# Sukikui/PTI-LDM-VAE

Measured on AMD Instinct MI355X. Metric: vae_train_images_per_sec_256x256, higher is better.
Workload: dtype fp16 forward operands + activations / bf16 backward operands + gradients, fp32 accumulate; 1 GPU; config/vae_dente_no_adv.json 256x256x1 batch 32/GPU: fwd + L1 + 1e-3*KL + bwd + all-reduce + Adam (perceptual term omitted: --perceptual times it; adversarial branch inactive before epoch 6, --adv times it); global_batch=32, parallelism=dp1

## Files before the change

### include/pti_vae.h

```cpp
#ifndef PTI_VAE_H
#define PTI_VAE_H

#include <stdint.h>

#ifdef __cplusplus
extern "C" {
#endif

typedef void* pti_stream_t;

#define PTI_ABI_VERSION 5

#define PTI_OK 0
#define PTI_EINVAL (-1)
#define PTI_EUNSUPPORTED (-2)
#define PTI_ELAUNCH (-3)

#define PTI_CONV_S1 0
#define PTI_CONV_S2PAD 1
#define PTI_CONV_UP2 2
#define PTI_CONV_ZINS 3

#define PTI_PRO_NONE 0
#define PTI_PRO_GN 1
#define PTI_PRO_GN_SILU 2

typedef struct pti_conv_desc {
  int32_t n, h, w, cin;
  int32_t ho, wo, cout;
  int32_t ksize;
  int32_t mode;
  int32_t prologue;
  int32_t groups;
  int32_t add_residual;
  int32_t accum_stats;
  int32_t out_groups;
  float eps;
  int32_t in_f32;
  int32_t out_f32;
  int64_t in_stride[4];
  int64_t out_stride[4];
  int32_t in_f16, res_f16, out_f16;
  int32_t pool2x2_out;
  int32_t w_f16;
  int32_t relu_out;
} pti_conv_desc;

int pti_abi_version(void);
const char* pti_last_error_string(void);
const char* pti_last_kernel_name(void);

int64_t pti_conv_packed_bytes(int cout, int cin, int ksize, int mode);
int pti_conv_pack_weights(const float* const* w_oihw, int nsrc, void* packed, int cout, int cin,
                          int ksize, int mode, int transpose_flip, int w_f16, pti_stream_t s);

int pti_conv_pack_entry_bytes(void);
int pti_conv_pack_table_fill(void* host_entry, const float* w_oihw_dev, void* packed_dev, int cout,
                             int cin, int ksize, int mode, int transpose_flip, int w_f16, int64_t* nblocks);
int pti_conv_pack_weights_batched(const void* table_dev, const int* blk_first_dev, int n,
                                  int total_blocks, pti_stream_t s);

int pti_gn_stats(const void* x_nhwc_16bit, int64_t* stats, int n, int hw, int c, int groups,
                 int x_f16, pti_stream_t s);

int pti_conv2d_mfma(const void* x, const void* w_packed, const float* bias, const int64_t* in_stats,
                    const float* gamma, const float* beta, const void* residual, void* y,
                    int64_t* out_stats, const pti_conv_desc* d, pti_stream_t s);

int pti_conv2d_mfma_saveact(const void* x, const void* w_packed, const float* bias, const int64_t* in_stats,
                            const float* gamma, const float* beta, const void* residual, void* y,
                            int64_t* out_stats, void* act_out, const pti_conv_desc* d, pti_stream_t s);

int pti_conv2d_direct(const void* x, const float* w_tck, const float* bias, const int64_t* in_stats,
                      const float* gamma, const float* beta, void* y, const pti_conv_desc* d,
                      pti_stream_t s);

#define PTI_DIRECT_REPACK_MAX 8
typedef struct {
  const float* w; const float* b;
  float* w_tck; float* w_tck_t; float* wpad; float* bpad;
  int cout, cin, pad_cin, reserved;
} pti_direct_repack_entry;
typedef struct {
  pti_direct_repack_entry e[PTI_DIRECT_REPACK_MAX];
  int n;
} pti_direct_repack_table;
int pti_direct_repack(const pti_direct_repack_table* t, pti_stream_t s);

int pti_wgrad_direct(const void* wide, const void* narrow, float* dw, float* dbias_wide,
                     float* dbias_narrow, const int64_t* in_stats, const float* gamma,
                     const float* beta, int n, int h, int w, int cw, int cn, int ksize, int sgn,
                     int prologue, int groups, float eps, int narrow_f32, int wide_f16,
                     const int64_t* narrow_stride, int64_t dw_stride_tap, int64_t dw_stride_cw,
                     int64_t dw_stride_k, void* workspace, int64_t workspace_bytes, pti_stream_t s);

int64_t pti_conv_wgrad_workspace_bytes(int cout, int cin, int ksize, int splits);
int pti_conv_wgrad_mfma(const void* x, const void* dy, const int64_t* in_stats, const float* gamma,
                        const float* beta, float* dw, float* dbias, void* workspace,
                        int64_t workspace_bytes, int accumulate, const pti_conv_desc* d,
                        pti_stream_t s);
int pti_conv_wgrad_mfma_partials(const void* x, const void* dy, const int64_t* in_stats,
                                 const float* gamma, const float* beta, void* workspace,
                                 int64_t workspace_bytes, const pti_conv_desc* d, int* splits_out,
                                 pti_stream_t s);
int pti_conv_wgrad_reduce(const void* workspace, int splits, float* dw, float* dbias,
                          int accumulate, const pti_conv_desc* d, pti_stream_t s);

#define PTI_WGRAD_BATCH_MAX 16
typedef struct pti_wgrad_job {
  const void* x;
  const void* dy;
  float* dw;
  float* dbias;
  int32_t n, h, w, cin, cout;
  int32_t accumulate;
} pti_wgrad_job;
int pti_conv_wgrad_mfma_batched(const pti_wgrad_job* jobs, int njobs, void* workspace, int64_t workspace_bytes,
                                pti_stream_t s);
int pti_conv_wgrad_batched_mode(int n, int h, int w, int cin, int cout);

int pti_gn_bwd_blocks(int n, int hw, int c);
int pti_gn_bwd(const void* x, const void* da, const void* dres, void* dx, const int64_t* stats,
               const float* gamma, const float* beta, float* sums, float* partials, float* dgamma,
               float* dbeta, int n, int hw, int c, int groups, float eps, int silu, int x_f16,
               pti_stream_t s);
int pti_conv_gnbwd_tiles(const pti_conv_desc* d);
int pti_conv_gnbwd_chain_supported(int cin, int cout, int ksize);
int pti_conv2d_mfma_gnbwd_chain(const void* g_in, const void* x_in, int x_in_f16, const int64_t* in_stats,
                                const float* in_gamma, const float* in_sums, void* dx_in_out, const void* w_packed,
                                const void* gx, const int64_t* gstats, const float* ggamma, const float* gbeta,
                                void* dy_out, float* gsums, const pti_conv_desc* d, int silu, pti_stream_t s);
int pti_gn_affine_grads(const float* sums, float* dgamma, float* dbeta, int n, int c, pti_stream_t s);
int pti_gn_sums_finalize_affine(const float* partials, float* sums, int n, int tiles, int row_len, const float* affine_sums,
                                float* dgamma, float* dbeta, int affine_c, pti_stream_t s);
int pti_conv2d_mfma_gnbwd(const void* dy_in, const void* w_packed, const void* gx, const int64_t* gstats,
                          const float* ggamma, const float* gbeta, void* dy_out, float* gpartials,
                          const pti_conv_desc* d, int silu, pti_stream_t s);
int pti_gn_sums_finalize(const float* partials, float* sums, int n, int tiles, int row_len,
                         pti_stream_t s);
int pti_gn_bwd_apply(const void* x, const void* dy, const void* dres, void* dx, const int64_t* stats,
                     const float* gamma, const float* beta, const float* sums, float* dgamma,
                     float* dbeta, int n, int hw, int c, int groups, float eps, int x_f16,
                     pti_stream_t s);
int pti_pool2x2_sum(const void* x, void* y, int n, int h, int w, int c, pti_stream_t s);

int pti_attention_fwd(const void* qkv, void* o, float* lse2, int b, int l, int c, pti_stream_t s);
int pti_attention_bwd(const void* qkv, const void* o, const void* dout, const float* lse2,
                      float* delta, void* dqkv, int b, int l, int c, pti_stream_t s);

int pti_latent_head_fwd(const float* h, const float* eps, const float* wm, const float* bm,
                        const float* wl, const float* bl, const float* wp, const float* bp,
                        float* mu, float* sigma, float* logvar, float* zq, int b, int hw, int l,
                        pti_stream_t s);
int pti_post_quant(const float* z_nchw, const float* wp, const float* bp, float* zq_nhwc, int b,
                   int hw, int l, pti_stream_t s);
#define PTI_POST_QUANT_BWD_MAX_BLOCKS 256
#define PTI_POST_QUANT_BWD_WS_FLOATS(l) (PTI_POST_QUANT_BWD_MAX_BLOCKS * ((l) * (l) + (l)))
int pti_post_quant_bwd(const float* dzq_nhwc, const float* z_nchw, const float* wp, float* dz_nchw,
                       float* gwp, float* gbp, float* workspace, int b, int hw, int l,
                       pti_stream_t s);
#define PTI_LATENT_BWD_MAX_BLOCKS 512
#define PTI_LATENT_BWD_WS_FLOATS(l) (PTI_LATENT_BWD_MAX_BLOCKS * 3 * ((l) * (l) + (l)))
int pti_latent_head_bwd(const float* h, const float* eps, const float* wm, const float* bm,
                        const float* wl, const float* bl, const float* wp, const float* bp,
                        const float* dzq, const float* dmu, const float* dsigma, float* dh,
                        float* gwm, float* gbm, float* gwl, float* gbl, float* gwp, float* gbp,
                        float* workspace, int b, int hw, int l, pti_stream_t s);

#define PTI_VAE_LOSS_MAX_BLOCKS 1024
#define PTI_VAE_LOSS_WS_FLOATS (2 * PTI_VAE_LOSS_MAX_BLOCKS)
int pti_vae_loss(const float* recon, const float* images, int64_t npix, const float* mu,
                 const float* third, int64_t nlat, int batch, float* out2, float* d_recon,
                 float* d_mu, float* d_third, float* workspace, int l2, int third_mode,
                 float kl_weight, pti_stream_t s);

int pti_ar_vae_loss(const float* mu_nchw, int b, int l, int hw, const float* attrs, const int32_t* channels,
                    const float* deltas, int na, const uint8_t* pair_mask, float gamma, float* per_attr,
                    int32_t* counts, float* d_mu, pti_stream_t s);

int pti_adam_step(float* p, const float* g, float* m, float* v, int64_t n, float lr, float beta1,
                  float beta2, float eps, int step, float grad_scale, pti_stream_t s);

int pti_cast_nchw_f32_to_nhwc_bf16(const float* x, void* y, int n, int c, int hw, pti_stream_t s);
int pti_cast_nhwc_bf16_to_nchw_f32(const void* x, float* y, int n, int c, int hw, pti_stream_t s);

int pti_preprocess_batch(const float* src, const int64_t* offsets, const int32_t* hw, int b, int hp, int wp,
                         float* out, double* stats, pti_stream_t s);

int pti_pd_im2col_image(const float* img, void* patches, int n, int h, int w, pti_stream_t s);
int pti_pd_im2col(const void* src, const float* norm, void* patches, int n, int h, int w, int c, int stride,
                  int act, float slope, pti_stream_t s);
int pti_pd_in_stats(const void* y, float* table, int n, int hw, int c, float eps, pti_stream_t s);
int pti_pd_col2im_blocks(int n, int hw, int c);
int pti_pd_col2im(const void* d_patches, const void* y_prev, const float* norm, void* g, float* partials, int n,
                  int h, int w, int c, int stride, float slope, pti_stream_t s);
int pti_pd_col2im_image(const void* d_patches, float* d_img, int n, int h, int w, float scale, int accumulate,
                        pti_stream_t s);
int pti_pd_in_bwd_apply(const void* g, const void* y, const float* norm, const float* sums, void* dy, int n, int hw,
                        int c, pti_stream_t s);
int pti_pd_lsgan_blocks(int count);
int pti_pd_lsgan(const void* logits, int logits_f16, int stride, int count, float target, float slope,
                 float grad_scale, float* loss_out, void* d_logits, pti_stream_t s);

int pti_pd_final_fwd(const void* y_prev, const float* norm, const float* w, const float* bias, float* logits, int n,
                     int h, int w_, int c, float slope, pti_stream_t s);
int pti_pd_final_dgrad(const float* d_logits, const void* y_prev, const float* norm, const float* w, void* g,
                       float* partials, int n, int h, int w_, int c, float slope, pti_stream_t s);
int pti_pd_final_wgrad_blocks(int n, int h, int w_);
int pti_pd_final_wgrad(const float* d_logits, const void* y_prev, const float* norm, float* partials, int n, int h,
                       int w_, int c, float slope, pti_stream_t s);

int pti_lpips_tap_blocks(int c, int hw);
int pti_lpips_tap_fwd(const float* a, const float* b, const float* w, float* saved, float* partials, int n, int c, int hw,
                      pti_stream_t s);
int pti_lpips_tap_bwd(const float* a, const float* b, const float* w, const float* saved, const float* gout, float* ga,
                      int n, int c, int hw, pti_stream_t s);

int pti_relu_f16(void* x, int64_t count, pti_stream_t s);
int pti_relu_bwd(void* g, const void* y, int64_t count, pti_stream_t s);
int pti_relu_bwd_add(void* g, const void* g2, const void* y, int64_t count, pti_stream_t s);
int pti_maxpool3s2_out(int h);
int pti_maxpool3s2_fwd(const void* x, void* y, int n, int h, int w, int c, pti_stream_t s);
int pti_maxpool3s2_bwd(const void* gy, const void* x, const void* y, void* gx, int n, int h, int w, int c, int accumulate,
                       pti_stream_t s);
int pti_squeeze_conv1_fwd(const float* x, const float* w10, void* y, int n, int h, int w, pti_stream_t s);
int pti_squeeze_conv1_bwd(const void* g, const void* t0, const float* w10, float* dx, int n, int h, int w, pti_stream_t s);
int pti_nchw_f32_to_nhwc_f16(const float* x, void* y, int n, int c, int hw, pti_stream_t s);
int pti_nhwc_bf16_add_to_nchw_f32(const void* g, float* y, int n, int c, int hw, pti_stream_t s);
int pti_pad_nchw_to_nhwc32(const float* x, void* ya, void* yb, int n, int c, int hw, int a_f16, int b_f16, pti_stream_t s);
int pti_slice_nhwc32_to_nchw(const void* x, float* y, int n, int c, int hw, int x_f16, pti_stream_t s);
int pti_lpips_tap_nhwc_blocks(int c, int hw);
int pti_lpips_tap_nhwc_fwd(const void* a, const void* b, const float* w, float* saved, float* partials, int n, int c,
                           int hw, pti_stream_t s);
int pti_lpips_tap_nhwc_bwd(const void* a, const void* b, const float* w, const float* saved, const float* gout, void* ga,
                           int n, int c, int hw, pti_stream_t s);


int64_t pti_image_metrics_ws_floats(int n, int c, int h, int w);
int pti_image_metrics(const float* pred, const float* target, int n, int c, int h, int w, int clamp, float lo, float hi,
                      float data_range, float k1, float k2, const float* taps11, float* out_n4, float* workspace,
                      pti_stream_t s);

int64_t pti_latent_pairwise_ws_floats(int n1, int n2, int d);
int pti_latent_pairwise(const float* a, int64_t lda, int n1, const float* b, int64_t ldb, int n2, int d, const float* center,
                        int mode, float* out, int64_t ldo, float* workspace, pti_stream_t s);
int64_t pti_latent_group_stats_ws_floats(int n1, int n2, int patients, int d);
int pti_latent_group_stats(const float* a, int64_t lda, int n1, const int32_t* seg_a, const float* b, int64_t ldb, int n2,
                           const int32_t* seg_b, int patients, int d, float* out_e4, float* workspace, pti_stream_t s);

int pti_mask_geometry(const void* src, const int64_t* offsets, const int32_t* hw, int b, int elem, int max_h,
                      const int32_t* sample_rows, int samples, const int32_t* bottom_offsets, int n_bottom,
                      int32_t* bbox_b4, int32_t* bbox_widths, int32_t* bottom_widths, pti_stream_t s);

#define PTI_MLP_MAX_LAYERS 8
#define PTI_MLP_MAX_WIDTH 1024
#define PTI_MLP_MAX_OUT 64
int64_t pti_mlp_head_ws_floats(int n, int d, const int32_t* dims, int n_layers);
int pti_mlp_head_fwd(const float* x, int64_t ldx, int n, int d, const float* params, const int32_t* dims, int n_layers,
                     int act, const float* mean, const float* std, const float* targets, int loss_kind, float* pred,
                     float* rowloss, float* workspace, pti_stream_t s);
int pti_regression_metrics(const float* pred, const float* targets, const float* rowloss, int n, int t, int batch,
                           double* out, pti_stream_t s);

#define PTI_ELASTIC_MAX_RADIUS 30
int pti_elastic_field(const uint64_t* keys, const float* alpha, float sigma, int b, int h, int w, float* field,
                      pti_stream_t s);
int pti_augment_warp(const float* src, const float* mat, const float* field, int b, int c, int h, int w, float* out,
                     pti_stream_t s);

int64_t pti_tsne_affinities_ws_floats(int n);
int pti_tsne_affinities(const float* d2, int64_t ldd, int n, float perplexity, float* p, int64_t ldp, double* plogp2,
                        float* workspace, pti_stream_t s);
int64_t pti_tsne_step_ws_floats(int n, int n_components);
int pti_tsne_step(const float* p, int64_t ldp, int n, int n_components, const float* y_in, float* y_out, float* update,
                  float* gains, const double* plogp2, float exaggeration, float momentum, float lr, double* record,
                  int with_record, float* workspace, pti_stream_t s);

int pti_umap_knn(const float* dist, int64_t ldd, int n, int k, int* knn_idx, float* knn_dist, pti_stream_t s);
int64_t pti_umap_graph_capacity(int n, int k);
int64_t pti_umap_graph_ws_floats(int n, int k);
int pti_umap_graph(const int* knn_idx, const float* knn_dist, int n, int k, int n_epochs, int* indptr, int* indices,
                   float* weights, int* rate, int64_t capacity, float* rho, float* sigma, float* workspace, pti_stream_t s);
int pti_umap_epoch(const int* indptr, const int* indices, const int* rate, int64_t capacity, int n, int n_components,
                   const float* y_in, float* y_out, double a, double b, double alpha, int epoch, uint32_t seed,
                   int negative_sample_rate, pti_stream_t s);

int pti_umap_knn_cross(const float* dist, int64_t ldd, int m, int n, int k, int* knn_idx, float* knn_dist, pti_stream_t s);
int64_t pti_umap_transform_graph_ws_floats(int m, int n, int k);
int pti_umap_transform_graph(const int* knn_idx, const float* knn_dist, int m, int k, const float* y_train, int n, int n_epochs,
                             float* sigma, float* weights, int* rate, float* y0, float* workspace, pti_stream_t s);
int pti_umap_transform_layout(const int* knn_idx, const int* rate, int m, int k, const float* y_train, int n, const float* y_in,
                              float* y_out, double a, double b, double initial_alpha, int n_epochs, int epoch_begin,
                              int epoch_end, uint32_t seed, int negative_sample_rate, pti_stream_t s);

int pti_display_planes(const float* a, const float* b, int n, int h, int w, int nsrc, double low, double high, int rot_k,
                       float* out_f32, uint8_t* out_u8, double* stats, pti_stream_t s);

int64_t pti_rank_agreement_ws_bytes(int n, int l, int na);
int pti_rank_agreement(const float* zt, int64_t ldz, const float* attrs, int64_t lda, int n, int l, int na,
                       const int32_t* channels, const float* deltas, int64_t* counts, double* loss_sum, void* workspace,
                       int64_t ws_bytes, pti_stream_t s);

int pti_tied_ranks(const float* cols, int64_t ld, int n, int m, int32_t* rank2, pti_stream_t s);
int pti_rank_moments(const int32_t* rank2, int n, int m, int64_t* sums, int64_t* gram, pti_stream_t s);

int64_t pti_joint_histogram_ws_bytes(int n, int l, int na, int bins);
int pti_joint_histogram(const float* zt, int64_t ldz, const float* attrs, int64_t lda, int n, int l, int na, int bins,
                        const double* edges_z, const double* edges_a, uint8_t* bins_z, uint8_t* bins_a, int32_t* counts,
                        void* workspace, int64_t ws_bytes, pti_stream_t s);

int pti_ksg_counts(const float* zt, int64_t ldz, const float* attrs, int64_t lda, int n, int l, int na, int k, float* eps,
                   int32_t* nx, int32_t* ny, pti_stream_t s);

#define PTI_MASK_COMPARE_MAX_EDGE 1024
#define PTI_MASK_COMPARE_COLUMNS 24
int64_t pti_mask_compare_ws_bytes(int n, int h, int w);
int pti_mask_compare(const float* gt, const float* pred, int n, int h, int w, float threshold, int32_t* counts, double* sums,
                     void* workspace, int64_t ws_bytes, pti_stream_t s);

int pti_neighbor_ranks(const float* dist, int64_t ldd, int n, const int32_t* nbr_idx, int m, int32_t* out, pti_stream_t s);
int pti_segment_row_sums(const float* dist, int64_t ldd, int n, const int32_t* seg, int groups, double* out, pti_stream_t s);
int pti_projection_distances(const float* y, int64_t ldy, int n, int d, float* out, int64_t ldo, pti_stream_t s);

int pti_full_ranks(const float* dist, int64_t ldd, int m, int n, int row0, int16_t* out, int64_t ldo, pti_stream_t s);
int pti_coranking_fold(const int16_t* rank_high, int64_t ldh, const int16_t* rank_low, int64_t ldl, int m, int n, uint32_t* hist,
                       int64_t* sqdiff, pti_stream_t s);
int pti_shepard_fold(const float* dist_high, int64_t ldh, const float* dist_low, int64_t ldl, int n, const float* scale, int bins,
                     double* sums, uint32_t* hist, pti_stream_t s);

#define PTI_MASK_MOMENTS_COLUMNS 10
#define PTI_ALIGN_BOTTOM_COLUMNS 6
int64_t pti_mask_moments_ws_bytes(int n, int h, int w);
int pti_mask_moments(const float* gt, const float* pred, int n, int h, int w, float threshold, float* cleaned, int64_t* moments,
                     double* coeffs, void* workspace, int64_t ws_bytes, pti_stream_t s);
int pti_warp_cubic(const float* gt, const float* pred, const double* coeffs, int n, int h, int w, float* out_gt, float* out_pred,
                   pti_stream_t s);
int pti_align_bottom(const float* rot_gt, const float* rot_pred, int n, int h, int w, float* aligned, int32_t* info,
                     pti_stream_t s);

int64_t pti_ssim_uniform_ws_bytes(int n, int h, int w);
int pti_ssim_uniform(const float* x, const float* y, int n, int h, int w, double data_range, double* out, void* workspace,
                     int64_t ws_bytes, pti_stream_t s);
int pti_mask_compare_cleaned(const float* gt, const float* pred, int n, int h, int w, float threshold, int32_t* counts,
                             double* sums, float* cleaned, void* workspace, int64_t ws_bytes, pti_stream_t s);

#ifdef __cplusplus
}
#endif
#endif
```

### pti_ldm_vae_amd/_lib.py

```python
from __future__ import annotations

import ctypes as C
import os

_HERE = os.path.dirname(os.path.abspath(__file__))
LIB_PATH = os.environ.get("PTI_VAE_LIB") or os.path.join(_HERE, "libpti_vae_hip.so")

def env_overrides() -> dict:
    return {k: v for k, v in sorted(os.environ.items()) if k.startswith("PTI_")}


def refuse_wrong_result_env(who: str) -> None:
    bad = [k for k in os.environ if k.startswith("PTI_") and ("DIAG" in k or k == "PTI_ALLOW_WRONG_RESULTS")]
    if bad:
        raise SystemExit(f"{who}: refusing to run with wrong-result diagnostic variable(s) set: {sorted(bad)} "
                         "(timing diagnostics live in tools/diag_skip.py)")


ABI_VERSION = 5
PTI_CONV_S1, PTI_CONV_S2PAD, PTI_CONV_UP2, PTI_CONV_ZINS = 0, 1, 2, 3
PTI_PRO_NONE, PTI_PRO_GN, PTI_PRO_GN_SILU = 0, 1, 2


class ConvDesc(C.Structure):

    _fields_ = [
        ("n", C.c_int32), ("h", C.c_int32), ("w", C.c_int32), ("cin", C.c_int32),
        ("ho", C.c_int32), ("wo", C.c_int32), ("cout", C.c_int32),
        ("ksize", C.c_int32), ("mode", C.c_int32), ("prologue", C.c_int32), ("groups", C.c_int32),
        ("add_residual", C.c_int32), ("accum_stats", C.c_int32), ("out_groups", C.c_int32),
        ("eps", C.c_float), ("in_f32", C.c_int32), ("out_f32", C.c_int32),
        ("in_stride", C.c_int64 * 4), ("out_stride", C.c_int64 * 4),
        ("in_f16", C.c_int32), ("res_f16", C.c_int32), ("out_f16", C.c_int32), ("pool2x2_out", C.c_int32),
        ("w_f16", C.c_int32), ("relu_out", C.c_int32),
    ]


class WgradJob(C.Structure):

    _fields_ = [("x", C.c_void_p), ("dy", C.c_void_p), ("dw", C.c_void_p), ("dbias", C.c_void_p),
                ("n", C.c_int32), ("h", C.c_int32), ("w", C.c_int32), ("cin", C.c_int32), ("cout", C.c_int32),
                ("accumulate", C.c_int32)]


WGRAD_BATCH_MAX = 16
DIRECT_REPACK_MAX = 8
MASK_COMPARE_COLUMNS = ("n_gt", "n_pred", "components_gt", "components_pred", "kept_gt", "kept_pred", "filled_pred",
                        "intersection", "union", "gt_x", "gt_y", "gt_w", "gt_h", "pred_x", "pred_y", "pred_w", "pred_h",
                        "gt_width_upper", "gt_width_middle", "gt_width_lower",
                        "pred_width_upper", "pred_width_middle", "pred_width_lower", "status")
MASK_MOMENTS_COLUMNS = ("m00", "m10", "m01", "m20", "m11", "m02", "A", "B", "C", "status")
ALIGN_BOTTOM_COLUMNS = ("centre_gt", "centre_pred", "count_gt", "count_pred", "shift", "status")


class DirectRepackEntry(C.Structure):

    _fields_ = [("w", C.c_void_p), ("b", C.c_void_p), ("w_tck", C.c_void_p), ("w_tck_t", C.c_void_p), ("wpad", C.c_void_p),
                ("bpad", C.c_void_p), ("cout", C.c_int32), ("cin", C.c_int32), ("pad_cin", C.c_int32), ("reserved", C.c_int32)]


class DirectRepackTable(C.Structure):

    _fields_ = [("e", DirectRepackEntry * DIRECT_REPACK_MAX), ("n", C.c_int32)]


_P = C.c_void_p
_I = C.c_int
_I64 = C.c_int64
_F = C.c_float
_D = C.c_double
_U32 = C.c_uint32

SIGNATURES = {
    "pti_abi_version": (_I, []),
    "pti_last_error_string": (C.c_char_p, []),
    "pti_last_kernel_name": (C.c_char_p, []),
    "pti_conv_packed_bytes": (_I64, [_I, _I, _I, _I]),
    "pti_conv_pack_weights": (_I, [C.POINTER(_P), _I, _P, _I, _I, _I, _I, _I, _I, _P]),
    "pti_conv_pack_entry_bytes": (_I, []),
    "pti_conv_pack_table_fill": (_I, [_P, _P, _P, _I, _I, _I, _I, _I, _I, C.POINTER(_I64)]),
    "pti_conv_pack_weights_batched": (_I, [_P, _P, _I, _I, _P]),
    "pti_gn_stats": (_I, [_P, _P, _I, _I, _I, _I, _I, _P]),
    "pti_conv2d_mfma": (_I, [_P, _P, _P, _P, _P, _P, _P, _P, _P, C.POINTER(ConvDesc), _P]),
    "pti_conv2d_mfma_saveact": (_I, [_P, _P, _P, _P, _P, _P, _P, _P, _P, _P, C.POINTER(ConvDesc), _P]),
    "pti_conv2d_direct": (_I, [_P, _P, _P, _P, _P, _P, _P, C.POINTER(ConvDesc), _P]),
    "pti_wgrad_direct": (_I, [_P, _P, _P, _P, _P, _P, _P, _P, _I, _I, _I, _I, _I, _I, _I, _I, _I, _F, _I, _I,
                              C.POINTER(_I64), _I64, _I64, _I64, _P, _I64, _P]),
    "pti_conv_wgrad_workspace_bytes": (_I64, [_I, _I, _I, _I]),
    "pti_conv_wgrad_mfma": (_I, [_P, _P, _P, _P, _P, _P, _P, _P, _I64, _I, C.POINTER(ConvDesc), _P]),
    "pti_conv_wgrad_mfma_partials": (_I, [_P, _P, _P, _P, _P, _P, _I64, C.POINTER(ConvDesc), C.POINTER(_I), _P]),
    "pti_conv_wgrad_mfma_batched": (_I, [C.POINTER(WgradJob), _I, _P, _I64, _P]),
    "pti_conv_wgrad_batched_mode": (_I, [_I, _I, _I, _I, _I]),
    "pti_direct_repack": (_I, [C.POINTER(DirectRepackTable), _P]),
    "pti_conv_wgrad_reduce": (_I, [_P, _I, _P, _P, _I, C.POINTER(ConvDesc), _P]),
    "pti_gn_bwd_blocks": (_I, [_I, _I, _I]),
    "pti_gn_bwd": (_I, [_P, _P, _P, _P, _P, _P, _P, _P, _P, _P, _P, _I, _I, _I, _I, _F, _I, _I, _P]),
    "pti_conv_gnbwd_tiles": (_I, [C.POINTER(ConvDesc)]),
    "pti_gn_sums_finalize": (_I, [_P, _P, _I, _I, _I, _P]),
    "pti_conv2d_mfma_gnbwd": (_I, [_P, _P, _P, _P, _P, _P, _P, _P, C.POINTER(ConvDesc), _I, _P]),
    "pti_conv_gnbwd_chain_supported": (_I, [_I, _I, _I]),
    "pti_conv2d_mfma_gnbwd_chain": (_I, [_P, _P, _I, _P, _P, _P, _P, _P, _P, _P, _P, _P, _P, _P, C.POINTER(ConvDesc), _I, _P]),
    "pti_gn_affine_grads": (_I, [_P, _P, _P, _I, _I, _P]),
    "pti_gn_sums_finalize_affine": (_I, [_P, _P, _I, _I, _I, _P, _P, _P, _I, _P]),
    "pti_gn_bwd_apply": (_I, [_P, _P, _P, _P, _P, _P, _P, _P, _P, _P, _I, _I, _I, _I, _F, _I, _P]),
    "pti_pool2x2_sum": (_I, [_P, _P, _I, _I, _I, _I, _P]),
    "pti_attention_fwd": (_I, [_P, _P, _P, _I, _I, _I, _P]),
    "pti_attention_bwd": (_I, [_P, _P, _P, _P, _P, _P, _I, _I, _I, _P]),
    "pti_latent_head_fwd": (_I, [_P] * 12 + [_I, _I, _I, _P]),
    "pti_post_quant": (_I, [_P, _P, _P, _P, _I, _I, _I, _P]),
    "pti_post_quant_bwd": (_I, [_P, _P, _P, _P, _P, _P, _P, _I, _I, _I, _P]),
    "pti_latent_head_bwd": (_I, [_P] * 19 + [_I, _I, _I, _P]),
    "pti_vae_loss": (_I, [_P, _P, _I64, _P, _P, _I64, _I, _P, _P, _P, _P, _P, _I, _I, _F, _P]),
    "pti_ar_vae_loss": (_I, [_P, _I, _I, _I, _P, _P, _P, _I, _P, _F, _P, _P, _P, _P]),
    "pti_pd_im2col_image": (_I, [_P, _P, _I, _I, _I, _P]),
    "pti_pd_im2col": (_I, [_P, _P, _P, _I, _I, _I, _I, _I, _I, _F, _P]),
    "pti_pd_in_stats": (_I, [_P, _P, _I, _I, _I, _F, _P]),
    "pti_pd_col2im_blocks": (_I, [_I, _I, _I]),
    "pti_pd_col2im": (_I, [_P, _P, _P, _P, _P, _I, _I, _I, _I, _I, _F, _P]),
    "pti_pd_col2im_image": (_I, [_P, _P, _I, _I, _I, _F, _I, _P]),
    "pti_pd_in_bwd_apply": (_I, [_P, _P, _P, _P, _P, _I, _I, _I, _P]),
    "pti_pd_lsgan_blocks": (_I, [_I]),
    "pti_pd_lsgan": (_I, [_P, _I, _I, _I, _F, _F, _F, _P, _P, _P]),
    "pti_pd_final_fwd": (_I, [_P, _P, _P, _P, _P, _I, _I, _I, _I, _F, _P]),
    "pti_pd_final_dgrad": (_I, [_P, _P, _P, _P, _P, _P, _I, _I, _I, _I, _F, _P]),
    "pti_pd_final_wgrad_blocks": (_I, [_I, _I, _I]),
    "pti_pd_final_wgrad": (_I, [_P, _P, _P, _P, _I, _I, _I, _I, _F, _P]),
    "pti_lpips_tap_blocks": (_I, [_I, _I]),
    "pti_lpips_tap_fwd": (_I, [_P, _P, _P, _P, _P, _I, _I, _I, _P]),
    "pti_lpips_tap_bwd": (_I, [_P, _P, _P, _P, _P, _P, _I, _I, _I, _P]),
    "pti_relu_f16": (_I, [_P, _I64, _P]),
    "pti_relu_bwd": (_I, [_P, _P, _I64, _P]),
    "pti_relu_bwd_add": (_I, [_P, _P, _P, _I64, _P]),
    "pti_maxpool3s2_out": (_I, [_I]),
    "pti_maxpool3s2_fwd": (_I, [_P, _P, _I, _I, _I, _I, _P]),
    "pti_maxpool3s2_bwd": (_I, [_P, _P, _P, _P, _I, _I, _I, _I, _I, _P]),
    "pti_squeeze_conv1_fwd": (_I, [_P, _P, _P, _I, _I, _I, _P]),
    "pti_squeeze_conv1_bwd": (_I, [_P, _P, _P, _P, _I, _I, _I, _P]),
    "pti_nchw_f32_to_nhwc_f16": (_I, [_P, _P, _I, _I, _I, _P]),
    "pti_pad_nchw_to_nhwc32": (_I, [_P, _P, _P, _I, _I, _I, _I, _I, _P]),
    "pti_slice_nhwc32_to_nchw": (_I, [_P, _P, _I, _I, _I, _I, _P]),
    "pti_nhwc_bf16_add_to_nchw_f32": (_I, [_P, _P, _I, _I, _I, _P]),
    "pti_lpips_tap_nhwc_blocks": (_I, [_I, _I]),
    "pti_lpips_tap_nhwc_fwd": (_I, [_P, _P, _P, _P, _P, _I, _I, _I, _P]),
    "pti_lpips_tap_nhwc_bwd": (_I, [_P, _P, _P, _P, _P, _P, _I, _I, _I, _P]),
    "pti_adam_step": (_I, [_P, _P, _P, _P, _I64, _F, _F, _F, _F, _I, _F, _P]),
    "pti_preprocess_batch": (_I, [_P, _P, _P, _I, _I, _I, _P, _P, _P]),
    "pti_cast_nchw_f32_to_nhwc_bf16": (_I, [_P, _P, _I, _I, _I, _P]),
    "pti_cast_nhwc_bf16_to_nchw_f32": (_I, [_P, _P, _I, _I, _I, _P]),
    "pti_image_metrics_ws_floats": (_I64, [_I, _I, _I, _I]),
    "pti_image_metrics": (_I, [_P, _P, _I, _I, _I, _I, _I, _F, _F, _F, _F, _F, _P, _P, _P, _P]),
    "pti_latent_pairwise_ws_floats": (_I64, [_I, _I, _I]),
    "pti_latent_pairwise": (_I, [_P, _I64, _I, _P, _I64, _I, _I, _P, _I, _P, _I64, _P, _P]),
    "pti_latent_group_stats_ws_floats": (_I64, [_I, _I, _I, _I]),
    "pti_latent_group_stats": (_I, [_P, _I64, _I, _P, _P, _I64, _I, _P, _I, _I, _P, _P, _P]),
    "pti_mask_geometry": (_I, [_P, _P, _P, _I, _I, _I, _P, _I, _P, _I, _P, _P, _P, _P]),
    "pti_mlp_head_ws_floats": (_I64, [_I, _I, C.POINTER(C.c_int32), _I]),
    "pti_mlp_head_fwd": (_I, [_P, _I64, _I, _I, _P, C.POINTER(C.c_int32), _I, _I, _P, _P, _P, _I, _P, _P, _P, _P]),
    "pti_regression_metrics": (_I, [_P, _P, _P, _I, _I, _I, _P, _P]),
    "pti_elastic_field": (_I, [_P, _P, _F, _I, _I, _I, _P, _P]),
    "pti_augment_warp": (_I, [_P, _P, _P, _I, _I, _I, _I, _P, _P]),
    "pti_tsne_affinities_ws_floats": (_I64, [_I]),
    "pti_tsne_affinities": (_I, [_P, _I64, _I, _F, _P, _I64, _P, _P, _P]),
    "pti_tsne_step_ws_floats": (_I64, [_I, _I]),
    "pti_tsne_step": (_I, [_P, _I64, _I, _I, _P, _P, _P, _P, _P, _F, _F, _F, _P, _I, _P, _P]),
    "pti_umap_knn": (_I, [_P, _I64, _I, _I, _P, _P, _P]),
    "pti_umap_graph_capacity": (_I64, [_I, _I]),
    "pti_umap_graph_ws_floats": (_I64, [_I, _I]),
    "pti_umap_graph": (_I, [_P, _P, _I, _I, _I, _P, _P, _P, _P, _I64, _P, _P, _P, _P]),
    "pti_umap_epoch": (_I, [_P, _P, _P, _I64, _I, _I, _P, _P, _D, _D, _D, _I, _U32, _I, _P]),
    "pti_umap_knn_cross": (_I, [_P, _I64, _I, _I, _I, _P, _P, _P]),
    "pti_umap_transform_graph_ws_floats": (_I64, [_I, _I, _I]),
    "pti_umap_transform_graph": (_I, [_P, _P, _I, _I, _P, _I, _I, _P, _P, _P, _P, _P, _P]),
    "pti_umap_transform_layout": (_I, [_P, _P, _I, _I, _P, _I, _P, _P, _D, _D, _D, _I, _I, _I, _U32, _I, _P]),
    "pti_display_planes": (_I, [_P, _P, _I, _I, _I, _I, _D, _D, _I, _P, _P, _P, _P]),
    "pti_rank_agreement_ws_bytes": (_I64, [_I, _I, _I]),
    "pti_rank_agreement": (_I, [_P, _I64, _P, _I64, _I, _I, _I, C.POINTER(C.c_int32), C.POINTER(_F), _P, _P, _P, _I64, _P]),
    "pti_tied_ranks": (_I, [_P, _I64, _I, _I, _P, _P]),
    "pti_rank_moments": (_I, [_P, _I, _I, _P, _P, _P]),
    "pti_joint_histogram_ws_bytes": (_I64, [_I, _I, _I, _I]),
    "pti_joint_histogram": (_I, [_P, _I64, _P, _I64, _I, _I, _I, _I, _P, _P, _P, _P, _P, _P, _I64, _P]),
    "pti_ksg_counts": (_I, [_P, _I64, _P, _I64, _I, _I, _I, _I, _P, _P, _P, _P]),
    "pti_mask_compare_ws_bytes": (_I64, [_I, _I, _I]),
    "pti_mask_compare": (_I, [_P, _P, _I, _I, _I, _F, _P, _P, _P, _I64, _P]),
    "pti_neighbor_ranks": (_I, [_P, _I64, _I, _P, _I, _P, _P]),
    "pti_segment_row_sums": (_I, [_P, _I64, _I, _P, _I, _P, _P]),
    "pti_projection_distances": (_I, [_P, _I64, _I, _I, _P, _I64, _P]),
    "pti_full_ranks": (_I, [_P, _I64, _I, _I, _I, _P, _I64, _P]),
    "pti_coranking_fold": (_I, [_P, _I64, _P, _I64, _I, _I, _P, _P, _P]),
    "pti_shepard_fold": (_I, [_P, _I64, _P, _I64, _I, _P, _I, _P, _P, _P]),
    "pti_mask_moments_ws_bytes": (_I64, [_I, _I, _I]),
    "pti_mask_moments": (_I, [_P, _P, _I, _I, _I, _F, _P, _P, _P, _P, _I64, _P]),
    "pti_warp_cubic": (_I, [_P, _P, _P, _I, _I, _I, _P, _P, _P]),
    "pti_align_bottom": (_I, [_P, _P, _I, _I, _I, _P, _P, _P]),
    "pti_ssim_uniform_ws_bytes": (_I64, [_I, _I, _I]),
    "pti_ssim_uniform": (_I, [_P, _P, _I, _I, _I, _D, _P, _P, _I64, _P]),
    "pti_mask_compare_cleaned": (_I, [_P, _P, _I, _I, _I, _F, _P, _P, _P, _P, _I64, _P]),
}

_lib = None


class PtiError(RuntimeError):
    pass


def lib() -> C.CDLL:
    global _lib
    if _lib is None:
        if not os.path.exists(LIB_PATH):
            raise PtiError(
                f"{LIB_PATH} is missing: the HIP extension was not built. Run "
                "`python -c 'import __graft_entry__ as g; g.build()'` (or pti_ldm_vae_amd/csrc/build.sh). "
                "There is no CPU/PyTorch fallback for the VAE hot path.")
        import torch
        handle = C.CDLL(LIB_PATH)
        for name, (res, args) in SIGNATURES.items():
            fn = getattr(handle, name)
            fn.restype = res
            fn.argtypes = args
        ver = handle.pti_abi_version()
        if ver != ABI_VERSION:
            raise PtiError(f"libpti_vae_hip.so ABI version {ver}, expected {ABI_VERSION}")
        _lib = handle
    return _lib


def check(rc: int, what: str = "") -> None:
    if rc != 0:
        msg = lib().pti_last_error_string()
        raise PtiError(f"{what or 'pti call'} failed (code {rc}): {msg.decode() if msg else ''}")
```

### pti_ldm_vae_amd/csrc/conv_mfma.hip

```cpp
#include "conv_common.h"

namespace {
using namespace pti_conv;

constexpr int TH = 8, TW = 16;

__host__ __device__ constexpr int pick_cout_tile(int cout) { return cout % 128 == 0 ? 128 : (cout % 64 == 0 ? 64 : 32); }
__host__ __device__ constexpr int pick_ck(int cin, int stride2) {
  int ck = cin % 128 == 0 ? 128 : (cin % 64 == 0 ? 64 : 32);
  return (stride2 && ck > 64) ? 64 : ck;
}
__host__ __device__ constexpr int pick_wblk(int kbc, int nt) {
  int best = 1;
  for (int w = 1; w <= kbc; ++w)
    if (kbc % w == 0 && w * nt <= 16) best = w;
  return best;
}

template <int KS, int S, int CK, int COUT_TILE>
struct Cfg {
  static constexpr int HH = (TH - 1) * S + KS, HW = (TW - 1) * S + KS;
  static constexpr int NP = HH * HW;
  static constexpr int NC = CK / 8;
  static constexpr int PIXB = CK * 2;
// ... 474 lines not shown
            if constexpr (OPH) {
              float f[8];
              unpack8f(piece, f, true);
              piece = pack8(f);
            }
            __builtin_amdgcn_raw_buffer_store_b128(__builtin_bit_cast(bu32x4, piece), srs,
                                                   ((unsigned)((n * a.H + vy) * a.W + vx) * a.Cin + chunk * CK + c8 * 8) * 2u, 0, 2 );
          }
        }
      }
    }

    if constexpr (WLATE) wload(wa, 0);
    const int txl = lane & 15;
    auto baddr = [&](int kb) -> const unsigned char* {
      kb = kb < C::KBC ? kb : C::KBC - 1;
      const int tap = kb / C::KPC, kc = kb - tap * C::KPC;
      const int kh = (KS == 3) ? tap / 3 : 0, kw = tap - kh * KS;
      const int hx = txl + kw;
      const int tk = (hsel ^ ((hx >> C::KEY_SHIFT) & (C::NC - 1))) << 4;
      return halo + pbase[0] + (kh * C::HW + kw) * C::PIXB + ((kc * 32) ^ tk);
    };
    bf16x8 b0[PXF], b1[PXF];
    auto bread = [&](bf16x8 (&dst)[PXF], int kb) {
      const unsigned char* bp = baddr(kb);
#pragma unroll
      for (int i = 0; i < PXF; ++i) dst[i] = *(const bf16x8*)(bp + 2 * i * C::HW * C::PIXB);
    };
    auto group = [&](const bf16x8 (&w)[C::R], int g) {
      const int kb0 = g * C::R;
#pragma unroll
      for (int u = 0; u < C::R; ++u) {
        if ((u & 1) == 0) {
          bread(b1, kb0 + u + 1);
#pragma unroll
          for (int i = 0; i < PXF; ++i) acc[i] = mfma32<OPH>(w[u], b0[i], acc[i]);
        } else {
          bread(b0, kb0 + u + 1);
#pragma unroll
          for (int i = 0; i < PXF; ++i) acc[i] = mfma32<OPH>(w[u], b1[i], acc[i]);
        }
      }
      if (C::R & 1) {
#pragma unroll
        for (int i = 0; i < PXF; ++i) b0[i] = b1[i];
      }
    };
    constexpr int NG = C::KBC / C::R;
    bread(b0, 0);
    if constexpr (NG == 1) {
      group(wa, 0);
    } else {
#pragma clang loop unroll(disable)
      for (int g = 0; g < NG; g += 2) {
        wload(wb, g + 1);
        group(wa, g);
        wload(wa, g + 2);
        group(wb, g + 1);
      }
    }
  }

  const int j = lane & 31;
  unsigned char* etile = smem;
  const bool do_stats = (FM == 2 || FM == 3) ? false : a.out_stats != nullptr;
  const int ocpg = do_stats ? a.Cout / a.out_groups : 1;
  __syncthreads();
  float* gtab = reinterpret_cast<float*>(smem + C::GT_OFF);
  if (gn_on) {
    if (tid < CT) {
      gtab[tid] = gq;
      gtab[CT + tid] = bq;
    }
    __syncthreads();
  }
  const unsigned char* rtile = smem + C::RT_OFF;
  const int col0 = wn * 32 + 4 * hsel;
  float st1[4] = {0.f, 0.f, 0.f, 0.f}, st2[4] = {0.f, 0.f, 0.f, 0.f};
  float su1[4] = {0.f, 0.f, 0.f, 0.f}, su2[4] = {0.f, 0.f, 0.f, 0.f};
  if (gn_on) {
    const int gcpg = a.Cout / a.g_groups;
    float* gsm = reinterpret_cast<float*>(smem + C::STAT_OFF);
    float L[32];
#pragma unroll
    for (int q = 0; q < 4; ++q) {
      const int col = col0 + 8 * q, ch0 = ct * CT + col;
      float scv[4], shv[4], muv[4], rsv[4], l1[4] = {0.f, 0.f, 0.f, 0.f}, l2[4] = {0.f, 0.f, 0.f, 0.f};
      gn_params<4>(sfl, gtab - ct * CT, gtab + CT - ct * CT, ch0, gcpg, a.g_inv_cnt, a.g_eps, scv, shv, muv, rsv);
      float nmr[4];
#pragma unroll
      for (int r = 0; r < 4; ++r) nmr[r] = -muv[r] * rsv[r];
#pragma unroll
      for (int i = 0; i < PXF; ++i) {
        const int p = (2 * PXF * wm + 2 * i + (j >> 4)) * 16 + (j & 15);
        const bool inb = (oy0 + (p >> 4) < a.Ho) && (ox0 + (p & 15) < a.Wo);
        unsigned char* ep = etile + p * C::EPITCH + col * 2;
        const u32x2 rr = *(const u32x2*)(rtile + p * (CT * 2) + ((((col >> 3) ^ (p >> 2)) & (C::ENC - 1)) << 4) + (col & 7) * 2);
        float xv[4];
        unpack2f(rr[0], res_f16, xv[0], xv[1]);
        unpack2f(rr[1], res_f16, xv[2], xv[3]);
        float dv[4];
#pragma unroll
        for (int r = 0; r < 4; ++r) {
          float v = acc[i][4 * q + r];
          if (a.gn_mode == 2) v *= dsilu_f(xv[r] * scv[r] + shv[r]);
          dv[r] = v;
        }
        const u32x2 packed = pack4(dv[0], dv[1], dv[2], dv[3]);
        *(u32x2*)ep = packed;
        if (inb) {
#pragma unroll
          for (int r = 0; r < 4; ++r) {
            l1[r] += dv[r];
            l2[r] = fmaf(dv[r], fmaf(xv[r], rsv[r], nmr[r]), l2[r]);
          }
        }
      }
#pragma unroll
      for (int r = 0; r < 4; ++r) {
        L[8 * q + 2 * r] = l1[r];
        L[8 * q + 2 * r + 1] = l2[r];
      }
    }
    fold32<32>(L, j);
    gsm[wm * 2 * CT + col0 * 2 + 16 * (j >> 3) + (j & 7)] = L[0];
  } else {
#pragma unroll
  for (int i = 0; i < PXF; ++i) {
    const int p = (2 * PXF * wm + 2 * i + (j >> 4)) * 16 + (j & 15);
    const bool inb = (oy0 + (p >> 4) < a.Ho) && (ox0 + (p & 15) < a.Wo);
#pragma unroll
    for (int q = 0; q < 4; ++q) {
      const int col = col0 + 8 * q;
      float v0 = acc[i][4 * q + 0], v1 = acc[i][4 * q + 1], v2 = acc[i][4 * q + 2], v3 = acc[i][4 * q + 3];
      if (a.bias) {
        const f32x4 b = *(const f32x4*)(smem + C::BIAS_OFF + col * 4);
        v0 += b[0]; v1 += b[1]; v2 += b[2]; v3 += b[3];
      }
      unsigned char* ep = etile + p * C::EPITCH + col * 2;
      if (a.res) {
        const u32x2 rr = *(const u32x2*)(rtile + p * (CT * 2) + ((((col >> 3) ^ (p >> 2)) & (C::ENC - 1)) << 4) + (col & 7) * 2);
        float e0, e1, e2, e3;
        unpack2f(rr[0], res_f16, e0, e1);
        unpack2f(rr[1], res_f16, e2, e3);
        v0 += e0; v1 += e1; v2 += e2; v3 += e3;
      }
      if constexpr (FM == 1 && PRO == PTI_PRO_NONE) {
        if (a.relu_out) { v0 = fmaxf(v0, 0.f); v1 = fmaxf(v1, 0.f); v2 = fmaxf(v2, 0.f); v3 = fmaxf(v3, 0.f); }
      }
      const u32x2 packed = pack4f(v0, v1, v2, v3, out_f16);
      *(u32x2*)ep = packed;
      if (do_stats && inb) {
        float r0, r1, r2, r3;
        unpack2f(packed[0], out_f16, r0, r1);
        unpack2f(packed[1], out_f16, r2, r3);
        if (ocpg >= 4) {
          st1[q] += (r0 + r1) + (r2 + r3);
          st2[q] += (r0 * r0 + r1 * r1) + (r2 * r2 + r3 * r3);
        } else {
          st1[q] += r0 + r1; st2[q] += r0 * r0 + r1 * r1;
          su1[q] += r2 + r3; su2[q] += r2 * r2 + r3 * r3;
        }
      }
    }
  }
  }
  if (do_stats) {
    stat_t* sstat = reinterpret_cast<stat_t*>(smem + C::STAT_OFF);
    if (ocpg >= 4) {
      float v[8];
#pragma unroll
      for (int q = 0; q < 4; ++q) { v[2 * q] = st1[q]; v[2 * q + 1] = st2[q]; }
      fold32<8>(v, j);
      if ((j & 3) == 0) {
        const int idx = j >> 2, q = idx >> 1;
        const int g = (ct * CT + col0 + 8 * q) / ocpg;
        stat_add(&sstat[2 * g + (idx & 1)], v[0]);
      }
    } else {
      float v[16];
#pragma unroll
      for (int q = 0; q < 4; ++q) { v[4 * q] = st1[q]; v[4 * q + 1] = st2[q]; v[4 * q + 2] = su1[q]; v[4 * q + 3] = su2[q]; }
      fold32<16>(v, j);
      if ((j & 1) == 0) {
        const int idx = j >> 1, q = idx >> 2;
        const int g = (ct * CT + col0 + 8 * q) / 2;
        stat_add(&sstat[2 * g + (idx & 3)], v[0]);
      }
    }
  }
  __syncthreads();
  const __amdgpu_buffer_rsrc_t yrs = __builtin_amdgcn_make_buffer_rsrc(
      a.y, 0, ((unsigned)a.N * (unsigned)a.Ho * (unsigned)a.Wo * (unsigned)a.Cout * 2u) >> (a.pool2 ? 2 : 0), 0x00020000);
  if ((FM == 0 || FM == 2) && a.pool2) {
    constexpr int PITERS = (C::EITERS + 3) / 4;
#pragma unroll
    for (int it = 0; it < PITERS; ++it) {
      const int idx = tid + it * 256;
      const int c8 = idx % C::ENC, pp = idx / C::ENC;
      const int py = pp / 8, px = pp % 8;
      const int oy = (oy0 >> 1) + py, ox = (ox0 >> 1) + px;
      if (pp < C::MPX / 4 && oy < (a.Ho >> 1) && ox < (a.Wo >> 1)) {
        const unsigned char* src = etile + ((2 * py) * 16 + 2 * px) * C::EPITCH + c8 * 16;
        float s_[8], f_[8];
        unpack8f(*(const u32x4*)src, s_, out_f16);
        unpack8f(*(const u32x4*)(src + C::EPITCH), f_, out_f16);
#pragma unroll
        for (int q = 0; q < 8; ++q) s_[q] += f_[q];
        unpack8f(*(const u32x4*)(src + 16 * C::EPITCH), f_, out_f16);
#pragma unroll
        for (int q = 0; q < 8; ++q) s_[q] += f_[q];
        unpack8f(*(const u32x4*)(src + 17 * C::EPITCH), f_, out_f16);
#pragma unroll
        for (int q = 0; q < 8; ++q) s_[q] += f_[q];
        __builtin_amdgcn_raw_buffer_store_b128(__builtin_bit_cast(bu32x4, pack8f(s_, out_f16)), yrs,
                                               ((unsigned)((n * (a.Ho >> 1) + oy) * (a.Wo >> 1) + ox) * a.Cout + ct * CT + c8 * 8) * 2u, 0, 2);
      }
    }
  } else
#pragma unroll
  for (int it = 0; it < C::EITERS; ++it) {
    const int p = epp0 + it * EPSTEP;
    const int oy = oy0 + (p >> 4), ox = ox0 + (p & 15);
    if (oy < a.Ho && ox < a.Wo)
      __builtin_amdgcn_raw_buffer_store_b128(__builtin_bit_cast(bu32x4, *(const u32x4*)(etile + p * C::EPITCH + epc * 16)), yrs,
                                             ((unsigned)((n * a.Ho + oy) * a.Wo + ox) * a.Cout + ct * CT + epc * 8) * 2u, 0, 2);
  }
  if (gn_on) {
    if (tid < 2 * CT) {
      const float* gsm = reinterpret_cast<const float*>(smem + C::STAT_OFF);
      float v = gsm[tid];
#pragma unroll
      for (int m = 1; m < C::WM; ++m) v += gsm[m * 2 * CT + tid];
      a.g_sums[(((size_t)n * a.g_T + tile_y * a.tiles_x + tile_x) * a.Cout + ct * CT) * 2 + tid] = v;
    }
  } else if (do_stats) {
    const stat_t* sstat = reinterpret_cast<const stat_t*>(smem + C::STAT_OFF);
    const int g0 = (ct * CT) / ocpg, ng = CT / ocpg;
    if (tid < 2 * ng)
      atomicAdd((unsigned long long*)&a.out_stats[(n * a.out_groups + g0) * 2 + tid], (unsigned long long)sstat[2 * g0 + tid]);
  }
}

template <int KS, int CK, int CT, int PXF>
int launch2_cfg(ConvArgs a, hipStream_t st) {
  using C = Cfg2<KS, CK, CT, PXF>;
  a.tiles_x = cdiv(a.Wo, C::TW2);
  a.tiles_y = cdiv(a.Ho, C::TH2);
  a.g_T = a.tiles_x * a.tiles_y;
  dim3 grid(a.N * a.tiles_x * a.tiles_y, a.Cout / CT);
  const bool res = a.res != nullptr;
  const int fm = (a.w_f16 && a.in_f16 && a.out_f16 && (a.res_f16 || !res)) ? 1
               : (!a.in_f16 && !a.out_f16 && (!a.res_f16 || !res)) ? 2
               : (!a.in_f16 && !a.out_f16 && a.res_f16) ? 3 : 0;
  const bool fwd_silu = fm == 1 && a.prologue == PTI_PRO_GN_SILU && !a.gn_mode && !a.pool2;
  const bool fwd_plain = fm == 1 && a.prologue == PTI_PRO_NONE && !a.gn_mode && !a.pool2;
  const bool dgrad = fm == 2 && a.prologue == PTI_PRO_NONE && !a.gn_mode && !a.out_stats;
  const bool dgrad_gn = fm == 3 && a.prologue == PTI_PRO_NONE && a.gn_mode && !a.out_stats && !a.pool2;
  if (a.x2) {
    if constexpr (KS == 3 && PXF == 4 && CT == 128) {
      if (!(fm == 3 && a.gn_mode && a.act_out && !a.out_stats && !a.pool2 && a.mode == PTI_CONV_S1 && !a.relu_out)) return 4;
      PTI_LAUNCH((conv_mfma2_kernel<KS, CK, CT, PXF, true, 3, PRO_GNB>), grid, dim3(256), 0, st, a);
      return 0;
    } else {
      return 4;
    }
  }
  if (a.relu_out && !(fwd_plain && !a.act_out)) return 3;
  constexpr int FPRO = PXF == 4 ? PTI_PRO_GN_SILU : -1;
  const bool fwd_gn_rt = fm == 1 && a.prologue == PTI_PRO_GN && !a.gn_mode && !a.pool2 && FPRO < 0;
  if constexpr (KS == 3) {
    if (a.act_out) {
      if (fwd_silu || fwd_gn_rt) PTI_LAUNCH((conv_mfma2_kernel<KS, CK, CT, PXF, true, 1, FPRO>), grid, dim3(256), 0, st, a);
      else if (a.w_f16) return 2;
      else PTI_LAUNCH((conv_mfma2_kernel<KS, CK, CT, PXF, true, 0, -1>), grid, dim3(256), 0, st, a);
      return 0;
    }
  } else if (a.act_out) {
    return 1;
  }
  if (fwd_silu) PTI_LAUNCH((conv_mfma2_kernel<KS, CK, CT, PXF, false, 1, FPRO>), grid, dim3(256), 0, st, a);
  else if (fwd_plain) PTI_LAUNCH((conv_mfma2_kernel<KS, CK, CT, PXF, false, 1, PTI_PRO_NONE>), grid, dim3(256), 0, st, a);
  else if (fm == 1 && !a.gn_mode && !a.pool2) PTI_LAUNCH((conv_mfma2_kernel<KS, CK, CT, PXF, false, 1, -1>), grid, dim3(256), 0, st, a);
  else if (a.w_f16) return 2;
  else if (dgrad) PTI_LAUNCH((conv_mfma2_kernel<KS, CK, CT, PXF, false, 2, PTI_PRO_NONE>), grid, dim3(256), 0, st, a);
  else if (dgrad_gn) PTI_LAUNCH((conv_mfma2_kernel<KS, CK, CT, PXF, false, 3, PTI_PRO_NONE>), grid, dim3(256), 0, st, a);
  else PTI_LAUNCH((conv_mfma2_kernel<KS, CK, CT, PXF, false, 0, -1>), grid, dim3(256), 0, st, a);
  return 0;
}
template <int KS>
int launch2(const ConvArgs& a, int ck, int ct, hipStream_t st) {
  if (ct == 128) {
    if (ck == 128) return launch2_cfg<KS, 128, 128, 4>(a, st);
    if (ck == 64) return launch2_cfg<KS, 64, 128, 4>(a, st);
    return launch2_cfg<KS, 32, 128, 4>(a, st);
  }
  if (ct == 64) {
    if (ck == 64) return launch2_cfg<KS, 64, 64, 2>(a, st);
    return launch2_cfg<KS, 32, 64, 2>(a, st);
  }
  return launch2_cfg<KS, 32, 32, 2>(a, st);
}

struct PackArgs {
  const float* src[4];
  int nsrc;
  bf16* dst;
  int cout_l, cin_l;
  int cout_o, cin_o;
  int ks, ck, cout_tile, flip;
  int f16;
  long long total;
};

__device__ __forceinline__ void pack_eight(const PackArgs& p, int e8) {
  const int NT = p.cout_tile / 32, KPC = p.ck / 16, KBC = p.ks * p.ks * KPC, nch = p.cin_l / p.ck;
  int r = e8;
  const int lane = r % 64; r /= 64;
  const int nt = r % NT; r /= NT;
  const int kb = r % KBC; r /= KBC;
  const int chunk = r % nch;
  const int ct = r / nch;
  const int co = ct * p.cout_tile + nt * 32 + (lane & 31);
  const int tap = kb / KPC, kc = kb % KPC;
  const int ci0 = chunk * p.ck + kc * 16 + 8 * (lane >> 5);
  const int kk = p.ks * p.ks;
  const float* src;
  size_t stride;
  if (!p.flip) {
    const int s_ = co / p.cout_o, cs = co % p.cout_o;
    src = p.src[s_] + ((size_t)cs * p.cin_o + ci0) * kk + tap;
    stride = kk;
  } else {
    src = p.src[0] + ((size_t)ci0 * p.cin_o + co) * kk + (kk - 1 - tap);
    stride = (size_t)p.cin_o * kk;
  }
  float f[8];
#pragma unroll
  for (int j = 0; j < 8; ++j) f[j] = src[j * stride];
  *(u32x4*)(p.dst + (size_t)e8 * 8) = p.f16 ? pack8f(f, true) : pack8(f);
}

__global__ void pack_weights_kernel(PackArgs p) {
  if (p.f16) fp16_saturate_on();
  const long long e8 = (long long)blockIdx.x * blockDim.x + threadIdx.x;
  if (e8 * 8 < p.total) pack_eight(p, (int)e8);
}

__global__ void pack_weights_batched_kernel(const PackArgs* __restrict__ table, const int* __restrict__ blk_first, int n) {
  int lo = 0, hi = n - 1;
  const int b = blockIdx.x;
  while (lo < hi) {
    const int mid = (lo + hi + 1) >> 1;
    if (blk_first[mid] <= b) lo = mid; else hi = mid - 1;
  }
  const PackArgs p = table[lo];
  if (p.f16) fp16_saturate_on();
  const int e8 = (b - blk_first[lo]) * 256 + threadIdx.x;
  if ((long long)e8 * 8 < p.total) pack_eight(p, e8);
}

template <int KS, int S, int CK, int COUT_TILE>
int launch_cfg(const ConvArgs& a, hipStream_t st) {
  dim3 grid(a.N * a.tiles_x * a.tiles_y, a.Cout / COUT_TILE);
  if (a.w_f16) PTI_LAUNCH((conv_mfma_kernel<KS, S, CK, COUT_TILE, true>), grid, dim3(256), 0, st, a);
  else PTI_LAUNCH((conv_mfma_kernel<KS, S, CK, COUT_TILE, false>), grid, dim3(256), 0, st, a);
  return 0;
}

template <int KS, int S, int CK>
int launch_ct(const ConvArgs& a, int cout_tile, hipStream_t st) {
  switch (cout_tile) {
    case 128: return launch_cfg<KS, S, CK, 128>(a, st);
    case 64: return launch_cfg<KS, S, CK, 64>(a, st);
    default: return launch_cfg<KS, S, CK, 32>(a, st);
  }
}

template <int KS, int S>
int launch_ck(const ConvArgs& a, int ck, int cout_tile, hipStream_t st) {
  static_assert(S == 2, "the v1 kernel is kept for the stride-2 gather only");
  switch (ck) {
    case 64: return launch_ct<KS, S, 64>(a, cout_tile, st);
    default: return launch_ct<KS, S, 32>(a, cout_tile, st);
  }
}

}

extern "C" int64_t pti_conv_packed_bytes(int cout, int cin, int ksize, int mode) {
  (void)mode;
  if (cout <= 0 || cin <= 0 || cout % 32 || cin % 32 || (ksize != 1 && ksize != 3)) return 0;
  return (int64_t)2 * cout * cin * ksize * ksize;
}

extern "C" int pti_conv_pack_weights(const float* const* w, int nsrc, void* packed, int cout, int cin,
                                     int ksize, int mode, int transpose_flip, int w_f16, pti_stream_t s) {
  if (!w || !packed || nsrc < 1 || nsrc > 4) PTI_FAIL(PTI_EINVAL, "pack_weights: bad pointer/nsrc");
  if (cout % 32 || cin % 32 || (ksize != 1 && ksize != 3))
    PTI_FAIL(PTI_EUNSUPPORTED, "pack_weights: cout=%d cin=%d k=%d need multiples of 32, k in {1,3}", cout, cin, ksize);
  if (transpose_flip && nsrc != 1) PTI_FAIL(PTI_EINVAL, "pack_weights: transpose_flip needs nsrc=1");
  PackArgs p;
  for (int i = 0; i < 4; ++i) p.src[i] = i < nsrc ? w[i] : nullptr;
  p.nsrc = nsrc;
  p.dst = (bf16*)packed;
  p.cout_o = cout;
  p.cin_o = cin;
  p.cout_l = transpose_flip ? cin : cout * nsrc;
  p.cin_l = transpose_flip ? cout : cin;
  p.ks = ksize;
  p.flip = transpose_flip;
  p.f16 = w_f16 ? 1 : 0;
  p.cout_tile = pick_cout_tile(p.cout_l);
  p.ck = (mode == PTI_CONV_S2PAD) ? pick_ck(p.cin_l, true) : pick_ck2(p.cin_l, p.cout_tile);
  p.total = (long long)p.cout_l * p.cin_l * ksize * ksize;
  const int blocks = (int)((p.total + 2047) / 2048);
  PTI_LAUNCH(pack_weights_kernel, dim3(blocks), dim3(256), 0, (hipStream_t)s, p);
  PTI_CHECK_LAUNCH("pack_weights");
  return PTI_OK;
}

static int fill_pack(PackArgs& p, const float* w, void* packed, int cout, int cin, int ksize, int mode, int flip, int f16) {
  if (cout % 32 || cin % 32 || (ksize != 1 && ksize != 3)) return -1;
  for (int i = 0; i < 4; ++i) p.src[i] = nullptr;
  p.src[0] = w;
  p.nsrc = 1;
  p.dst = (bf16*)packed;
  p.cout_o = cout; p.cin_o = cin;
  p.cout_l = flip ? cin : cout;
  p.cin_l = flip ? cout : cin;
  p.ks = ksize; p.flip = flip; p.f16 = f16 ? 1 : 0;
  p.cout_tile = pick_cout_tile(p.cout_l);
  p.ck = (mode == PTI_CONV_S2PAD) ? pick_ck(p.cin_l, true) : pick_ck2(p.cin_l, p.cout_tile);
  p.total = (long long)p.cout_l * p.cin_l * ksize * ksize;
  return 0;
}

extern "C" int pti_conv_pack_entry_bytes(void) { return (int)sizeof(PackArgs); }
extern "C" int pti_conv_pack_table_fill(void* host_entry, const float* w, void* packed, int cout, int cin, int ksize,
                                        int mode, int transpose_flip, int w_f16, int64_t* nblocks) {
  if (!host_entry || !w || !packed || !nblocks) PTI_FAIL(PTI_EINVAL, "pack_table_fill: null pointer");
  PackArgs p;
  if (fill_pack(p, w, packed, cout, cin, ksize, mode, transpose_flip, w_f16))
    PTI_FAIL(PTI_EUNSUPPORTED, "pack_table_fill: cout=%d cin=%d k=%d", cout, cin, ksize);
  *(PackArgs*)host_entry = p;
  *nblocks = (p.total + 2047) / 2048;
  return PTI_OK;
}
extern "C" int pti_conv_pack_weights_batched(const void* table_dev, const int* blk_first_dev, int n, int total_blocks,
                                             pti_stream_t s) {
  if (!table_dev || !blk_first_dev || n <= 0 || total_blocks <= 0) PTI_FAIL(PTI_EINVAL, "pack_weights_batched: bad args");
  PTI_LAUNCH(pack_weights_batched_kernel, dim3(total_blocks), dim3(256), 0, (hipStream_t)s,
                     (const PackArgs*)table_dev, blk_first_dev, n);
  PTI_CHECK_LAUNCH("pack_weights_batched");
  return PTI_OK;
}

struct GnBwdFuse {
  int mode; const int64_t* stats; const float* gamma; const float* beta; float* sums;
  const void* x2 = nullptr; int x2_f16 = 0; const int64_t* p_stats = nullptr; const float* p_gamma = nullptr; const float* p_sums = nullptr;
};

static int conv2d_mfma_impl(const void* x, const void* w_packed, const float* bias, const int64_t* in_stats,
                            const float* gamma, const float* beta, const void* residual, void* y,
                            int64_t* out_stats, const pti_conv_desc* d, const GnBwdFuse* gf, void* act_out,
                            pti_stream_t s) {
  if (!x || !w_packed || !y || !d) PTI_FAIL(PTI_EINVAL, "conv2d_mfma: null pointer");
  const bool chain = gf && gf->x2;
  if (act_out && !chain && (d->mode != PTI_CONV_S1 || d->prologue == PTI_PRO_NONE || d->ksize != 3))
    PTI_FAIL(PTI_EUNSUPPORTED, "conv2d_mfma: the activated-input side output needs a 3x3 PTI_CONV_S1 launch with a GroupNorm prologue");
  if (d->cin % 32 || d->cout % 32 || d->cin <= 0 || d->cout <= 0)
    PTI_FAIL(PTI_EUNSUPPORTED, "conv2d_mfma: cin=%d cout=%d must be positive multiples of 32", d->cin, d->cout);
  if (d->ksize != 1 && d->ksize != 3) PTI_FAIL(PTI_EUNSUPPORTED, "conv2d_mfma: ksize %d", d->ksize);
  if (d->ksize == 1 && d->mode != PTI_CONV_S1) PTI_FAIL(PTI_EUNSUPPORTED, "conv2d_mfma: 1x1 supports PTI_CONV_S1 only");
  if (d->n <= 0 || d->h <= 0 || d->w <= 0) PTI_FAIL(PTI_EINVAL, "conv2d_mfma: bad dims");
  int eho, ewo;
  switch (d->mode) {
    case PTI_CONV_S1: eho = d->h; ewo = d->w; break;
    case PTI_CONV_S2PAD: eho = (d->h + 1 - 3) / 2 + 1; ewo = (d->w + 1 - 3) / 2 + 1; break;
    case PTI_CONV_UP2: case PTI_CONV_ZINS: eho = 2 * d->h; ewo = 2 * d->w; break;
    default: PTI_FAIL(PTI_EUNSUPPORTED, "conv2d_mfma: mode %d", d->mode);
  }
  if (d->ho != eho || d->wo != ewo)
    PTI_FAIL(PTI_EINVAL, "conv2d_mfma: output %dx%d does not match mode %d on %dx%d (want %dx%d)", d->ho, d->wo,
             d->mode, d->h, d->w, eho, ewo);
  if (d->prologue != PTI_PRO_NONE) {
    if (!in_stats || !gamma || !beta || d->groups <= 0 || d->cin % d->groups)
      PTI_FAIL(PTI_EINVAL, "conv2d_mfma: prologue needs stats/gamma/beta and groups | cin");
    if (d->groups > 32) PTI_FAIL(PTI_EUNSUPPORTED, "conv2d_mfma: prologue supports at most 32 groups");
  }
  if (d->add_residual && !residual) PTI_FAIL(PTI_EINVAL, "conv2d_mfma: add_residual without residual");
  if (d->accum_stats) {
    if (!out_stats || d->out_groups <= 0 || d->cout % d->out_groups) PTI_FAIL(PTI_EINVAL, "conv2d_mfma: bad out stats");
    const int ocpg = d->cout / d->out_groups;
    if (ocpg != 2 && (ocpg % 4 != 0 || ocpg > 32)) PTI_FAIL(PTI_EUNSUPPORTED, "conv2d_mfma: channels/group %d for fused stats", ocpg);
    if (d->out_groups > 64) PTI_FAIL(PTI_EUNSUPPORTED, "conv2d_mfma: fused statistics support at most 64 groups");
  }
  ConvArgs a;
  a.x = (const bf16*)x; a.w = (const unsigned char*)w_packed; a.bias = bias; a.in_stats = (const stat_t*)in_stats;
  a.gamma = gamma; a.beta = beta; a.res = d->add_residual ? (const bf16*)residual : nullptr; a.y = (bf16*)y;
  a.out_stats = d->accum_stats ? (stat_t*)out_stats : nullptr;
  a.N = d->n; a.H = d->h; a.W = d->w; a.Cin = d->cin; a.Ho = d->ho; a.Wo = d->wo; a.Cout = d->cout;
  a.mode = d->mode; a.prologue = d->prologue; a.groups = d->groups; a.out_groups = d->out_groups;
  a.gn_mode = 0; a.g_groups = 0; a.g_inv_cnt = 0.f; a.g_eps = 0.f;
  a.g_stats = nullptr; a.g_gamma = a.g_beta = nullptr; a.g_sums = nullptr; a.g_T = 0;
  a.act_out = (bf16*)act_out;
  a.in_f16 = d->in_f16; a.res_f16 = d->res_f16; a.out_f16 = d->out_f16;
  a.pool2 = d->pool2x2_out;
  a.w_f16 = d->w_f16;
  a.relu_out = d->relu_out;
  if (a.relu_out && (gf || d->mode == PTI_CONV_S2PAD))
    PTI_FAIL(PTI_EUNSUPPORTED, "conv2d_mfma: relu_out is for plain fp16 forward launches (stride-1 gather, no prologue)");
  if (a.w_f16 && !(d->in_f16 && d->out_f16 && (d->res_f16 || !d->add_residual)) )
    PTI_FAIL(PTI_EUNSUPPORTED, "conv2d_mfma: fp16-packed weights need fp16 input, output and residual (the forward convs)");
  if (a.w_f16 && (gf || d->pool2x2_out))
    PTI_FAIL(PTI_EUNSUPPORTED, "conv2d_mfma: fp16-packed weights are for forward launches only");
  if (a.pool2 && (d->mode == PTI_CONV_S2PAD || d->accum_stats || gf || (d->ho & 1) || (d->wo & 1)))
    PTI_FAIL(PTI_EUNSUPPORTED, "conv2d_mfma: pool2x2_out needs a stride-1 gather, even output size, no fused statistics");
  a.eps = d->eps;
  a.inv_cnt = d->prologue != PTI_PRO_NONE ? 1.0f / ((float)(d->cin / d->groups) * (float)d->h * (float)d->w) : 0.f;
  if (gf) {
    if (d->groups > 32) PTI_FAIL(PTI_EUNSUPPORTED, "conv2d_mfma_gnbwd: at most 32 groups");
    a.gn_mode = gf->mode; a.g_groups = d->groups; a.g_eps = d->eps;
    a.g_inv_cnt = 1.0f / ((float)(d->cout / d->groups) * (float)d->ho * (float)d->wo);
    a.g_stats = (const stat_t*)gf->stats; a.g_gamma = gf->gamma; a.g_beta = gf->beta; a.g_sums = gf->sums;
  }
  a.x2 = nullptr; a.p_sums = nullptr; a.x2_f16 = 0;
  if (chain) {
    if (!gf->p_stats || !gf->p_gamma || !gf->p_sums || !act_out || d->mode != PTI_CONV_S1 || d->ksize != 3 ||
        d->cin % d->groups || d->cin / d->groups < 8)
      PTI_FAIL(PTI_EINVAL, "conv2d_mfma_gnbwd_chain: bad arguments (3x3 stride-1, >= 8 channels per group)");
    a.x2 = (const bf16*)gf->x2; a.x2_f16 = gf->x2_f16; a.p_sums = gf->p_sums;
    a.in_stats = (const stat_t*)gf->p_stats; a.gamma = gf->p_gamma; a.groups = d->groups;
    a.inv_cnt = 1.0f / ((float)(d->cin / d->groups) * (float)d->h * (float)d->w);
  }
  if ((long long)d->n * d->ho * d->wo * d->cout * 2 >= (1ll << 31))
    PTI_FAIL(PTI_EUNSUPPORTED, "conv2d_mfma: output tensor of %lld bytes (the stores use 32-bit offsets: < 2 GiB)",
             (long long)d->n * d->ho * d->wo * d->cout * 2);
  if (d->mode != PTI_CONV_S2PAD && (long long)d->n * d->h * d->w * d->cin * 2 >= (1ll << 31))
    PTI_FAIL(PTI_EUNSUPPORTED, "conv2d_mfma: input tensor of %lld bytes (the halo loads use 32-bit offsets: < 2 GiB)",
             (long long)d->n * d->h * d->w * d->cin * 2);
  a.tiles_x = cdiv(d->wo, TW); a.tiles_y = cdiv(d->ho, TH);
  const int cout_tile = pick_cout_tile(d->cout);
  int rc, ck;
  if (d->mode == PTI_CONV_S2PAD) {
    ck = pick_ck(d->cin, true);
    rc = launch_ck<3, 2>(a, ck, cout_tile, (hipStream_t)s);
  } else {
    ck = pick_ck2(d->cin, cout_tile);
    rc = (d->ksize == 3 && d->cin == 128 && d->cout == 128 && !a.x2) ? launch_conv_ws128(a, (hipStream_t)s) : 1;
    if (rc == 1)
      rc = d->ksize == 1 ? launch2<1>(a, ck, cout_tile, (hipStream_t)s) : launch2<3>(a, ck, cout_tile, (hipStream_t)s);
  }
  if (rc == 3) PTI_FAIL(PTI_EUNSUPPORTED, "conv2d_mfma: relu_out needs a plain fp16 forward launch (w_f16, fp16 in/out, no prologue, no side output)");
  if (rc == 2) PTI_FAIL(PTI_EUNSUPPORTED, "conv2d_mfma: no fp16-operand kernel for this launch (w_f16 with this prologue / epilogue)");
  if (rc == 4) PTI_FAIL(PTI_EUNSUPPORTED, "conv2d_mfma_gnbwd_chain: only 3x3 launches on 128-wide input and output tiles with an fp16 GroupNorm input");
  if (rc != 0) PTI_FAIL(PTI_EUNSUPPORTED, "conv2d_mfma: no kernel for ck=%d cout_tile=%d", ck, cout_tile);
  PTI_CHECK_LAUNCH("conv2d_mfma");
  return PTI_OK;
}

extern "C" int pti_conv2d_mfma(const void* x, const void* w_packed, const float* bias, const int64_t* in_stats,
                               const float* gamma, const float* beta, const void* residual, void* y,
                               int64_t* out_stats, const pti_conv_desc* d, pti_stream_t s) {
  return conv2d_mfma_impl(x, w_packed, bias, in_stats, gamma, beta, residual, y, out_stats, d, nullptr, nullptr, s);
}

extern "C" int pti_conv2d_mfma_saveact(const void* x, const void* w_packed, const float* bias, const int64_t* in_stats,
                                       const float* gamma, const float* beta, const void* residual, void* y,
                                       int64_t* out_stats, void* act_out, const pti_conv_desc* d, pti_stream_t s) {
  if (!act_out) PTI_FAIL(PTI_EINVAL, "conv2d_mfma_saveact: null act_out");
  return conv2d_mfma_impl(x, w_packed, bias, in_stats, gamma, beta, residual, y, out_stats, d, nullptr, act_out, s);
}

extern "C" int pti_conv_gnbwd_tiles(const pti_conv_desc* d) {
  if (!d || d->cout % 32 || d->ho <= 0 || d->wo <= 0) return 0;
  const int ct = pick_cout_tile(d->cout);
  const int th = ct == 128 ? 8 : (ct == 64 ? 8 : 16);
  return cdiv(d->ho, th) * cdiv(d->wo, 16);
}

extern "C" int pti_conv_gnbwd_chain_supported(int cin, int cout, int ksize) {
  return ksize == 3 && cin % 128 == 0 && cout % 128 == 0;
}

extern "C" int pti_conv2d_mfma_gnbwd_chain(const void* g_in, const void* x_in, int x_in_f16, const int64_t* in_stats,
                                           const float* in_gamma, const float* in_sums, void* dx_in_out, const void* w_packed,
                                           const void* gx, const int64_t* gstats, const float* ggamma, const float* gbeta,
                                           void* dy_out, float* gsums, const pti_conv_desc* d, int silu, pti_stream_t s) {
  if (!g_in || !x_in || !in_stats || !in_gamma || !in_sums || !dx_in_out || !gx || !gstats || !ggamma || !gbeta || !gsums || !d)
    PTI_FAIL(PTI_EINVAL, "conv2d_mfma_gnbwd_chain: null pointer");
  if (d->mode != PTI_CONV_S1 || d->prologue != PTI_PRO_NONE || d->add_residual || d->accum_stats)
    PTI_FAIL(PTI_EUNSUPPORTED, "conv2d_mfma_gnbwd_chain: plain stride-1 data-gradient launches only");
  if (d->groups <= 0 || d->cout % d->groups || d->cin % d->groups) PTI_FAIL(PTI_EINVAL, "conv2d_mfma_gnbwd_chain: groups must divide cin and cout");
  GnBwdFuse gf{silu ? 2 : 1, gstats, ggamma, gbeta, gsums};
  gf.x2 = x_in; gf.x2_f16 = x_in_f16; gf.p_stats = in_stats; gf.p_gamma = in_gamma; gf.p_sums = in_sums;
  pti_conv_desc dd = *d;
  dd.add_residual = 1;
  return conv2d_mfma_impl(g_in, w_packed, nullptr, nullptr, nullptr, nullptr, gx, dy_out, nullptr, &dd, &gf, dx_in_out, s);
}

extern "C" int pti_conv2d_mfma_gnbwd(const void* dy_in, const void* w_packed, const void* gx, const int64_t* gstats,
                                     const float* ggamma, const float* gbeta, void* dy_out, float* gsums,
                                     const pti_conv_desc* d, int silu, pti_stream_t s) {
  if (!gx || !gstats || !ggamma || !gbeta || !gsums || !d) PTI_FAIL(PTI_EINVAL, "conv2d_mfma_gnbwd: null pointer");
  if (d->mode == PTI_CONV_S2PAD || d->prologue != PTI_PRO_NONE || d->add_residual || d->accum_stats)
    PTI_FAIL(PTI_EUNSUPPORTED, "conv2d_mfma_gnbwd: plain stride-1 / zero-insert data-gradient launches only");
  if (d->groups <= 0 || d->cout % d->groups) PTI_FAIL(PTI_EINVAL, "conv2d_mfma_gnbwd: groups must divide cout");
  GnBwdFuse gf{silu ? 2 : 1, gstats, ggamma, gbeta, gsums};
  pti_conv_desc dd = *d;
  dd.add_residual = 1;
  return conv2d_mfma_impl(dy_in, w_packed, nullptr, nullptr, nullptr, nullptr, gx, dy_out, nullptr, &dd, &gf, nullptr, s);
}
```

### pti_ldm_vae_amd/engine.py

```python
from __future__ import annotations

import contextlib
import gc
import os
import warnings

import torch

from . import ops
from .models import autoencoderkl as M
from .ops import (BF16, F32, PTI_CONV_S1, PTI_CONV_S2PAD, PTI_CONV_UP2, PTI_CONV_ZINS, PTI_PRO_GN, PTI_PRO_GN_SILU,
                  PTI_PRO_NONE)


class _Act:

    __slots__ = ("t", "stats")

    def __init__(self, t, stats=None):
        self.t, self.stats = t, stats


def _empty(shape, like, dtype=BF16):
    return torch.empty(shape, dtype=dtype, device=like.device)


@contextlib.contextmanager
def gc_off_for_capture():
    gc.collect()
    enabled = gc.isenabled()
    gc.disable()
    try:
        yield
    finally:
        if enabled:
            gc.enable()


def capture_or_eager(what, *bodies):
    graphs, results = [], []
    try:
        with gc_off_for_capture():
            for body in bodies:
                g = torch.cuda.CUDAGraph()
                with torch.cuda.graph(g, pool=graphs[0].pool() if graphs else None, capture_error_mode="thread_local"):
                    results.append(body(*results))
                graphs.append(g)
    except Exception as ex:
        warnings.warn(f"HIP-graph capture of {what} failed ({ex!r}); continuing with eager launches")
        torch.cuda.synchronize()
        return None
    return graphs, results


class _MfmaConv:

    def __init__(self, net, wname, bname, ksize, mode, fused_names=None, fwd_f16=True):
        self.net, self.ksize, self.mode = net, ksize, mode
        self.fwd_f16, self.f16 = fwd_f16, False
        self.wname, self.bname, self.fused = wname, bname, fused_names
        if fused_names:
            w0 = net._param_by_name[fused_names[0][0]]
            self.cout, self.cin = 3 * w0.shape[0], w0.shape[1]
        else:
            w = net._param_by_name[wname]
            self.cout, self.cin = w.shape[0], w.shape[1]
        self.wp = self.wpt = None

    def _w(self):
        if self.fused:
            o, n, _ = self.net._slots[self.fused[0][0]]
            return self.net._arena[o:o + 3 * n].view(self.cout, self.cin, 1, 1)
        return self.net._param_by_name[self.wname].data.view(self.cout, self.cin, self.ksize, self.ksize)

    def bias(self):
        if self.fused:
            o, n, _ = self.net._slots[self.fused[0][1]]
            return self.net._arena[o:o + 3 * n]
        return self.net._param_by_name[self.bname].data

    def grads(self):
        if self.fused:
            o, n, _ = self.net._slots[self.fused[0][0]]
            ob, nb, _ = self.net._slots[self.fused[0][1]]
            g = self.net.grad_arena
            return g[o:o + 3 * n], g[ob:ob + 3 * nb]
        return self.net.grad_view(self.wname).view(-1), self.net.grad_view(self.bname)

    def fwd(self, x, *, pro=PTI_PRO_NONE, norm=None, residual=None, want_stats=False, eng=None, act_out=None,
            out_dtype=None):
        n, h, w, _ = x.t.shape
        ho, wo = ops.conv_out_hw(h, w, self.mode)
        y = _empty((n, ho, wo, self.cout), x.t, out_dtype or eng.act_dtype)
        st = eng.new_stats(n) if want_stats else None
        g, b = (norm.weight.data, norm.bias.data) if norm is not None else (None, None)
        ops.conv_mfma(x.t, self.wp, self.bias(), y, cout=self.cout, ksize=self.ksize, mode=self.mode, prologue=pro,
                      in_stats=x.stats if pro else None, gamma=g, beta=b, groups=eng.G, eps=eng.eps,
                      residual=residual, out_stats=st, out_groups=eng.G, act_out=act_out)
        return _Act(y, st)

    def dgrad(self, dy, *, residual=None):
        n, ho, wo, _ = dy.shape
        if self.mode == PTI_CONV_S2PAD:
            out = _empty((n, 2 * ho, 2 * wo, self.cin), dy)
            ops.conv_mfma(dy, self.wpt, None, out, cout=self.cin, ksize=3, mode=PTI_CONV_ZINS, residual=residual)
            return out
        if self.mode == PTI_CONV_UP2:
            pooled = _empty((n, ho // 2, wo // 2, self.cin), dy)
            ops.conv_mfma(dy, self.wpt, None, pooled, cout=self.cin, ksize=self.ksize, mode=PTI_CONV_S1, pool2=True)
            return pooled
        out = _empty((n, ho, wo, self.cin), dy)
        ops.conv_mfma(dy, self.wpt, None, out, cout=self.cin, ksize=self.ksize, mode=PTI_CONV_S1, residual=residual)
        return out

    def dgrad_gn(self, dy, x, norm, *, silu, dres, eng):
        g, sums = self.dgrad_gn_raw(dy, x, norm, silu=silu, eng=eng)
        return self._gn_apply(g, sums, x, norm, dres, eng)

    def _gn_apply(self, g, sums, x, norm, dres, eng):
        dx = _empty(x.t.shape, x.t)
        ops.gn_bwd_apply(x.t, g, dx, x.stats, norm.weight.data, norm.bias.data, sums,
                         norm.net.grad_view(norm.prefix + ".weight"), norm.net.grad_view(norm.prefix + ".bias"),
                         groups=eng.G, eps=eng.eps, dres=dres)
        return dx

    def dgrad_gn_raw(self, dy, x, norm, *, silu, eng):
        n, ho, wo, _ = dy.shape
        g = _empty((n, ho, wo, self.cin), dy)
        sums = eng.zeros(n * self.cin * 2)
        ops.conv_mfma_gnbwd(dy, self.wpt, x.t, x.stats, norm.weight.data, norm.bias.data, g, sums, cout=self.cin,
                            ksize=self.ksize, mode=PTI_CONV_S1, groups=eng.G, eps=eng.eps, silu=silu)
        return g, sums

    def dgrad_gn_chain(self, g_in, x_in, norm_in, sums_in, x, norm, *, silu, dres, eng):
        n, ho, wo, _ = g_in.shape
        dxin = _empty(g_in.shape, g_in)
        dyt = _empty((n, ho, wo, self.cin), g_in)
        sums = eng.zeros(n * self.cin * 2)
        ops.conv_mfma_gnbwd_chain(g_in, x_in.t, x_in.stats, norm_in.weight.data, sums_in, dxin, self.wpt, x.t, x.stats,
                                  norm.weight.data, norm.bias.data, dyt, sums, cout=self.cin, groups=eng.G, eps=eng.eps,
                                  silu=silu, in_dgamma=norm_in.net.grad_view(norm_in.prefix + ".weight"),
                                  in_dbeta=norm_in.net.grad_view(norm_in.prefix + ".bias"))
        return self._gn_apply(dyt, sums, x, norm, dres, eng), dxin

    def wgrad(self, x, dy, *, pro=PTI_PRO_NONE, norm=None, eng=None):
        dw, db = self.grads()
        if eng.batch_wgrad and ops.wgrad_batch_eligible(x.t, dy, self.ksize, self.mode, pro):
            eng.defer_wgrad(x.t, dy, dw, db)
            return
        g, b = (norm.weight.data, norm.bias.data) if norm is not None else (None, None)
        kw = dict(ksize=self.ksize, mode=self.mode, prologue=pro, in_stats=x.stats if pro else None, gamma=g, beta=b,
                  groups=eng.G, eps=eng.eps, accumulate=True)
        with eng.side_stream(x.t, dy, dw, db, *kw.values()) as workspace:
            ops.conv_wgrad_mfma(x.t, dy, dw, db, workspace=workspace, **kw)


class _Norm:
    def __init__(self, net, prefix):
        self.net, self.prefix = net, prefix
        self.weight = net._param_by_name[prefix + ".weight"]
        self.bias = net._param_by_name[prefix + ".bias"]

    def bwd(self, x, da, *, silu, dres, eng):
        n, h, w, c = x.t.shape
        dx = _empty(x.t.shape, x.t)
        sums = eng.zeros(n * c * 2)
        ops.gn_bwd(x.t, da, dx, x.stats, self.weight.data, self.bias.data, sums,
                   self.net.grad_view(self.prefix + ".weight"), self.net.grad_view(self.prefix + ".bias"),
                   groups=eng.G, eps=eng.eps, silu=silu, dres=dres)
        return dx


class _ResBlock:
    def __init__(self, net, p, blk):
        self.norm1, self.norm2 = _Norm(net, p + ".norm1"), _Norm(net, p + ".norm2")
        self.conv1 = _MfmaConv(net, p + ".conv1.conv.weight", p + ".conv1.conv.bias", 3, PTI_CONV_S1)
        self.conv2 = _MfmaConv(net, p + ".conv2.conv.weight", p + ".conv2.conv.bias", 3, PTI_CONV_S1)
        self.nin = None
        if blk.in_channels != blk.out_channels:
            self.nin = _MfmaConv(net, p + ".nin_shortcut.conv.weight", p + ".nin_shortcut.conv.bias", 1, PTI_CONV_S1)
        self.convs = [c for c in (self.conv1, self.conv2, self.nin) if c is not None]
        self.needs_in_stats = True
        self.prefix = p + "."

    def fwd(self, x, eng, want_stats, save):
        a1 = a2 = None
        if save is not None and eng.saves_activated_input(x.t):
            a1 = _empty(x.t.shape, x.t)
        h1 = self.conv1.fwd(x, pro=PTI_PRO_GN_SILU, norm=self.norm1, want_stats=True, eng=eng, act_out=a1)
        sc = x.t if self.nin is None else self.nin.fwd(x, eng=eng).t
        if save is not None and eng.saves_activated_input(h1.t):
            a2 = _empty(h1.t.shape, h1.t)
        out = self.conv2.fwd(h1, pro=PTI_PRO_GN_SILU, norm=self.norm2, residual=sc, want_stats=want_stats, eng=eng,
                             act_out=a2)
        if save is not None:
            save.append((x, h1, a1, a2))
        return out

    @staticmethod
    def _wgrad(conv, x, norm, a, dy, eng):
        if a is not None:
            conv.wgrad(_Act(a), dy, eng=eng)
        else:
            conv.wgrad(x, dy, pro=PTI_PRO_GN_SILU, norm=norm, eng=eng)

    def _shortcut_bwd(self, x, dout, eng):
        if self.nin is None:
            return dout
        dres = self.nin.dgrad(dout)
        self.nin.wgrad(x, dout, eng=eng)
        return dres

    def bwd(self, dout, saved, eng):
        x, h1, a1, a2 = saved
        self._wgrad(self.conv2, h1, self.norm2, a2, dout, eng)
        if eng.gnbwd_chain and ops.gnbwd_chain_supported(self.conv1.cout, self.conv1.cin, 3, x.t.dtype, eng.G):
            g2, sums2 = self.conv2.dgrad_gn_raw(dout, h1, self.norm2, silu=True, eng=eng)
            dres = self._shortcut_bwd(x, dout, eng)
            dx, dh1 = self.conv1.dgrad_gn_chain(g2, h1, self.norm2, sums2, x, self.norm1, silu=True, dres=dres, eng=eng)
            self._wgrad(self.conv1, x, self.norm1, a1, dh1, eng)
            return dx
        dh1 = self.conv2.dgrad_gn(dout, h1, self.norm2, silu=True, dres=None, eng=eng)
        self._wgrad(self.conv1, x, self.norm1, a1, dh1, eng)
        dres = self._shortcut_bwd(x, dout, eng)
        return self.conv1.dgrad_gn(dh1, x, self.norm1, silu=True, dres=dres, eng=eng)


class _Resample:

    def __init__(self, net, wprefix, mode, prefix):
        self.conv = _MfmaConv(net, wprefix + ".weight", wprefix + ".bias", 3, mode)
        self.convs = [self.conv]
        self.needs_in_stats = False
        self.prefix = prefix

    def fwd(self, x, eng, want_stats, save):
        out = self.conv.fwd(x, want_stats=want_stats, eng=eng)
        if save is not None:
            save.append(x)
        return out

    def bwd(self, dout, saved, eng):
        x = saved
        self.conv.wgrad(x, dout, eng=eng)
        return self.conv.dgrad(dout)


class _Attention:
    def __init__(self, net, p):
        self.norm = _Norm(net, p + ".norm")
        a = p + ".attn."
        self.qkv = _MfmaConv(net, None, None, 1, PTI_CONV_S1,
                             fused_names=[(a + "to_q.weight", a + "to_q.bias")], fwd_f16=False)
        self.proj = _MfmaConv(net, a + "out_proj.weight", a + "out_proj.bias", 1, PTI_CONV_S1, fwd_f16=False)
        self.convs = [self.qkv, self.proj]
        self.needs_in_stats = True
        self.prefix = p + "."

    def fwd(self, x, eng, want_stats, save):
        n, h, w, c = x.t.shape
        qkv = self.qkv.fwd(x, pro=PTI_PRO_GN, norm=self.norm, eng=eng, out_dtype=BF16).t
        o = _empty((n, h * w, c), x.t)
        lse = _empty((n, h * w), x.t, F32)
        ops.attention_fwd(qkv.view(n, h * w, 3 * c), o, lse)
        out = self.proj.fwd(_Act(o.view(n, h, w, c)), residual=x.t, want_stats=want_stats, eng=eng)
        if save is not None:
            save.append((x, qkv, o, lse))
        return out

    def bwd(self, dout, saved, eng):
        x, qkv, o, lse = saved
        n, h, w, c = x.t.shape
        do = self.proj.dgrad(dout)
        self.proj.wgrad(_Act(o.view(n, h, w, c)), dout, eng=eng)
        dqkv = _empty(qkv.shape, qkv)
        delta = _empty((n, h * w), qkv, F32)
        ops.attention_bwd(qkv.view(n, h * w, 3 * c), o, do.view(n, h * w, c), lse, delta, dqkv.view(n, h * w, 3 * c))
        self.qkv.wgrad(x, dqkv, pro=PTI_PRO_GN, norm=self.norm, eng=eng)
        return self.qkv.dgrad_gn(dqkv, x, self.norm, silu=False, dres=dout, eng=eng)


class _DirectConv:

    def __init__(self, net, prefix, norm_prefix=None):
        self.net, self.prefix = net, prefix
        self.w = net._param_by_name[prefix + ".weight"]
        self.b = net._param_by_name[prefix + ".bias"]
        self.cout, self.cin = self.w.shape[0], self.w.shape[1]
        self.norm = _Norm(net, norm_prefix) if norm_prefix else None
        self.few_cin = self.cin <= 16
        self.w_tck = self.w_tck_t = None
        self.convs = []
        self.needs_in_stats = self.norm is not None
        narrow, wide = min(self.cin, self.cout), max(self.cin, self.cout)
        self.mfma_narrow = 4 <= narrow <= 32 and wide % 32 == 0
        self.wpad = self.wp_mfma = None
        self.pack_f16 = False
        self.img_mfma = False
        self.wp_img = self.wpt_img = self.wpad_img = self.bpad_img = None
        self.dw_img = self.db_img = None

    def alloc(self):
        w = self.w.data
        if self.w_tck is not None:
            return
        self.w_tck = torch.empty(9, self.cin, self.cout, dtype=F32, device=w.device)
        self.w_tck_t = torch.empty(9, self.cout, self.cin, dtype=F32, device=w.device)
        if self.mfma_narrow:
            shape = (32, self.cin, 3, 3) if self.cout < self.cin else (self.cout, 32, 3, 3)
            self.wpad = torch.zeros(shape, dtype=F32, device=w.device)
            self.bpad = torch.zeros(32, dtype=F32, device=w.device)
        if self.img_mfma:
            shape = (self.cout, 32, 3, 3) if self.cin < self.cout else (32, self.cin, 3, 3)
            self.wpad_img = torch.zeros(shape, dtype=F32, device=w.device)
            self.bpad_img = torch.zeros(32, dtype=F32, device=w.device)
            self.dw_img = torch.zeros(shape, dtype=F32, device=w.device)
            self.db_img = torch.zeros(32, dtype=F32, device=w.device) if self.cout < self.cin else None

    def repack_entries(self):
        w, b = self.w.data, self.b.data
        out = [dict(w=w, b=b, w_tck=self.w_tck, w_tck_t=self.w_tck_t,
                    wpad=self.wpad, bpad=self.bpad if (self.mfma_narrow and self.cout < self.cin) else None)]
        if self.img_mfma:
            out.append(dict(w=w, b=b, wpad=self.wpad_img, bpad=self.bpad_img if self.cout < self.cin else None))
        return out

    def pack_entries(self):
        out = []
        if self.mfma_narrow:
            if self.cout < self.cin:
                out.append(("wp_mfma", (self.wpad, 3, PTI_CONV_S1, False, self.pack_f16)))
            else:
                out.append(("wp_mfma", (self.wpad, 3, PTI_CONV_S1, True, False)))
        if self.img_mfma:
            out.append(("wp_img", (self.wpad_img, 3, PTI_CONV_S1, False, self.pack_f16)))
            if self.cout < self.cin:
                out.append(("wpt_img", (self.wpad_img, 3, PTI_CONV_S1, True, False)))
        return out


class Engine:
    def __init__(self, net: "M.AutoencoderKL"):
        self.net = net
        self.G, self.eps = net.norm_num_groups, float(net.norm_eps)
        self.dev = net.param_arena.device
        self.workspace = ops.wgrad_workspace(self.dev)
        self.packed_version = -1
        self.pack_gen = 0
        self.grad_ready_cb = None
        self._range_cache = {}
        self._zpool, self._zoff, self._zpool_size = None, 0, 1 << 16
        self._packer = None
        self.save_act_min_hw = int(os.environ.get("PTI_SAVE_ACT_MIN_HW", "0"))
        self.act_dtype = {"fp16": torch.float16, "bf16": BF16}[os.environ.get("PTI_FWD_ACT_DTYPE", "fp16")]
        self.wgrad_stream = torch.cuda.Stream(device=self.dev) if os.environ.get("PTI_WGRAD_STREAM", "1") == "1" else None
        self.workspace_side = torch.empty_like(self.workspace) if self.wgrad_stream is not None else None
        self._wgrad_pending = False
        self._side_owned = set()
        self.wgrad_batch_max = max(1, min(ops.L.WGRAD_BATCH_MAX, int(os.environ.get("PTI_WGRAD_BATCH", "16"))))
        self.batch_wgrad = self.wgrad_batch_max > 1
        self._wgrad_jobs, self._ready_queue = [], []
        self.encode_graphs = os.environ.get("PTI_ENCODE_GRAPH", "1") == "1"
        self._enc_graphs, self._dec_graphs, self._enc_graph_version = {}, {}, None
        ops.L.lib()
        for c in net.channels:
            if c % 32:
                raise ValueError(f"HIP path needs channel counts that are multiples of 32, got {net.channels}")
            cpg = c // self.G
            if cpg not in (2, 4, 8, 16, 32) or (c & (c - 1)):
                raise ValueError(f"HIP GroupNorm path supports power-of-two channels with 2..32 channels per group; "
                                 f"got channels={c}, groups={self.G}")
        eb = net.encoder.blocks
        self.enc_in = _DirectConv(net, "encoder.blocks.0.conv")
        self.enc_layers = []
        last = len(eb) - 1
        for i in range(1, last - 1):
            self.enc_layers.append(self._make_layer(eb[i], f"encoder.blocks.{i}"))
        self.enc_out = _DirectConv(net, f"encoder.blocks.{last}.conv", norm_prefix=f"encoder.blocks.{last - 1}")
        db = net.decoder.blocks
        self.dec_in = _DirectConv(net, "decoder.blocks.0.conv")
        self.dec_layers = []
        last = len(db) - 1
        for i in range(1, last - 1):
            self.dec_layers.append(self._make_layer(db[i], f"decoder.blocks.{i}"))
        self.dec_out = _DirectConv(net, f"decoder.blocks.{last}.conv", norm_prefix=f"decoder.blocks.{last - 1}")
        self.mfma_convs = [c for l in self.enc_layers + self.dec_layers for c in l.convs]
        for c in self.mfma_convs:
            c.f16 = c.fwd_f16 and self.act_dtype == torch.float16
        self.direct_convs = [self.enc_in, self.enc_out, self.dec_in, self.dec_out]
        self.enc_out.pack_f16 = self.act_dtype == torch.float16
        img = os.environ.get("PTI_IMG_MFMA", "1") == "1"
        self.enc_in.img_mfma = img and 2 <= net.in_channels <= 8 and net.channels[0] % 32 == 0
        self.dec_out.img_mfma = img and 2 <= net.out_channels <= 8 and net.channels[0] % 32 == 0
        self.enc_in.pack_f16 = self.dec_out.pack_f16 = self.act_dtype == torch.float16
        self._wgrad_posts, self._wgrad_zero = [], ()
        self._flush_up = int(os.environ.get("PTI_WGRAD_FLUSH_UP", "1"))
        self.gnbwd_chain = os.environ.get("PTI_GNBWD_CHAIN", "0") == "1"
        self.Lc = net.latent_channels
        self._plist = list(net._param_by_name.values())

    def saves_activated_input(self, t) -> bool:
        return t.shape[1] * t.shape[2] >= self.save_act_min_hw

    def _make_layer(self, blk, prefix):
        if isinstance(blk, M.AEKLResBlock):
            return _ResBlock(self.net, prefix, blk)
        if isinstance(blk, M.AEKLDownsample):
            return _Resample(self.net, prefix + ".conv.conv", PTI_CONV_S2PAD, prefix + ".")
        if isinstance(blk, M.Upsample):
            return _Resample(self.net, prefix + ".postconv.conv", PTI_CONV_UP2, prefix + ".")
        if isinstance(blk, M.SpatialAttentionBlock):
            return _Attention(self.net, prefix)
        raise TypeError(f"unsupported block {type(blk)} at {prefix}")

    def new_stats(self, n):
        return self.zeros(n * self.G * 4).view(torch.int64).view(n, self.G, 2)

    def zeros(self, count):
        count = (count + 3) // 4 * 4
        pool = self._zpool
        if pool is None or self._zoff + count > pool.numel():
            pool = self._zpool = torch.zeros(max(count, self._zpool_size), dtype=F32, device=self.dev)
            self._zoff = 0
        out = pool[self._zoff:self._zoff + count]
        self._zoff += count
        return out

    def begin_pass(self, batch, backward=False):
        cmax = max(self.net.channels)
        self._zpool_size = (64 * batch * cmax * 2) if backward else (96 * batch * self.G * 2)
        self._zpool = None
        if backward and self.wgrad_stream is not None:
            self._side_owned = {t.untyped_storage().data_ptr()
                                for t in (self.net.param_arena, self.net.grad_arena, self.workspace_side)}

    def _pack_buffer_ids(self):
        ids = [t.data_ptr() for c in self.mfma_convs for t in (c.wp, c.wpt) if t is not None]
        for c in self.direct_convs:
            ids += [t.data_ptr() for t in (c.w_tck, c.w_tck_t, c.wp_mfma, c.wpad, c.wp_img, c.wpt_img, c.wpad_img) if t is not None]
        return tuple(ids)

    def _drop_stale_graphs(self):
        ids = self._pack_buffer_ids()
        if ids != self._enc_graph_version:
            self._enc_graphs.clear()
            self._dec_graphs.clear()
            self._enc_graph_version = ids

    def refresh_weights(self):
        v = sum(p._version for p in self._plist)
        if v == self.packed_version:
            return
        if self._packer is None:
            entries = []
            for c in self.mfma_convs:
                dmode = PTI_CONV_ZINS if c.mode == PTI_CONV_S2PAD else PTI_CONV_S1
                entries += [(c._w(), c.ksize, c.mode, False, c.f16), (c._w(), c.ksize, dmode, True, False)]
            rep, targets = [], []
            for c in self.direct_convs:
                c.alloc()
                rep += c.repack_entries()
                for attr, e in c.pack_entries():
                    targets.append((c, attr, len(entries)))
                    entries.append(e)
            self._direct_repack = ops.DirectRepack(rep)
            self._packer = ops.BatchedPacker(entries, self.dev)
            for i, c in enumerate(self.mfma_convs):
                c.wp, c.wpt = self._packer.outputs[2 * i], self._packer.outputs[2 * i + 1]
            for c, attr, i in targets:
                setattr(c, attr, self._packer.outputs[i])
        self._direct_repack.run()
        self._packer.run()
        self.packed_version = v
        self.pack_gen += 1

    def _qp(self, name):
        L = self.Lc
        w = self.net._param_by_name[name + ".conv.weight"].data.view(L, L)
        b = self.net._param_by_name[name + ".conv.bias"].data
        return w, b

    def _check_input(self, x, channels, what):
        if not x.is_cuda:
            raise RuntimeError(f"{what}: expected a cuda (HIP) tensor; the VAE hot path has no CPU fallback")
        if x.dim() != 4 or x.shape[1] != channels:
            raise ValueError(f"{what}: expected [B,{channels},H,W], got {tuple(x.shape)}")
        if x.dtype != F32:
            x = x.float()
        return x.contiguous()

    def _walk_fwd(self, layers, act, tail_needs_stats, save):
        for i, l in enumerate(layers):
            nxt_needs = layers[i + 1].needs_in_stats if i + 1 < len(layers) else tail_needs_stats
            act = l.fwd(act, self, nxt_needs, save)
        return act

    def _walk_bwd(self, layers, dout, saved):
        for l, s in zip(reversed(layers), reversed(saved)):
            dout = l.bwd(dout, s, self)
            self._ready(l.prefix)
        return dout

    @contextlib.contextmanager
    def side_stream(self, *operands):
        ws = self.wgrad_stream
        if ws is None:
            yield self.workspace
            return
        ev = torch.cuda.Event()
        ev.record(torch.cuda.current_stream())
        ws.wait_event(ev)
        self.record_side(*operands)
        with torch.cuda.stream(ws):
            yield self.workspace_side
        self._wgrad_pending = True

    def _wgrad_direct(self, wide, narrow, *args, **kw):
        with self.side_stream(wide, narrow, *args, *kw.values()) as workspace:
            ops.wgrad_direct(wide, narrow, *args, workspace=workspace, **kw)

    def record_side(self, *operands):
        ws = self.wgrad_stream
        owned = self._side_owned
        for t in operands:
            if isinstance(t, torch.Tensor) and t.untyped_storage().data_ptr() not in owned:
                t.record_stream(ws)

    def defer_wgrad(self, x, dy, dw, db, post=None, zero=()):
        if self._flush_up and self._wgrad_jobs:
            new, old = x.shape[1] * x.shape[2], self._wgrad_jobs[-1][0].shape[1] * self._wgrad_jobs[-1][0].shape[2]
            if new > old or (self._flush_up == 2 and new != old):
                self.flush_wgrad()
        self._wgrad_jobs.append((x, dy, dw, db))
        if post is not None:
            self._wgrad_posts.append(post)
        self._wgrad_zero += zero
        if len(self._wgrad_jobs) >= self.wgrad_batch_max:
            self.flush_wgrad()

    def wgrad_padded(self, x, dy, dw, db, post, zero):
        if self.batch_wgrad and ops.wgrad_batch_eligible(x, dy, 3, PTI_CONV_S1, PTI_PRO_NONE):
            self.defer_wgrad(x, dy, dw, db, post, zero)
            return
        with self.side_stream(x, dy, dw, db) as workspace:
            for t in zero:
                t.zero_()
            ops.conv_wgrad_mfma(x, dy, dw, db, accumulate=True, workspace=workspace)
            post()

    def flush_wgrad(self):
        jobs, self._wgrad_jobs = self._wgrad_jobs, []
        posts, self._wgrad_posts = self._wgrad_posts, []
        zero, self._wgrad_zero = self._wgrad_zero, ()
        if jobs:
            with self.side_stream(*(t for job in jobs for t in job)) as workspace:
                for t in zero:
                    t.zero_()
                ops.conv_wgrad_mfma_batched(jobs, workspace=workspace)
                for p in posts:
                    p()
        queue, self._ready_queue = self._ready_queue, []
        for rng in queue:
            self._emit_ready(rng)

    def join_wgrad(self):
        self.flush_wgrad()
        if self.wgrad_stream is not None and self._wgrad_pending:
            ev = torch.cuda.Event()
            ev.record(self.wgrad_stream)
            torch.cuda.current_stream().wait_event(ev)
            self._wgrad_pending = False

    def _ready(self, *prefixes):
        cb = self.grad_ready_cb
        if cb is None:
            return
        rng = self._range_cache.get(prefixes)
        if rng is None:
            lo, hi = None, None
            for name, (o, n, _) in self.net._slots.items():
                if name.startswith(prefixes):
                    lo = o if lo is None else min(lo, o)
                    hi = o + (n + 3) // 4 * 4 if hi is None else max(hi, o + (n + 3) // 4 * 4)
            rng = self._range_cache[prefixes] = (lo, hi)
        if rng[0] is None:
            return
        if self._wgrad_jobs or self._ready_queue:
            self._ready_queue.append(rng)
            if len(self._ready_queue) >= 6:
                self.flush_wgrad()
            return
        self._emit_ready(rng)

    def _emit_ready(self, rng):
        cb = self.grad_ready_cb
        if cb is None:
            return
        with self.side_stream():
            cb(*rng)

    def encode_forward(self, x, save):
        self.refresh_weights()
        x = self._check_input(x, self.net.in_channels, "encode")
        n, cin, h, w = x.shape
        down = 2 ** (len(self.net.channels) - 1)
        if h % down or w % down:
            raise ValueError(f"encode: H,W must be multiples of {down}, got {h}x{w}")
        self.begin_pass(n)
        c0 = self.net.channels[0]
        t0 = _empty((n, h, w, c0), x, self.act_dtype)
        xpad_b = None
        if self.enc_in.img_mfma:
            xpad, xpad_b = ops.pad_nchw_to_nhwc32(x, self.act_dtype, BF16 if (save and self.act_dtype != BF16) else None)
            if save and xpad_b is None:
                xpad_b = xpad
            st0 = self.new_stats(n)
            ops.conv_mfma(xpad, self.enc_in.wp_img, self.enc_in.b.data, t0, cout=c0, ksize=3, out_stats=st0, out_groups=self.G)
            a0 = _Act(t0, st0)
        else:
            ops.conv_direct(x, self.enc_in.w_tck, self.enc_in.b.data, t0, n=n, h=h, w=w, cin=cin, cout=c0, x_layout="nchw")
            a0 = _Act(t0, ops.gn_stats(t0, self.G, self.new_stats(n)))
        saved = [] if save else None
        act = self._walk_fwd(self.enc_layers, a0, True, saved)
        hl, wl, L = act.t.shape[1], act.t.shape[2], self.Lc
        nm = self.enc_out.norm
        if self.enc_out.mfma_narrow:
            ypad = _empty((n, hl, wl, 32), x, self.act_dtype)
            ops.conv_mfma(act.t, self.enc_out.wp_mfma, self.enc_out.bpad, ypad, cout=32, ksize=3, prologue=PTI_PRO_GN,
                          in_stats=act.stats, gamma=nm.weight.data, beta=nm.bias.data, groups=self.G, eps=self.eps)
            hlat = ypad.view(n, hl * wl, 32)[..., :L].float()
        else:
            hlat = _empty((n, hl * wl, L), x, F32)
            ops.conv_direct(act.t, self.enc_out.w_tck, self.enc_out.b.data, hlat.view(n, hl, wl, L), n=n, h=hl, w=wl,
                            cin=act.t.shape[3], cout=L, prologue=PTI_PRO_GN, in_stats=act.stats, gamma=nm.weight.data,
                            beta=nm.bias.data, groups=self.G, eps=self.eps)
        mu = _empty((n, L, hl, wl), x, F32)
        sigma = _empty((n, L, hl, wl), x, F32)
        zq_unused = _empty((n, hl * wl, L), x, F32)
        wm, bm = self._qp("quant_conv_mu")
        wl_, bl = self._qp("quant_conv_log_sigma")
        wp, bp = self._qp("post_quant_conv")
        ops.latent_head_fwd(hlat, None, wm, bm, wl_, bl, wp, bp, mu, sigma, None, zq_unused)
        ctx = (x, a0, saved, act, hlat, xpad_b) if save else None
        return mu, sigma, ctx

    def encode_backward(self, ctx, dmu, dsigma, want_dx=False):
        x, a0, saved, act, hlat, xpad_b = ctx
        net = self.net
        n, L = hlat.shape[0], self.Lc
        hl, wl = act.t.shape[1], act.t.shape[2]
        wm, bm = self._qp("quant_conv_mu")
        wl_, bl = self._qp("quant_conv_log_sigma")
        wp, bp = self._qp("post_quant_conv")
        self.begin_pass(n, backward=True)
        dh = torch.empty_like(hlat)
        gv = net.grad_view
        scratch = self.zeros(L * L + L)
        ops.latent_head_bwd(hlat, None, wm, bm, wl_, bl, wp, bp, None,
                            None if dmu is None else dmu.contiguous().float(),
                            None if dsigma is None else dsigma.contiguous().float(), dh,
                            gv("quant_conv_mu.conv.weight"), gv("quant_conv_mu.conv.bias"),
                            gv("quant_conv_log_sigma.conv.weight"), gv("quant_conv_log_sigma.conv.bias"),
                            scratch[:L * L], scratch[L * L:])
        self._ready("quant_conv_mu.", "quant_conv_log_sigma.")
        eo, nm = self.enc_out, self.enc_out.norm
        C = act.t.shape[3]
        self._wgrad_direct(act.t, dh.view(n, hl, wl, L), gv(eo.prefix + ".weight"), n=n, h=hl, w=wl, cw=C, cn=L, ksize=3,
                         sgn=1, narrow_layout="nhwc", dw_strides=(1, 9, C * 9), dbias_narrow=gv(eo.prefix + ".bias"),
                         prologue=PTI_PRO_GN, in_stats=act.stats, gamma=nm.weight.data, beta=nm.bias.data, groups=self.G,
                         eps=self.eps)
        da = _empty(act.t.shape, x)
        ops.conv_direct(dh.view(n, hl, wl, L), eo.w_tck_t, None, da, n=n, h=hl, w=wl, cin=L, cout=C)
        dout = nm.bwd(act, da, silu=False, dres=None, eng=self)
        self._ready(eo.prefix[:-4], nm.prefix + ".")
        dout = self._walk_bwd(self.enc_layers, dout, saved)
        ei = self.enc_in
        _, cin, h, w = x.shape
        c0 = dout.shape[3]
        if ei.img_mfma:
            dwp = ei.dw_img
            gw = gv(ei.prefix + ".weight")
            self.wgrad_padded(xpad_b, dout, dwp, gv(ei.prefix + ".bias"),
                              lambda: gw.view(c0, cin, 3, 3).add_(dwp[:, :cin]), (dwp,))
        else:
            self._wgrad_direct(dout, x, gv(ei.prefix + ".weight"), n=n, h=h, w=w, cw=c0, cn=cin, ksize=3, sgn=-1,
                               narrow_layout="nchw", dw_strides=(1, cin * 9, 9), dbias_wide=gv(ei.prefix + ".bias"))
        self._ready("encoder.blocks.0.")
        self.join_wgrad()
        if not want_dx:
            return None
        dx = torch.empty_like(x)
        ops.conv_direct(dout, ei.w_tck_t, None, dx, n=n, h=h, w=w, cin=c0, cout=cin, y_layout="nchw")
        return dx

    def decode_forward(self, z, save):
        self.refresh_weights()
        z = self._check_input(z, self.Lc, "decode")
        n, L, hl, wl = z.shape
        self.begin_pass(n)
        wp, bp = self._qp("post_quant_conv")
        zq = _empty((n, hl * wl, L), z, F32)
        ops.post_quant(z, wp, bp, zq)
        di = self.dec_in
        t0 = _empty((n, hl, wl, di.cout), z, self.act_dtype)
        ops.conv_direct(zq.view(n, hl, wl, L), di.w_tck, di.b.data, t0, n=n, h=hl, w=wl, cin=L, cout=di.cout)
        a0 = _Act(t0, ops.gn_stats(t0, self.G, self.new_stats(n)))
        saved = [] if save else None
        act = self._walk_fwd(self.dec_layers, a0, True, saved)
        h, w, C = act.t.shape[1], act.t.shape[2], act.t.shape[3]
        do, nm = self.dec_out, self.dec_out.norm
        recon = _empty((n, do.cout, h, w), z, F32)
        gact = None
        if do.img_mfma:
            ypad = _empty((n, h, w, 32), z, self.act_dtype)
            gact = _empty(act.t.shape, z) if save else None
            ops.conv_mfma(act.t, do.wp_img, do.bpad_img, ypad, cout=32, ksize=3, prologue=PTI_PRO_GN, in_stats=act.stats,
                          gamma=nm.weight.data, beta=nm.bias.data, groups=self.G, eps=self.eps, act_out=gact)
            ops.slice_nhwc32_to_nchw(ypad, do.cout, out=recon)
        else:
            ops.conv_direct(act.t, do.w_tck, do.b.data, recon, n=n, h=h, w=w, cin=C, cout=do.cout, y_layout="nchw",
                            prologue=PTI_PRO_GN, in_stats=act.stats, gamma=nm.weight.data, beta=nm.bias.data, groups=self.G,
                            eps=self.eps)
        ctx = (z, zq, a0, saved, act, gact) if save else None
        return recon, ctx

    def decode_backward(self, ctx, drecon, want_dz=True, join=True):
        z, zq, a0, saved, act, gact = ctx
        net, gv = self.net, self.net.grad_view
        n, L, hl, wl = z.shape
        self.begin_pass(n, backward=True)
        drecon = drecon.contiguous().float()
        do, nm = self.dec_out, self.dec_out.norm
        h, w, C = act.t.shape[1], act.t.shape[2], act.t.shape[3]
        co = do.cout
        da = _empty(act.t.shape, z)
        if do.img_mfma:
            dpad, _ = ops.pad_nchw_to_nhwc32(drecon, BF16)
            dwp, dbp = do.dw_img, do.db_img
            gw, gb = gv(do.prefix + ".weight"), gv(do.prefix + ".bias")

            def post():
                gw.view(co, C, 3, 3).add_(dwp[:co])
                gb.add_(dbp[:co])
            self.wgrad_padded(gact, dpad, dwp, dbp, post, (dwp, dbp))
            ops.conv_mfma(dpad, do.wpt_img, None, da, cout=C, ksize=3)
        else:
            self._wgrad_direct(act.t, drecon, gv(do.prefix + ".weight"), n=n, h=h, w=w, cw=C, cn=co, ksize=3, sgn=1,
                               narrow_layout="nchw", dw_strides=(1, 9, C * 9), dbias_narrow=gv(do.prefix + ".bias"),
                               prologue=PTI_PRO_GN, in_stats=act.stats, gamma=nm.weight.data, beta=nm.bias.data,
                               groups=self.G, eps=self.eps)
            ops.conv_direct(drecon, do.w_tck_t, None, da, n=n, h=h, w=w, cin=co, cout=C, x_layout="nchw")
        dout = nm.bwd(act, da, silu=False, dres=None, eng=self)
        self._ready(do.prefix[:-4], nm.prefix + ".")
        dout = self._walk_bwd(self.dec_layers, dout, saved)
        di = self.dec_in
        self._wgrad_direct(dout, zq.view(n, hl, wl, L), gv(di.prefix + ".weight"), n=n, h=hl, w=wl, cw=di.cout, cn=L,
                         ksize=3, sgn=-1, narrow_layout="nhwc", dw_strides=(1, L * 9, 9),
                         dbias_wide=gv(di.prefix + ".bias"))
        self._ready("decoder.blocks.0.")
        if di.mfma_narrow:
            dpad = _empty((n, hl, wl, 32), z)
            ops.conv_mfma(dout, di.wp_mfma, None, dpad, cout=32, ksize=3)
            dzq = dpad.view(n, hl * wl, 32)[..., :L].float()
        else:
            dzq = _empty((n, hl * wl, L), z, F32)
            ops.conv_direct(dout, di.w_tck_t, None, dzq.view(n, hl, wl, L), n=n, h=hl, w=wl, cin=di.cout, cout=L)
        wp, _ = self._qp("post_quant_conv")
        dz = torch.empty_like(z) if want_dz else None
        ops.post_quant_bwd(dzq, z, wp, dz, gv("post_quant_conv.conv.weight"), gv("post_quant_conv.conv.bias"))
        self._ready("post_quant_conv.")
        if join:
# ... 108 lines not shown
```

### pti_ldm_vae_amd/ops.py

```python
from __future__ import annotations

import ctypes as C
import os
from collections import namedtuple

import torch

from . import _lib as L
from ._lib import (PTI_CONV_S1, PTI_CONV_S2PAD, PTI_CONV_UP2, PTI_CONV_ZINS, PTI_PRO_GN, PTI_PRO_GN_SILU,
                   PTI_PRO_NONE, ConvDesc)

BF16 = torch.bfloat16
F16 = torch.float16
F32 = torch.float32
I64 = torch.int64
I32 = torch.int32
I16 = torch.int16
STAT_SCALE = 65536.0
ACT16 = (BF16, F16)
LATENT_BWD_MAX_BLOCKS = 512
VAE_LOSS_MAX_BLOCKS = 1024
POST_QUANT_BWD_MAX_BLOCKS = 256


_raw_stream = getattr(torch._C, "_cuda_getCurrentRawStream", None)
_cur_device = getattr(torch._C, "_cuda_getDevice", None)


def _stream() -> int:
    if _raw_stream is not None and _cur_device is not None:
        return _raw_stream(_cur_device())
    return torch.cuda.current_stream().cuda_stream


def _ptr(t):
    return None if t is None else C.c_void_p(t.data_ptr())


def _chk(t, dtype, name, dims=None):
    if not t.is_cuda:
        raise ValueError(f"{name}: expected a CUDA(HIP) tensor")
    if (t.dtype not in dtype) if isinstance(dtype, tuple) else (t.dtype != dtype):
        raise TypeError(f"{name}: expected {dtype}, got {t.dtype}")
    if not t.is_contiguous():
        raise ValueError(f"{name}: must be contiguous")
    if dims is not None and t.dim() != dims:
        raise ValueError(f"{name}: expected {dims} dims, got {tuple(t.shape)}")


def _out(out, shape, dtype, device, name, chk_name=None, rank=True, msg=None):
    if out is None:
        return torch.empty(shape, dtype=dtype, device=device)
    _chk(out, dtype, chk_name or name, len(shape) if rank else None)
    if tuple(out.shape) != tuple(shape) or out.device != device:
        raise ValueError(msg or f"{name} must be {list(shape)} on {device}")
    return out


_SCRATCH = {}


def _scratch(kind, shape, floats, device, stream):
    key = (kind, device.index, stream) + tuple(shape)
    ws = _SCRATCH.get(key)
    if ws is None:
        ws = _SCRATCH[key] = torch.empty(floats, dtype=F32, device=device)
    return ws


def conv_out_hw(h, w, mode):
    if mode == PTI_CONV_S1:
        return h, w
    if mode == PTI_CONV_S2PAD:
        return (h + 1 - 3) // 2 + 1, (w + 1 - 3) // 2 + 1
    return 2 * h, 2 * w


def pack_conv_weight(ws, ksize, mode=PTI_CONV_S1, flip=False, out=None, f16=False):
    ws = list(ws) if isinstance(ws, (list, tuple)) else [ws]
    w0 = ws[0]
    cout, cin = w0.shape[0], w0.shape[1]
    for w in ws:
        _chk(w, F32, "weight")
        if w.shape[0] != cout or w.shape[1] != cin or w.numel() != cout * cin * ksize * ksize:
            raise ValueError("pack_conv_weight: inconsistent weight shapes")
    nbytes = L.lib().pti_conv_packed_bytes(cout * len(ws), cin, ksize, mode)
    if nbytes == 0:
        raise ValueError(f"pack_conv_weight: unsupported cout={cout} cin={cin} k={ksize}")
    if out is None:
        out = torch.empty(nbytes // 2, dtype=F16 if f16 else BF16, device=w0.device)
    elif out.numel() * 2 != nbytes or out.dtype != (F16 if f16 else BF16):
        raise ValueError("pack_conv_weight: bad out size")
    arr = (C.c_void_p * len(ws))(*[w.data_ptr() for w in ws])
    L.check(L.lib().pti_conv_pack_weights(arr, len(ws), _ptr(out), cout, cin, ksize, mode, int(flip), int(f16), _stream()),
            "pti_conv_pack_weights")
    return out


class DirectRepack:

    def __init__(self, entries):
        if not 1 <= len(entries) <= L.DIRECT_REPACK_MAX:
            raise ValueError(f"DirectRepack: 1..{L.DIRECT_REPACK_MAX} entries")
        self.table = L.DirectRepackTable()
        self.table.n = len(entries)
        self._keep = entries
        for i, e in enumerate(entries):
            w = e["w"]
            _chk(w, F32, "w", 4)
            cout, cin = w.shape[0], w.shape[1]
            if w.shape[2] != 3 or w.shape[3] != 3:
                raise ValueError("DirectRepack: 3x3 weights")
            for k in ("b", "w_tck", "w_tck_t", "wpad", "bpad"):
                if e.get(k) is not None:
                    _chk(e[k], F32, k)
            wpad = e.get("wpad")
            pad_cin = 0
            if wpad is not None:
                pad_cin = wpad.shape[1]
                if wpad.dim() != 4 or wpad.shape[0] < cout or pad_cin < cin or wpad.shape[2:] != w.shape[2:]:
                    raise ValueError("DirectRepack: wpad shape")
            for k, size in (("w_tck", cout * cin * 9), ("w_tck_t", cout * cin * 9), ("bpad", cout)):
                if e.get(k) is not None and e[k].numel() < size:
                    raise ValueError(f"DirectRepack: {k} too small")
            if e.get("bpad") is not None and (e.get("b") is None or e["b"].numel() != cout):
                raise ValueError("DirectRepack: bpad needs b")
            self.table.e[i] = L.DirectRepackEntry(_ptr(w), _ptr(e.get("b")), _ptr(e.get("w_tck")), _ptr(e.get("w_tck_t")),
                                                  _ptr(wpad), _ptr(e.get("bpad")), cout, cin, pad_cin, 0)

    def run(self):
        L.check(L.lib().pti_direct_repack(C.byref(self.table), _stream()), "pti_direct_repack")


def _chk_stats(t, count, name):
    _chk(t, I64, name)
    if t.numel() != count:
        raise ValueError(f"{name}: expected {count} fixed-point sums, got {t.numel()}")


def _chk_prologue(who, in_stats, gamma, beta, n, groups, cin):
    _chk_stats(in_stats, n * groups * 2, "in_stats")
    for t, nm in ((gamma, "gamma"), (beta, "beta")):
        _chk(t, F32, nm)
        if t.numel() != cin:
            raise ValueError(f"{who}: {nm} size")


KERNEL_PROFILE = None
_MODE_NAME = {PTI_CONV_S1: "s1", PTI_CONV_S2PAD: "s2", PTI_CONV_UP2: "up2", PTI_CONV_ZINS: "zins"}


def last_kernel_name() -> str:
    name = (L.lib().pti_last_kernel_name() or b"").decode()
    name = name.replace("(anonymous namespace)::", "")
    if name.startswith("void "):
        name = name[5:]
    depth = 0
    for i, ch in enumerate(name):
        if ch == "<":
            depth += 1
        elif ch == ">":
            depth -= 1
        elif ch == "(" and depth == 0:
            return name[:i].strip()
    return name.strip()


def _prof_begin(prof):
    e0, e1 = (torch.cuda.Event(enable_timing=True) for _ in range(2))
    e0.record()
    return prof, e0, e1


def _prof_end(rec, flops, nbytes, shape):
    prof, e0, e1 = rec
    e1.record()
    prof.append((last_kernel_name(), flops, nbytes, e0, e1, shape))


def stats_to_float(stats):
    return stats.double() / STAT_SCALE


def gn_stats(x, groups, stats=None):
    _chk(x, ACT16, "x", 4)
    n, h, w, c = x.shape
    if stats is None:
        stats = torch.zeros(n, groups, 2, dtype=I64, device=x.device)
    else:
        _chk_stats(stats, n * groups * 2, "stats")
    L.check(L.lib().pti_gn_stats(_ptr(x), _ptr(stats), n, h * w, c, groups, int(x.dtype == F16), _stream()),
            "pti_gn_stats")
    return stats


def conv_mfma(x, w_packed, bias, y, *, cout, ksize=3, mode=PTI_CONV_S1, prologue=PTI_PRO_NONE, in_stats=None,
              gamma=None, beta=None, groups=0, eps=1e-6, residual=None, out_stats=None, out_groups=0, act_out=None,
              pool2=False, relu=False):
    _chk(x, ACT16, "x", 4)
    _chk(y, ACT16, "y", 4)
    n, h, w, cin = x.shape
    if act_out is not None:
        _chk(act_out, BF16, "act_out", 4)
        if act_out.shape != x.shape:
            raise ValueError("conv_mfma: act_out shape")
    ho, wo = conv_out_hw(h, w, mode)
    yshape = (n, ho // 2, wo // 2, cout) if pool2 else (n, ho, wo, cout)
    if tuple(y.shape) != yshape:
        raise ValueError(f"conv_mfma: y shape {tuple(y.shape)} != {yshape}")
    if w_packed.numel() != cout * cin * ksize * ksize or w_packed.dtype not in (BF16, F16):
        raise ValueError("conv_mfma: packed weight size/dtype mismatch")
    w_f16 = w_packed.dtype == F16
    if bias is not None:
        _chk(bias, F32, "bias")
        if bias.numel() != cout:
            raise ValueError("conv_mfma: bias size")
    if prologue != PTI_PRO_NONE:
        _chk_prologue("conv_mfma", in_stats, gamma, beta, n, groups, cin)
    if residual is not None:
        _chk(residual, ACT16, "residual", 4)
        if residual.shape != y.shape or pool2:
            raise ValueError("conv_mfma: residual shape")
    if out_stats is not None:
        _chk_stats(out_stats, n * out_groups * 2, "out_stats")
    d = ConvDesc(n=n, h=h, w=w, cin=cin, ho=ho, wo=wo, cout=cout, ksize=ksize, mode=mode, prologue=prologue,
                 groups=groups, add_residual=int(residual is not None), accum_stats=int(out_stats is not None),
                 out_groups=out_groups, eps=eps, in_f16=int(x.dtype == F16),
                 res_f16=int(residual is not None and residual.dtype == F16), out_f16=int(y.dtype == F16),
                 pool2x2_out=int(pool2), w_f16=int(w_f16), relu_out=int(relu))
    prof = KERNEL_PROFILE
    rec = None if prof is None else _prof_begin(prof)
    if act_out is not None:
        L.check(L.lib().pti_conv2d_mfma_saveact(_ptr(x), _ptr(w_packed), _ptr(bias), _ptr(in_stats), _ptr(gamma),
                                                _ptr(beta), _ptr(residual), _ptr(y), _ptr(out_stats), _ptr(act_out),
                                                C.byref(d), _stream()), "pti_conv2d_mfma_saveact")
    else:
        L.check(L.lib().pti_conv2d_mfma(_ptr(x), _ptr(w_packed), _ptr(bias), _ptr(in_stats), _ptr(gamma), _ptr(beta),
                                        _ptr(residual), _ptr(y), _ptr(out_stats), C.byref(d), _stream()),
                "pti_conv2d_mfma")
    if rec is not None:
        flops = 2.0 * n * ho * wo * cout * cin * ksize * ksize * (0.25 if mode == PTI_CONV_ZINS else 1.0)
        nbytes = 2.0 * (x.numel() * (2 if act_out is not None else 1) + y.numel() * (2 if residual is not None else 1))
        kind = "conv fwd" if x.dtype == F16 or prologue != PTI_PRO_NONE else "conv dgrad"
        _prof_end(rec, flops, nbytes, (kind, cin, cout, ho, wo, ksize, _MODE_NAME[mode], n))
    return y


def _strides4(t, layout):
    s = t.stride()
    return (s[0], s[2], s[3], s[1]) if layout == "nchw" else (s[0], s[1], s[2], s[3])


def conv_direct(x, w_tck, bias, y, *, n, h, w, cin, cout, ksize=3, x_layout="nhwc", y_layout="nhwc",
                prologue=PTI_PRO_NONE, in_stats=None, gamma=None, beta=None, groups=0, eps=1e-6):
    _chk(w_tck, F32, "w_tck")
    if w_tck.numel() != ksize * ksize * cin * cout:
        raise ValueError("conv_direct: weight size")
    if x.numel() != n * h * w * cin or y.numel() != n * h * w * cout:
        raise ValueError("conv_direct: tensor sizes do not match n,h,w,cin,cout")
    if prologue != PTI_PRO_NONE:
        _chk_stats(in_stats, n * groups * 2, "in_stats")
    d = ConvDesc(n=n, h=h, w=w, cin=cin, ho=h, wo=w, cout=cout, ksize=ksize, mode=PTI_CONV_S1, prologue=prologue,
                 groups=groups, eps=eps, in_f32=int(x.dtype == F32), out_f32=int(y.dtype == F32),
                 in_f16=int(x.dtype == F16), out_f16=int(y.dtype == F16))
    d.in_stride = (C.c_int64 * 4)(*_strides4(x, x_layout))
    d.out_stride = (C.c_int64 * 4)(*_strides4(y, y_layout))
    if cout % 32 == 0 and cin <= 16:
        if y.dtype not in ACT16 or not y.is_contiguous() or y_layout != "nhwc":
            raise ValueError("conv_direct: wide output must be dense NHWC bf16/fp16")
    else:
        if x.dtype not in ACT16 or not x.is_contiguous() or x_layout != "nhwc":
            raise ValueError("conv_direct: wide input must be dense NHWC bf16/fp16")
    L.check(L.lib().pti_conv2d_direct(_ptr(x), _ptr(w_tck), _ptr(bias), _ptr(in_stats), _ptr(gamma), _ptr(beta),
                                      _ptr(y), C.byref(d), _stream()), "pti_conv2d_direct")
    return y


def wgrad_direct(wide, narrow, dw, *, n, h, w, cw, cn, ksize, sgn, narrow_layout, dw_strides, dbias_wide=None,
                 dbias_narrow=None, prologue=PTI_PRO_NONE, in_stats=None, gamma=None, beta=None, groups=0, eps=1e-6,
                 workspace=None):
    _chk(wide, ACT16, "wide", 4)
    _chk(dw, F32, "dw")
    if prologue != PTI_PRO_NONE:
        _chk_stats(in_stats, n * groups * 2, "in_stats")
    ns = (C.c_int64 * 4)(*_strides4(narrow, narrow_layout))
    ws = workspace if workspace is not None else wgrad_workspace(wide.device)
    L.check(L.lib().pti_wgrad_direct(_ptr(wide), _ptr(narrow), _ptr(dw), _ptr(dbias_wide), _ptr(dbias_narrow),
                                     _ptr(in_stats), _ptr(gamma), _ptr(beta), n, h, w, cw, cn, ksize, sgn, prologue,
                                     groups, eps, int(narrow.dtype == F32), int(wide.dtype == F16), ns, dw_strides[0],
                                     dw_strides[1],
                                     dw_strides[2], _ptr(ws), ws.numel() * 4, _stream()), "pti_wgrad_direct")
    return dw


_WS = {}


def wgrad_workspace(device, nbytes=int(os.environ.get("PTI_WGRAD_WORKSPACE_MB", "256")) << 20):
    key = (device.index if device.index is not None else torch.cuda.current_device())
    ws = _WS.get(key)
    if ws is None or ws.numel() * 4 < nbytes:
        ws = torch.empty(nbytes // 4, dtype=F32, device=device)
        _WS[key] = ws
    return ws


def conv_wgrad_mfma(x, dy, dw, dbias, *, ksize=3, mode=PTI_CONV_S1, prologue=PTI_PRO_NONE, in_stats=None, gamma=None,
                    beta=None, groups=0, eps=1e-6, accumulate=False, workspace=None):
    _chk(x, ACT16, "x", 4)
    _chk(dy, BF16, "dy", 4)
    _chk(dw, F32, "dw")
    n, h, w, cin = x.shape
    ho, wo = conv_out_hw(h, w, mode)
    cout = dy.shape[3]
    if tuple(dy.shape) != (n, ho, wo, cout):
        raise ValueError(f"conv_wgrad_mfma: dy shape {tuple(dy.shape)} != {(n, ho, wo, cout)}")
    if dw.numel() != cout * cin * ksize * ksize:
        raise ValueError("conv_wgrad_mfma: dw size")
    if dbias is not None:
        _chk(dbias, F32, "dbias")
        if dbias.numel() != cout:
            raise ValueError("conv_wgrad_mfma: dbias size")
    if prologue != PTI_PRO_NONE:
        _chk_prologue("conv_wgrad_mfma", in_stats, gamma, beta, n, groups, cin)
    ws = workspace if workspace is not None else wgrad_workspace(x.device)
    d = ConvDesc(n=n, h=h, w=w, cin=cin, ho=ho, wo=wo, cout=cout, ksize=ksize, mode=mode, prologue=prologue,
                 groups=groups, eps=eps, in_f16=int(x.dtype == F16))
    prof = KERNEL_PROFILE
    if prof is None:
        L.check(L.lib().pti_conv_wgrad_mfma(_ptr(x), _ptr(dy), _ptr(in_stats), _ptr(gamma), _ptr(beta), _ptr(dw),
                                            _ptr(dbias), _ptr(ws), ws.numel() * 4, int(accumulate), C.byref(d),
                                            _stream()), "pti_conv_wgrad_mfma")
        return dw
    splits = C.c_int(0)
    rec = _prof_begin(prof)
    L.check(L.lib().pti_conv_wgrad_mfma_partials(_ptr(x), _ptr(dy), _ptr(in_stats), _ptr(gamma), _ptr(beta), _ptr(ws),
                                                 ws.numel() * 4, C.byref(d), C.byref(splits), _stream()),
            "pti_conv_wgrad_mfma_partials")
    _prof_end(rec, 2.0 * n * ho * wo * cout * cin * ksize * ksize, 2.0 * (x.numel() + dy.numel()),
              ("conv wgrad", cin, cout, ho, wo, ksize, _MODE_NAME[mode], n))
    L.check(L.lib().pti_conv_wgrad_reduce(_ptr(ws), splits.value, _ptr(dw), _ptr(dbias), int(accumulate), C.byref(d),
                                          _stream()), "pti_conv_wgrad_reduce")
    return dw


def wgrad_batch_eligible(x, dy, ksize, mode, prologue):
    return (ksize == 3 and mode == PTI_CONV_S1 and prologue == PTI_PRO_NONE and x.dtype == BF16 and dy.dtype == BF16
            and x.shape[3] % 32 == 0 and dy.shape[3] % 32 == 0 and x.numel() * 2 < (1 << 31) and dy.numel() * 2 < (1 << 31))


def conv_wgrad_mfma_batched(jobs, workspace=None, accumulate=True):
    if not 1 <= len(jobs) <= L.WGRAD_BATCH_MAX:
        raise ValueError(f"conv_wgrad_mfma_batched: 1..{L.WGRAD_BATCH_MAX} jobs, got {len(jobs)}")
    arr = (L.WgradJob * len(jobs))()
    for i, (x, dy, dw, db) in enumerate(jobs):
        _chk(x, BF16, "x", 4)
        _chk(dy, BF16, "dy", 4)
        _chk(dw, F32, "dw")
        n, h, w, cin = x.shape
        cout = dy.shape[3]
        if tuple(dy.shape) != (n, h, w, cout) or dw.numel() != cout * cin * 9 or (db is not None and db.numel() != cout):
            raise ValueError(f"conv_wgrad_mfma_batched: job {i}: shapes")
        if db is not None:
            _chk(db, F32, "dbias")
        arr[i] = L.WgradJob(x.data_ptr(), dy.data_ptr(), dw.data_ptr(), None if db is None else db.data_ptr(), n, h, w, cin,
                            cout, int(accumulate))
    ws = workspace if workspace is not None else wgrad_workspace(jobs[0][0].device)
    prof = KERNEL_PROFILE
    if prof is None:
        L.check(L.lib().pti_conv_wgrad_mfma_batched(arr, len(jobs), _ptr(ws), ws.numel() * 4, _stream()),
                "pti_conv_wgrad_mfma_batched")
        return
    groups = {}
    for i, j in enumerate(arr):
        groups.setdefault(L.lib().pti_conv_wgrad_batched_mode(j.n, j.h, j.w, j.cin, j.cout), []).append(i)
    for mode in sorted(groups, reverse=True):
        idx = groups[mode]
        sub = (L.WgradJob * len(idx))(*[arr[i] for i in idx])
        rec = _prof_begin(prof)
        L.check(L.lib().pti_conv_wgrad_mfma_batched(sub, len(idx), _ptr(ws), ws.numel() * 4, _stream()),
                "pti_conv_wgrad_mfma_batched")
        _prof_end(rec, sum(2.0 * arr[i].n * arr[i].h * arr[i].w * arr[i].cout * arr[i].cin * 9 for i in idx),
                  sum(2.0 * (jobs[i][0].numel() + jobs[i][1].numel()) for i in idx),
                  ("conv wgrad (batched)", 0, 0, 0, 0, 3, "s1", len(idx)))


def gn_bwd(x, da, dx, stats, gamma, beta, sums, dgamma, dbeta, *, groups, eps=1e-6, silu=True, dres=None):
    _chk(x, ACT16, "x", 4)
    _chk(da, BF16, "da", 4)
    _chk(dx, BF16, "dx", 4)
    n, h, w, c = x.shape
    if da.shape != x.shape or dx.shape != x.shape or (dres is not None and dres.shape != x.shape):
        raise ValueError("gn_bwd: shape mismatch")
    _chk_stats(stats, n * groups * 2, "stats")
    if sums.numel() != n * c * 2:
        raise ValueError("gn_bwd: scratch sizes")
    blocks = L.lib().pti_gn_bwd_blocks(n, h * w, c)
    if blocks <= 0:
        raise ValueError(f"gn_bwd: unsupported channel count {c}")
    part = torch.empty(n * blocks * c * 2, dtype=torch.float32, device=x.device)
    L.check(L.lib().pti_gn_bwd(_ptr(x), _ptr(da), _ptr(dres), _ptr(dx), _ptr(stats), _ptr(gamma), _ptr(beta),
                               _ptr(sums), _ptr(part), _ptr(dgamma), _ptr(dbeta), n, h * w, c, groups, eps, int(silu),
                               int(x.dtype == F16), _stream()), "pti_gn_bwd")
    return dx


def conv_mfma_gnbwd(dy_in, w_packed_t, gx, gstats, ggamma, gbeta, dy_out, gsums, *, cout, ksize=3, mode=PTI_CONV_S1,
                    groups=0, eps=1e-6, silu=True):
    _chk(dy_in, BF16, "dy_in", 4)
    _chk(gx, ACT16, "gx", 4)
    _chk(dy_out, BF16, "dy_out", 4)
    n, h, w, cin = dy_in.shape
    ho, wo = conv_out_hw(h, w, mode)
    if tuple(dy_out.shape) != (n, ho, wo, cout) or gx.shape != dy_out.shape:
        raise ValueError("conv_mfma_gnbwd: shapes")
    _chk_stats(gstats, n * groups * 2, "gstats")
    if gsums.numel() != n * cout * 2 or ggamma.numel() != cout:
        raise ValueError("conv_mfma_gnbwd: GroupNorm buffers")
    d = ConvDesc(n=n, h=h, w=w, cin=cin, ho=ho, wo=wo, cout=cout, ksize=ksize, mode=mode, groups=groups, eps=eps,
                 res_f16=int(gx.dtype == F16))
    tiles = L.lib().pti_conv_gnbwd_tiles(C.byref(d))
    if tiles <= 0:
        raise ValueError("conv_mfma_gnbwd: unsupported shape")
    part = torch.empty(n * tiles * cout * 2, dtype=torch.float32, device=dy_in.device)
    prof = KERNEL_PROFILE
    rec = None if prof is None else _prof_begin(prof)
    L.check(L.lib().pti_conv2d_mfma_gnbwd(_ptr(dy_in), _ptr(w_packed_t), _ptr(gx), _ptr(gstats), _ptr(ggamma),
                                          _ptr(gbeta), _ptr(dy_out), _ptr(part), C.byref(d), int(silu), _stream()),
            "pti_conv2d_mfma_gnbwd")
    if rec is not None:
        _prof_end(rec, 2.0 * n * ho * wo * cout * cin * ksize * ksize * (0.25 if mode == PTI_CONV_ZINS else 1.0),
                  2.0 * (dy_in.numel() + 2 * dy_out.numel()),
                  ("conv dgrad+GN bwd", cin, cout, ho, wo, ksize, "zins" if mode == PTI_CONV_ZINS else "s1", n))
    L.check(L.lib().pti_gn_sums_finalize(_ptr(part), _ptr(gsums), n, tiles, 2 * cout, _stream()), "pti_gn_sums_finalize")
    return dy_out


def gnbwd_chain_supported(cin, cout, ksize, x_dtype, groups=16):
    return (x_dtype == F16 and groups > 0 and cin % groups == 0 and cin // groups >= 8
            and bool(L.lib().pti_conv_gnbwd_chain_supported(int(cin), int(cout), int(ksize))))


def conv_mfma_gnbwd_chain(g_in, x_in, in_stats, in_gamma, in_sums, dx_in, w_packed_t, gx, gstats, ggamma, gbeta, dy_out, gsums,
                          *, cout, groups, eps=1e-6, silu=True, in_dgamma=None, in_dbeta=None):
    _chk(g_in, BF16, "g_in", 4)
    _chk(x_in, ACT16, "x_in", 4)
    _chk(dx_in, BF16, "dx_in", 4)
    _chk(gx, ACT16, "gx", 4)
    _chk(dy_out, BF16, "dy_out", 4)
    n, h, w, cin = g_in.shape
    if x_in.shape != g_in.shape or dx_in.shape != g_in.shape or tuple(dy_out.shape) != (n, h, w, cout) or gx.shape != dy_out.shape:
        raise ValueError("conv_mfma_gnbwd_chain: shapes")
    _chk_stats(in_stats, n * groups * 2, "in_stats")
    _chk_stats(gstats, n * groups * 2, "gstats")
    if in_sums.numel() != n * cin * 2 or gsums.numel() != n * cout * 2 or in_gamma.numel() != cin or ggamma.numel() != cout:
        raise ValueError("conv_mfma_gnbwd_chain: GroupNorm buffers")
    d = ConvDesc(n=n, h=h, w=w, cin=cin, ho=h, wo=w, cout=cout, ksize=3, mode=PTI_CONV_S1, groups=groups, eps=eps,
                 res_f16=int(gx.dtype == F16))
    tiles = L.lib().pti_conv_gnbwd_tiles(C.byref(d))
    if tiles <= 0:
        raise ValueError("conv_mfma_gnbwd_chain: unsupported shape")
    part = torch.empty(n * tiles * cout * 2, dtype=torch.float32, device=g_in.device)
    prof = KERNEL_PROFILE
    rec = None if prof is None else _prof_begin(prof)
    L.check(L.lib().pti_conv2d_mfma_gnbwd_chain(_ptr(g_in), _ptr(x_in), int(x_in.dtype == F16), _ptr(in_stats), _ptr(in_gamma),
                                                _ptr(in_sums), _ptr(dx_in), _ptr(w_packed_t), _ptr(gx), _ptr(gstats),
                                                _ptr(ggamma), _ptr(gbeta), _ptr(dy_out), _ptr(part), C.byref(d), int(silu),
                                                _stream()), "pti_conv2d_mfma_gnbwd_chain")
    if rec is not None:
        _prof_end(rec, 2.0 * n * h * w * cout * cin * 9, 2.0 * (3 * g_in.numel() + 2 * dy_out.numel()),
                  ("conv dgrad+GN bwd (chained)", cin, cout, h, w, 3, "s1", n))
    if in_dgamma is not None or in_dbeta is not None:
        L.check(L.lib().pti_gn_sums_finalize_affine(_ptr(part), _ptr(gsums), n, tiles, 2 * cout, _ptr(in_sums), _ptr(in_dgamma),
                                                    _ptr(in_dbeta), cin, _stream()), "pti_gn_sums_finalize_affine")
    else:
        L.check(L.lib().pti_gn_sums_finalize(_ptr(part), _ptr(gsums), n, tiles, 2 * cout, _stream()), "pti_gn_sums_finalize")
    return dy_out


def gn_affine_grads(sums, dgamma, dbeta, n, c):
    L.check(L.lib().pti_gn_affine_grads(_ptr(sums), _ptr(dgamma), _ptr(dbeta), int(n), int(c), _stream()), "pti_gn_affine_grads")


def gn_bwd_apply(x, dy, dx, stats, gamma, beta, sums, dgamma, dbeta, *, groups, eps=1e-6, dres=None):
    _chk(x, ACT16, "x", 4)
    _chk(dy, BF16, "dy", 4)
    _chk(dx, BF16, "dx", 4)
    n, h, w, c = x.shape
    if dy.shape != x.shape or dx.shape != x.shape or (dres is not None and dres.shape != x.shape):
        raise ValueError("gn_bwd_apply: shape mismatch")
    _chk_stats(stats, n * groups * 2, "stats")
    prof = KERNEL_PROFILE
    rec = None if prof is None else _prof_begin(prof)
    L.check(L.lib().pti_gn_bwd_apply(_ptr(x), _ptr(dy), _ptr(dres), _ptr(dx), _ptr(stats), _ptr(gamma), _ptr(beta),
                                     _ptr(sums), _ptr(dgamma), _ptr(dbeta), n, h * w, c, groups, eps,
                                     int(x.dtype == F16), _stream()), "pti_gn_bwd_apply")
    if rec is not None:
        _prof_end(rec, 8.0 * x.numel(), 2.0 * x.numel() * (4 if dres is not None else 3),
                  ("GroupNorm bwd apply", c, c, h, w, 0, "-", n))
    return dx


def pool2x2_sum(x, y):
    _chk(x, BF16, "x", 4)
    _chk(y, BF16, "y", 4)
    n, h2, w2, c = x.shape
    if tuple(y.shape) != (n, h2 // 2, w2 // 2, c) or h2 % 2 or w2 % 2:
        raise ValueError("pool2x2_sum: shapes")
    L.check(L.lib().pti_pool2x2_sum(_ptr(x), _ptr(y), n, h2 // 2, w2 // 2, c, _stream()), "pti_pool2x2_sum")
    return y


def latent_head_fwd(h, eps, wm, bm, wl, bl, wp, bp, mu, sigma, logvar, zq):
    b, hw, l = h.shape
    for t, nm in ((h, "h"), (wm, "wm"), (bm, "bm"), (wl, "wl"), (bl, "bl"), (wp, "wp"), (bp, "bp"), (mu, "mu"),
                  (sigma, "sigma"), (zq, "zq")):
        _chk(t, F32, nm)
    if mu.numel() != b * hw * l or sigma.numel() != b * hw * l or zq.numel() != b * hw * l:
        raise ValueError("latent_head_fwd: output sizes")
    if eps is not None and (eps.numel() != b * hw * l or eps.dtype != F32 or not eps.is_contiguous()):
        raise ValueError("latent_head_fwd: eps must be contiguous fp32 of the latent shape")
    L.check(L.lib().pti_latent_head_fwd(_ptr(h), _ptr(eps), _ptr(wm), _ptr(bm), _ptr(wl), _ptr(bl), _ptr(wp), _ptr(bp),
                                        _ptr(mu), _ptr(sigma), _ptr(logvar), _ptr(zq), b, hw, l, _stream()),
            "pti_latent_head_fwd")


def post_quant(z_nchw, wp, bp, zq):
    b, l = z_nchw.shape[0], z_nchw.shape[1]
    hw = z_nchw.numel() // (b * l)
    _chk(z_nchw, F32, "z")
    L.check(L.lib().pti_post_quant(_ptr(z_nchw), _ptr(wp), _ptr(bp), _ptr(zq), b, hw, l, _stream()), "pti_post_quant")


def post_quant_bwd(dzq, z_nchw, wp, dz, gwp, gbp):
    b, l = z_nchw.shape[0], z_nchw.shape[1]
    hw = z_nchw.numel() // (b * l)
    _chk(dzq, F32, "dzq")
    _chk(z_nchw, F32, "z")
    if dzq.numel() != z_nchw.numel() or (dz is not None and dz.numel() != z_nchw.numel()):
        raise ValueError("post_quant_bwd: sizes")
    ws = torch.empty(POST_QUANT_BWD_MAX_BLOCKS * (l * l + l), dtype=torch.float32, device=dzq.device)
    L.check(L.lib().pti_post_quant_bwd(_ptr(dzq), _ptr(z_nchw), _ptr(wp), _ptr(dz), _ptr(gwp), _ptr(gbp), _ptr(ws), b, hw, l,
                                       _stream()), "pti_post_quant_bwd")


def latent_head_bwd(h, eps, wm, bm, wl, bl, wp, bp, dzq, dmu, dsigma, dh, gwm, gbm, gwl, gbl, gwp, gbp):
    b, hw, l = h.shape
    for t in (dzq, dmu, dsigma):
        if t is not None and (t.dtype != F32 or not t.is_contiguous() or t.numel() != b * hw * l):
            raise ValueError("latent_head_bwd: gradient inputs must be contiguous fp32 of the latent size")
    ws = torch.empty(LATENT_BWD_MAX_BLOCKS * 3 * (l * l + l), dtype=torch.float32, device=h.device)
    L.check(L.lib().pti_latent_head_bwd(_ptr(h), _ptr(eps), _ptr(wm), _ptr(bm), _ptr(wl), _ptr(bl), _ptr(wp), _ptr(bp),
                                        _ptr(dzq), _ptr(dmu), _ptr(dsigma), _ptr(dh), _ptr(gwm), _ptr(gbm), _ptr(gwl),
                                        _ptr(gbl), _ptr(gwp), _ptr(gbp), _ptr(ws), b, hw, l, _stream()),
            "pti_latent_head_bwd")


def vae_loss(recon, images, mu, third, out2, d_recon, d_mu, d_third, *, l2=False, third_mode=0, kl_weight=1e-3):
    for t, nm in ((recon, "recon"), (images, "images"), (mu, "mu"), (third, "third"), (out2, "out2")):
        _chk(t, F32, nm)
    if recon.shape != images.shape or mu.shape != third.shape or out2.numel() < 2:
        raise ValueError("vae_loss: shapes")
    ws = torch.empty(2 * VAE_LOSS_MAX_BLOCKS, dtype=torch.float32, device=recon.device)
    L.check(L.lib().pti_vae_loss(_ptr(recon), _ptr(images), recon.numel(), _ptr(mu), _ptr(third), mu.numel(),
                                 recon.shape[0], _ptr(out2), _ptr(d_recon), _ptr(d_mu), _ptr(d_third), _ptr(ws), int(l2),
                                 third_mode, kl_weight, _stream()), "pti_vae_loss")


def ar_vae_loss(mu, attrs, channels, deltas, per_attr, counts, *, gamma=0.0, d_mu=None, pair_mask=None):
    _chk(mu, F32, "mu", 4)
    _chk(attrs, F32, "attrs", 2)
    _chk(deltas, F32, "deltas")
    _chk(per_attr, F32, "per_attr")
    b, l, h, w = mu.shape
    na = attrs.shape[0]
    if attrs.shape[1] != b or channels.numel() != na or deltas.numel() != na or per_attr.numel() != na or counts.numel() != na:
        raise ValueError("ar_vae_loss: attrs must be [na, b]; channels / deltas / per_attr / counts [na]")
    if channels.dtype != torch.int32 or counts.dtype != torch.int32 or not (channels.is_cuda and counts.is_cuda):
        raise TypeError("ar_vae_loss: channels / counts must be int32 device tensors")
    if d_mu is not None:
        _chk(d_mu, F32, "d_mu", 4)
        if d_mu.shape != mu.shape:
            raise ValueError("ar_vae_loss: d_mu shape")
    if pair_mask is not None:
        if pair_mask.dtype != torch.uint8 or tuple(pair_mask.shape) != (na, b, b) or not pair_mask.is_cuda or not pair_mask.is_contiguous():
            raise ValueError("ar_vae_loss: pair_mask must be a contiguous uint8 device tensor [na, b, b]")
    L.check(L.lib().pti_ar_vae_loss(_ptr(mu), b, l, h * w, _ptr(attrs), _ptr(channels), _ptr(deltas), na, _ptr(pair_mask),
                                    float(gamma), _ptr(per_attr), _ptr(counts), _ptr(d_mu), _stream()), "pti_ar_vae_loss")


def adam_step(p, g, m, v, *, lr, beta1=0.9, beta2=0.999, eps=1e-8, step=1, grad_scale=1.0):
    for t, nm in ((p, "p"), (g, "g"), (m, "m"), (v, "v")):
        _chk(t, F32, nm)
        if t.numel() != p.numel():
            raise ValueError("adam_step: size mismatch")
    L.check(L.lib().pti_adam_step(_ptr(p), _ptr(g), _ptr(m), _ptr(v), p.numel(), lr, beta1, beta2, eps, step,
                                  grad_scale, _stream()), "pti_adam_step")


def cast_nchw_f32_to_nhwc_bf16(x, y):
    n, c = x.shape[0], x.shape[1]
    _chk(x, F32, "x")
    _chk(y, BF16, "y")
    L.check(L.lib().pti_cast_nchw_f32_to_nhwc_bf16(_ptr(x), _ptr(y), n, c, x.numel() // (n * c), _stream()), "cast")
    return y


def cast_nhwc_bf16_to_nchw_f32(x, y):
    n, c = y.shape[0], y.shape[1]
    _chk(x, BF16, "x")
    _chk(y, F32, "y")
    L.check(L.lib().pti_cast_nhwc_bf16_to_nchw_f32(_ptr(x), _ptr(y), n, c, y.numel() // (n * c), _stream()), "cast")
    return y


def attention_fwd(qkv, o, lse2):
    _chk(qkv, BF16, "qkv", 3)
    _chk(o, BF16, "o", 3)
    _chk(lse2, F32, "lse2")
    b, l, c3 = qkv.shape
    c = c3 // 3
    if tuple(o.shape) != (b, l, c) or lse2.numel() != b * l or c3 != 3 * c:
        raise ValueError("attention_fwd: shapes")
    L.check(L.lib().pti_attention_fwd(_ptr(qkv), _ptr(o), _ptr(lse2), b, l, c, _stream()), "pti_attention_fwd")
    return o


def attention_bwd(qkv, o, dout, lse2, delta, dqkv):
    _chk(qkv, BF16, "qkv", 3)
    _chk(o, BF16, "o", 3)
    _chk(dout, BF16, "dout", 3)
    _chk(dqkv, BF16, "dqkv", 3)
    b, l, c3 = qkv.shape
    c = c3 // 3
    if o.shape != dout.shape or tuple(o.shape) != (b, l, c) or dqkv.shape != qkv.shape:
        raise ValueError("attention_bwd: shapes")
    if lse2.numel() != b * l or delta.numel() != b * l:
        raise ValueError("attention_bwd: lse/delta sizes")
    L.check(L.lib().pti_attention_bwd(_ptr(qkv), _ptr(o), _ptr(dout), _ptr(lse2), _ptr(delta), _ptr(dqkv), b, l, c,
                                      _stream()), "pti_attention_bwd")
    return dqkv


class BatchedPacker:

    def __init__(self, entries, device):
        lib = L.lib()
        esz = lib.pti_conv_pack_entry_bytes()
        host = bytearray(esz * len(entries))
        hbuf = (C.c_char * len(host)).from_buffer(host)
        first, total, self.outputs = [], 0, []
        for i, (w, ksize, mode, flip, *rest) in enumerate(entries):
            f16 = bool(rest[0]) if rest else False
            _chk(w, F32, "weight")
            cout, cin = w.shape[0], w.shape[1]
            out = torch.empty(w.numel(), dtype=F16 if f16 else BF16, device=device)
            nb = C.c_int64(0)
            L.check(lib.pti_conv_pack_table_fill(C.byref(hbuf, i * esz), _ptr(w), _ptr(out), cout, cin, ksize, mode,
                                                 int(flip), int(f16), C.byref(nb)), "pti_conv_pack_table_fill")
            first.append(total)
            total += nb.value
            self.outputs.append(out)
        self.n, self.total_blocks = len(entries), total
        self.table = torch.frombuffer(host, dtype=torch.uint8).clone().to(device)
        self.first = torch.tensor(first, dtype=torch.int32, device=device)
        self._keep = [e[0] for e in entries]

    def run(self):
        L.check(L.lib().pti_conv_pack_weights_batched(_ptr(self.table), _ptr(self.first), self.n, self.total_blocks,
                                                      _stream()), "pti_conv_pack_weights_batched")


def preprocess_batch(src, offsets, hw, out, stats=None):
    _chk(src, F32, "src")
    _chk(out, F32, "out", 4)
    b, _, hp, wp = out.shape
    if offsets.dtype != torch.int64 or hw.dtype != torch.int32 or offsets.numel() != b or hw.numel() != 2 * b:
        raise ValueError("preprocess_batch: offsets must be int64 [B], hw int32 [B,2]")
    if not (offsets.is_cuda and hw.is_cuda and offsets.is_contiguous() and hw.is_contiguous()):
        raise ValueError("preprocess_batch: descriptor tables must be contiguous device tensors")
    if stats is None:
        stats = torch.empty(3 * b, dtype=torch.float64, device=out.device)
    L.check(L.lib().pti_preprocess_batch(_ptr(src), _ptr(offsets), _ptr(hw), b, hp, wp, _ptr(out), _ptr(stats), _stream()),
            "pti_preprocess_batch")
    return out


def _tensor(t, dtype, name, dims=None):
    if not isinstance(t, torch.Tensor):
        raise ValueError(f"{name}: expected a CUDA(HIP) tensor")
    _chk(t, dtype, name, dims)


def _dense_rows(t, name, dtype=F32, *, square=False, copy=False):
    if not isinstance(t, torch.Tensor) or not t.is_cuda:
        raise ValueError(f"{name}: expected a CUDA(HIP) tensor")
    if copy and not t.is_floating_point():
        raise TypeError(f"{name}: expected a floating-point matrix, got {t.dtype}")
    if not copy and t.dtype != dtype:
        raise TypeError(f"{name}: expected {dtype}, got {t.dtype}")
    want = (f"{name}: expected {'a square [n, n]' if square else 'an [m, n]'} matrix {'that is not empty' if copy else 'with dense rows'}, "
            f"got {tuple(t.shape)}")
    if t.dim() != 2 or (square and t.shape[0] != t.shape[1]) or (copy and 0 in t.shape):
        raise ValueError(want)
    if copy and t.dtype != dtype:
        t = t.to(dtype)
    if t.stride(1) != 1 or t.stride(0) < t.shape[1]:
        if not copy:
            raise ValueError(want)
        t = t.contiguous()
    return t


def _rows_out(out, shape, dtype, device, name):
    if out is None:
        return torch.empty(shape, dtype=dtype, device=device)
    _dense_rows(out, f"{name}: out", dtype)
    if tuple(out.shape) != tuple(shape) or out.device != device:
        raise ValueError(f"{name}: out must be {list(shape)} on {device}")
    return out


def _outs(who, out, names):
    if out is None:
        return (None,) * len(names)
    if len(out) != len(names):
        raise ValueError(f"{who}: out must be ({', '.join(names)})")
    return tuple(out)


def _scratch_bytes(who, kind, shape, nbytes, what, device, stream):
    if nbytes <= 0:
        raise ValueError(f"{who}: unsupported shape {what}")
    ws = _scratch(kind, shape, (nbytes + 3) // 4, device, stream)
    return ws, ws.numel() * 4


def _offsets(who, name, seg, device, what, host=False):
    if not isinstance(seg, torch.Tensor) or (seg.device != device and (seg.is_cuda or not host)):
        raise ValueError(f"{who}: {name} must be a CUDA(HIP) tensor on {device}")
    if seg.dtype != I32:
        raise TypeError(f"{who}: {name} must be int32, got {seg.dtype}")
    if seg.dim() != 1 or seg.numel() < 2 or not seg.is_contiguous():
        raise ValueError(f"{who}: {name} must be a contiguous vector of {what} + 1 offsets")


def _latent_attrs(who, z, attrs):
    for name, t in (("z", z), ("attrs", attrs)):
        if not isinstance(t, torch.Tensor) or not t.is_cuda:
            raise ValueError(f"{who}: {name}: expected a CUDA(HIP) tensor")
        if not t.is_floating_point():
            raise TypeError(f"{who}: {name}: expected a floating-point matrix, got {t.dtype}")
        if t.dim() != 2:
            raise ValueError(f"{who}: {name}: expected a matrix, got {tuple(t.shape)}")
    n, l = z.shape
    na = attrs.shape[0]
    if attrs.shape[1] != n or attrs.device != z.device:
        raise ValueError(f"{who}: z {tuple(z.shape)} needs attrs [na, {n}] on {z.device}, got {tuple(attrs.shape)} on {attrs.device}")
    zt, attrs = _dense_rows(z.t(), f"{who}: z", copy=True), _dense_rows(attrs, f"{who}: attrs", copy=True)
    return zt, attrs, n, l, na, (zt.stride(0) if l > 1 else n), (attrs.stride(0) if na > 1 else n)
SSIM_WINDOW, SSIM_SIGMA = 11, 1.5
_ssim_taps = None


def ssim_taps() -> torch.Tensor:
    global _ssim_taps
    if _ssim_taps is None:
        coords = torch.arange(SSIM_WINDOW) - SSIM_WINDOW // 2
        g = torch.exp(-(coords ** 2) / (2 * SSIM_SIGMA * SSIM_SIGMA))
        _ssim_taps = (g / g.sum()).to(F32).contiguous()
    return _ssim_taps


def image_metrics(pred, target, *, clamp=None, data_range=1.0, k1=0.01, k2=0.03, out=None):
    if not (pred.is_cuda and target.is_cuda):
        raise ValueError("image_metrics: expected CUDA(HIP) tensors")
    if pred.dim() != 4 or pred.shape != target.shape:
        raise ValueError(f"image_metrics: expected two [n, c, h, w] tensors of one shape, got {tuple(pred.shape)} / {tuple(target.shape)}")
    if not (pred.is_floating_point() and target.is_floating_point()):
        raise TypeError("image_metrics: expected floating-point images")
    pred, target = pred.to(F32).contiguous(), target.to(F32).contiguous()
    n, c, h, w = pred.shape
    floats = L.lib().pti_image_metrics_ws_floats(n, c, h, w)
    if floats <= 0:
        raise ValueError(f"image_metrics: unsupported shape {tuple(pred.shape)}")
    out = _out(out, (n, 4), F32, pred.device, "image_metrics: out", chk_name="out")
    stream = _stream()
    ws = _scratch("metrics", (n, c, h, w), floats, pred.device, stream)
    lo, hi = (0.0, 0.0) if clamp is None else (float(clamp[0]), float(clamp[1]))
    L.check(L.lib().pti_image_metrics(_ptr(pred), _ptr(target), n, c, h, w, int(clamp is not None), lo, hi, float(data_range),
                                      float(k1), float(k2), C.c_void_p(ssim_taps().data_ptr()), _ptr(out), _ptr(ws), stream),
            "pti_image_metrics")
    return out


def latent_pairwise(a, b=None, *, mode="dist", center=None, out=None):
    if mode not in ("dist", "dot"):
        raise ValueError(f"latent_pairwise: mode must be 'dist' or 'dot', got {mode!r}")
    a = _dense_rows(a, "latent_pairwise: a", copy=True)
    b = a if b is None else _dense_rows(b, "latent_pairwise: b", copy=True)
    if b.shape[1] != a.shape[1] or b.device != a.device:
        raise ValueError(f"latent_pairwise: a {tuple(a.shape)} and b {tuple(b.shape)} must share columns and device")
    n1, d = a.shape
    n2 = b.shape[0]
    if center is not None:
        if not isinstance(center, torch.Tensor) or not center.is_cuda:
            raise ValueError("latent_pairwise: center must be a CUDA(HIP) tensor")
        if not center.is_floating_point():
            raise TypeError("latent_pairwise: center must be floating-point")
        if center.numel() != d or center.device != a.device:
            raise ValueError(f"latent_pairwise: center must hold {d} values on {a.device}")
        center = center.reshape(-1).to(F32).contiguous()
    floats = L.lib().pti_latent_pairwise_ws_floats(n1, n2, d)
    if floats <= 0:
        raise ValueError(f"latent_pairwise: unsupported shape a {tuple(a.shape)} b {tuple(b.shape)}")
    out = _rows_out(out, (n1, n2), F32, a.device, "latent_pairwise")
    stream = _stream()
    ws = _scratch("pair", (n1, n2, d), floats, a.device, stream)
    L.check(L.lib().pti_latent_pairwise(_ptr(a), a.stride(0), n1, _ptr(b), b.stride(0), n2, d, _ptr(center),
                                        int(mode == "dot"), _ptr(out), out.stride(0), _ptr(ws), stream), "pti_latent_pairwise")
    return out


def latent_group_stats(a, seg_a, b, seg_b, *, out=None):
    a = _dense_rows(a, "latent_group_stats: a", copy=True)
    b = _dense_rows(b, "latent_group_stats: b", copy=True)
    if b.shape[1] != a.shape[1] or b.device != a.device:
        raise ValueError(f"latent_group_stats: a {tuple(a.shape)} and b {tuple(b.shape)} must share columns and device")
    _offsets("latent_group_stats", "seg_a", seg_a, a.device, "patients")
    _offsets("latent_group_stats", "seg_b", seg_b, a.device, "patients")
    if seg_a.numel() != seg_b.numel():
        raise ValueError("latent_group_stats: seg_a and seg_b must describe the same patients")
    e = seg_a.numel() - 1
    (n1, d), n2 = a.shape, b.shape[0]
    floats = L.lib().pti_latent_group_stats_ws_floats(n1, n2, e, d)
    if floats <= 0:
        raise ValueError(f"latent_group_stats: unsupported shape a {tuple(a.shape)} b {tuple(b.shape)} patients {e}")
    out = _rows_out(out, (e, 4), F32, a.device, "latent_group_stats")
    if out.stride(0) != 4:
        raise ValueError("latent_group_stats: out must be contiguous")
    stream = _stream()
    ws = _scratch("group", (n1, n2, e, d), floats, a.device, stream)
    L.check(L.lib().pti_latent_group_stats(_ptr(a), a.stride(0), n1, _ptr(seg_a), _ptr(b), b.stride(0), n2, _ptr(seg_b), e, d,
                                           _ptr(out), _ptr(ws), stream), "pti_latent_group_stats")
    return out


def tsne_affinities(d2, perplexity, *, out=None):
    d2 = _dense_rows(d2, "tsne_affinities: d2", square=True)
    n = d2.shape[0]
    perplexity = float(perplexity)
    if not 0.0 < perplexity < n:
        raise ValueError(f"tsne_affinities: perplexity ({perplexity:g}) must be positive and < n ({n})")
    floats = L.lib().pti_tsne_affinities_ws_floats(n)
    if floats <= 0:
        raise ValueError(f"tsne_affinities: unsupported shape {tuple(d2.shape)} (2 <= n <= 8192)")
    out = _rows_out(out, (n, n), F32, d2.device, "tsne_affinities")
    if out.data_ptr() == d2.data_ptr():
        raise ValueError("tsne_affinities: out must not be d2")
    sums = torch.empty(2, dtype=torch.float64, device=d2.device)
    stream = _stream()
    ws = _scratch("tsne_aff", (n,), floats, d2.device, stream)
    L.check(L.lib().pti_tsne_affinities(_ptr(d2), d2.stride(0), n, perplexity, _ptr(out), out.stride(0), _ptr(sums), _ptr(ws),
                                        stream), "pti_tsne_affinities")
    return out, sums


def tsne_step(p, y_in, y_out, update, gains, record, *, sums, exaggeration, momentum, lr, with_record=True):
    p = _dense_rows(p, "tsne_step: p", square=True)
    n = p.shape[0]
    for name, t in (("y_in", y_in), ("y_out", y_out), ("update", update), ("gains", gains)):
        _tensor(t, F32, f"tsne_step: {name}", 2)
        if t.shape[0] != n or t.device != p.device:
            raise ValueError(f"tsne_step: {name} must be [{n}, 2] on {p.device}, got {tuple(t.shape)}")
        if t.shape[1] != 2:
            raise ValueError(f"tsne_step: {name} has {t.shape[1]} columns; only n_components = 2 is built")
    for name, t in (("record", record), ("sums", sums)):
        _tensor(t, torch.float64, f"tsne_step: {name}", 1)
        if t.numel() != 2 or t.device != p.device:
            raise ValueError(f"tsne_step: {name} must hold 2 doubles on {p.device}")
    if y_in.data_ptr() == y_out.data_ptr():
        raise ValueError("tsne_step: y_out must not be y_in")
    floats = L.lib().pti_tsne_step_ws_floats(n, 2)
    if floats <= 0:
        raise ValueError(f"tsne_step: unsupported shape {tuple(p.shape)} (2 <= n <= 8192)")
    stream = _stream()
    ws = _scratch("tsne_step", (n,), floats, p.device, stream)
    L.check(L.lib().pti_tsne_step(_ptr(p), p.stride(0), n, 2, _ptr(y_in), _ptr(y_out), _ptr(update), _ptr(gains), _ptr(sums),
                                  float(exaggeration), float(momentum), float(lr), _ptr(record), int(bool(with_record)),
                                  _ptr(ws), stream), "pti_tsne_step")


UmapGraph = namedtuple("UmapGraph", "indptr indices weights rate rho sigma nnz")
UmapGraph.__doc__ = """The fuzzy graph of ``umap_graph`` as device CSR: ``indptr`` int32 [n + 1]; ``indices`` int32 (ascending
within a row), ``weights`` fp32 and ``rate`` int32, allocated for min(2 n k, n^2) entries of which the first ``nnz`` are
written; ``rho`` / ``sigma`` fp32 [n]; ``nnz`` = ``indptr[n]``, a 0-d DEVICE tensor (reading it is a host sync)."""


def umap_knn(dist, k, *, out=None):
    idx, kd = _outs("umap_knn", out, ("knn_idx", "knn_dist"))
    dist = _dense_rows(dist, "umap_knn: dist", square=True)
    n, k = dist.shape[0], int(k)
    if not (3 <= n <= 8192 and 2 <= k <= 256 and k < n):
        raise ValueError(f"umap_knn: unsupported shape {tuple(dist.shape)} with k={k} (3 <= n <= 8192, 2 <= k <= 256, k < n)")
    idx = _out(idx, (n, k), I32, dist.device, "umap_knn: knn_idx")
    kd = _out(kd, (n, k), F32, dist.device, "umap_knn: knn_dist")
    L.check(L.lib().pti_umap_knn(_ptr(dist), dist.stride(0), n, k, _ptr(idx), _ptr(kd), _stream()), "pti_umap_knn")
    return idx, kd


def umap_graph(knn_idx, knn_dist, n_epochs):
    for name, t, dtype in (("knn_idx", knn_idx, I32), ("knn_dist", knn_dist, F32)):
        _tensor(t, dtype, f"umap_graph: {name}", 2)
    n, k = knn_idx.shape
    if tuple(knn_dist.shape) != (n, k) or knn_dist.device != knn_idx.device:
        raise ValueError(f"umap_graph: knn_dist must be [{n}, {k}] on {knn_idx.device}, got {tuple(knn_dist.shape)}")
    n_epochs = int(n_epochs)
    floats, cap = L.lib().pti_umap_graph_ws_floats(n, k), L.lib().pti_umap_graph_capacity(n, k)
    if floats <= 0 or not 1 <= n_epochs <= 2000:
        raise ValueError(f"umap_graph: unsupported shape {tuple(knn_idx.shape)} with n_epochs={n_epochs} "
                         f"(3 <= n <= 8192, 2 <= k <= 256, k < n, 1 <= n_epochs <= 2000)")
    dev = knn_idx.device
    indptr = torch.empty(n + 1, dtype=I32, device=dev)
    indices, rate = torch.empty(cap, dtype=I32, device=dev), torch.empty(cap, dtype=I32, device=dev)
    weights = torch.empty(cap, dtype=F32, device=dev)
    rho, sigma = torch.empty(n, dtype=F32, device=dev), torch.empty(n, dtype=F32, device=dev)
    stream = _stream()
    ws = _scratch("umap_graph", (n, k), floats, dev, stream)
    L.check(L.lib().pti_umap_graph(_ptr(knn_idx), _ptr(knn_dist), n, k, n_epochs, _ptr(indptr), _ptr(indices), _ptr(weights),
                                   _ptr(rate), cap, _ptr(rho), _ptr(sigma), _ptr(ws), stream), "pti_umap_graph")
    return UmapGraph(indptr, indices, weights, rate, rho, sigma, indptr[n])


def umap_epoch(graph, y_in, y_out, *, a, b, alpha, epoch, seed, negative_sample_rate=5):
    for name, t, dtype in (("indptr", graph.indptr, I32), ("indices", graph.indices, I32), ("rate", graph.rate, I32),
                           ("y_in", y_in, F32), ("y_out", y_out, F32)):
        _tensor(t, dtype, f"umap_epoch: {name}", 2 if name[0] == "y" else 1)
    n = graph.indptr.numel() - 1
    if not 3 <= n <= 8192:
        raise ValueError(f"umap_epoch: unsupported shape: {n} rows (3 <= n <= 8192)")
    cap = graph.indices.numel()
    if graph.rate.numel() != cap or cap > n * n:
        raise ValueError(f"umap_epoch: indices ({cap}) and rate ({graph.rate.numel()}) must have one length of at most n^2")
    for name, t in (("y_in", y_in), ("y_out", y_out)):
        if t.shape[0] != n or t.device != graph.indptr.device:
            raise ValueError(f"umap_epoch: {name} must be [{n}, 2] on {graph.indptr.device}, got {tuple(t.shape)}")
        if t.shape[1] != 2:
            raise ValueError(f"umap_epoch: {name} has {t.shape[1]} columns; only n_components = 2 is built")
    if y_in.data_ptr() == y_out.data_ptr():
        raise ValueError("umap_epoch: y_out must not be y_in")
    L.check(L.lib().pti_umap_epoch(_ptr(graph.indptr), _ptr(graph.indices), _ptr(graph.rate), cap, n, 2, _ptr(y_in), _ptr(y_out),
                                   float(a), float(b), float(alpha), int(epoch), int(seed) & 0xFFFFFFFF,
                                   int(negative_sample_rate), _stream()), "pti_umap_epoch")


UmapTransformGraph = namedtuple("UmapTransformGraph", "indices weights rate sigma y0")
UmapTransformGraph.__doc__ = """What ``umap_transform_graph`` makes of m new rows' k nearest training rows, a regular device slab:
``indices`` int32 [m, k] (the ``knn_idx`` it was given), ``weights`` fp32 [m, k], ``rate`` int32 [m, k] (0 = dropped),
``sigma`` fp32 [m] and the start points ``y0`` fp32 [m, 2]."""


def _umap_cross_shape(who, m, n, k):
# ... 1017 lines not shown
```

Before: 2749 images/s.

## Add polyphase 2x2-tap conv kernels for upsample and stride-2 resample convs

Adds a polyphase MFMA convolution kernel and weight packer. They rewrite the nearest-upsample 3x3 conv (forward and dgrad) and the stride-2 conv routes as four 2x2-tap phase convolutions using pre-summed weights. This avoids redundant MACs on duplicated upsampled pixels and the zero-inserted taps in stride-2 dgrad. It adds extra packed weight buffers, and the routes are selected through an env knob that defaults on. The new indexing paths carry correctness risk.

Measured after the change: 2751 images/s (median of 3 runs). About the same (+0.1%).

```diff
diff --git a/include/pti_vae.h b/include/pti_vae.h
--- a/include/pti_vae.h
+++ b/include/pti_vae.h
@@ -20,6 +20,13 @@
 #define PTI_CONV_S2PAD 1
 #define PTI_CONV_UP2 2
 #define PTI_CONV_ZINS 3
+#define PTI_CONV_PHASE_OUT 4
+#define PTI_CONV_PHASE_IN 5
+
+#define PTI_POLY_UP2_FWD 0
+#define PTI_POLY_UP2_DGRAD 1
+#define PTI_POLY_S2_FWD 2
+#define PTI_POLY_S2_DGRAD 3
 
 #define PTI_PRO_NONE 0
 #define PTI_PRO_GN 1
@@ -59,6 +66,12 @@
                              int cin, int ksize, int mode, int transpose_flip, int w_f16, int64_t* nblocks);
 int pti_conv_pack_weights_batched(const void* table_dev, const int* blk_first_dev, int n,
                                   int total_blocks, pti_stream_t s);
+
+int64_t pti_conv_poly_packed_bytes(int cout, int cin);
+int pti_conv_pack_weights_poly(const float* w_oihw, void* packed, int cout, int cin, int kind, int w_f16,
+                               pti_stream_t s);
+int pti_conv_pack_table_fill_poly(void* host_entry, const float* w_oihw_dev, void* packed_dev, int cout,
+                                  int cin, int kind, int w_f16, int64_t* nblocks);
 
 int pti_gn_stats(const void* x_nhwc_16bit, int64_t* stats, int n, int hw, int c, int groups,
                  int x_f16, pti_stream_t s);
diff --git a/pti_ldm_vae_amd/_lib.py b/pti_ldm_vae_amd/_lib.py
--- a/pti_ldm_vae_amd/_lib.py
+++ b/pti_ldm_vae_amd/_lib.py
@@ -19,6 +19,8 @@
 
 ABI_VERSION = 5
 PTI_CONV_S1, PTI_CONV_S2PAD, PTI_CONV_UP2, PTI_CONV_ZINS = 0, 1, 2, 3
+PTI_CONV_PHASE_OUT, PTI_CONV_PHASE_IN = 4, 5
+PTI_POLY_UP2_FWD, PTI_POLY_UP2_DGRAD, PTI_POLY_S2_FWD, PTI_POLY_S2_DGRAD = 0, 1, 2, 3
 PTI_PRO_NONE, PTI_PRO_GN, PTI_PRO_GN_SILU = 0, 1, 2
 
 
@@ -80,6 +82,9 @@
     "pti_conv_pack_entry_bytes": (_I, []),
     "pti_conv_pack_table_fill": (_I, [_P, _P, _P, _I, _I, _I, _I, _I, _I, C.POINTER(_I64)]),
     "pti_conv_pack_weights_batched": (_I, [_P, _P, _I, _I, _P]),
+    "pti_conv_poly_packed_bytes": (_I64, [_I, _I]),
+    "pti_conv_pack_weights_poly": (_I, [_P, _P, _I, _I, _I, _I, _P]),
+    "pti_conv_pack_table_fill_poly": (_I, [_P, _P, _P, _I, _I, _I, _I, C.POINTER(_I64)]),
     "pti_gn_stats": (_I, [_P, _P, _I, _I, _I, _I, _I, _P]),
     "pti_conv2d_mfma": (_I, [_P, _P, _P, _P, _P, _P, _P, _P, _P, C.POINTER(ConvDesc), _P]),
     "pti_conv2d_mfma_saveact": (_I, [_P, _P, _P, _P, _P, _P, _P, _P, _P, _P, C.POINTER(ConvDesc), _P]),
diff --git a/pti_ldm_vae_amd/csrc/conv_mfma.hip b/pti_ldm_vae_amd/csrc/conv_mfma.hip
--- a/pti_ldm_vae_amd/csrc/conv_mfma.hip
+++ b/pti_ldm_vae_amd/csrc/conv_mfma.hip
@@ -800,6 +800,281 @@
   return launch2_cfg<KS, 32, 32, 2>(a, st);
 }
 
+template <int CK, int CT, int PXF, int GEO>
+struct CfgP {
+  using B = Cfg2<3, CK, CT, PXF>;
+  static constexpr int WN = B::WN, WM = B::WM, TH2 = B::TH2, TW2 = B::TW2;
+  static constexpr int HH = TH2 + (GEO == 0 ? 2 : 1), HW = TW2 + (GEO == 0 ? 2 : 1);
+  static constexpr int NP = HH * HW;
+  static constexpr int NC = B::NC, PIXB = B::PIXB, NT = B::NT, KPC = B::KPC, KEY_SHIFT = B::KEY_SHIFT;
+  static constexpr int KBC = 4 * KPC;
+  static constexpr int R = PXF == 4 ? 8 : 4;
+  static constexpr int NG = KBC / R;
+  static constexpr int HALO_BYTES = NP * PIXB;
+  static constexpr int HITERS = (NP * NC + 255) / 256;
+  static constexpr int MPX = B::MPX, ENC = B::ENC, EITERS = B::EITERS;
+  static constexpr int ESH = ENC == 16 ? 0 : (ENC == 8 ? 1 : 2);
+  static constexpr int EPI_BYTES = MPX * CT * 2;
+  static constexpr int EPI_OFF = GEO == 0 ? HALO_BYTES : 0;
+  static constexpr int STAT_OFF = GEO == 0 ? HALO_BYTES + EPI_BYTES : (HALO_BYTES > EPI_BYTES ? HALO_BYTES : EPI_BYTES);
+  static constexpr int BIAS_OFF = STAT_OFF + 1024;
+  static constexpr int LDS_BYTES = BIAS_OFF + 4 * CT;
+  static_assert(NG == 1 || NG % 2 == 0, "weight ring");
+  static_assert(LDS_BYTES * B::WGS_PER_CU <= 160 * 1024, "LDS per CU");
+};
+
+template <int CK, int CT, int PXF, int GEO, bool OPH>
+__global__ __launch_bounds__(256, (PXF == 2 ? 4 : 2)) void conv_mfma2_poly_kernel(ConvArgs a) {
+  using C = CfgP<CK, CT, PXF, GEO>;
+  if (OPH) fp16_saturate_on();
+  __shared__ __attribute__((aligned(16))) unsigned char smem[C::LDS_BYTES];
+  unsigned char* halo = smem;
+  unsigned char* etile = smem + C::EPI_OFF;
+  const int tid = threadIdx.x, lane = tid & 63, wave = tid >> 6;
+  const int hsel = lane >> 5, j = lane & 31, txl = lane & 15;
+  int t = blockIdx.x;
+  const int tile_x = t % a.tiles_x;
+  t /= a.tiles_x;
+  const int tile_y = t % a.tiles_y;
+  const int n = t / a.tiles_y;
+  const int oy0 = tile_y * C::TH2, ox0 = tile_x * C::TW2;
+  const int SH = GEO == 0 ? a.H : a.Ho, SW = GEO == 0 ? a.W : a.Wo;
+  const int ct = blockIdx.y;
+  const int nchunks = a.Cin / CK;
+  const int wm = wave / C::WN, wn = wave % C::WN;
+  const int pbase0 = ((2 * PXF * wm + (j >> 4)) * C::HW + txl) * C::PIXB;
+
+  f32x16 acc[PXF];
+#pragma unroll
+  for (int i = 0; i < PXF; ++i)
+#pragma unroll
+    for (int r = 0; r < 16; ++r) acc[i][r] = 0.f;
+
+  const int lc = tid % C::NC, lp0 = tid / C::NC;
+  constexpr int PSTEP = 256 / C::NC;
+  reinterpret_cast<float*>(smem + C::STAT_OFF)[tid] = 0.f;
+  if (a.bias) {
+    if (tid < CT) reinterpret_cast<float*>(smem + C::BIAS_OFF)[tid] = a.bias[ct * CT + tid];
+  }
+  const int epc = tid % C::ENC, epp0 = tid / C::ENC;
+  constexpr int EPSTEP = 256 / C::ENC;
+  const bool do_stats = a.out_stats != nullptr;
+  const int ocpg = do_stats ? a.Cout / a.out_groups : 1;
+  const __amdgpu_buffer_rsrc_t xrs = __builtin_amdgcn_make_buffer_rsrc(
+      const_cast<bf16*>(a.x), 0, (unsigned)a.N * (unsigned)a.H * (unsigned)a.W * (unsigned)a.Cin * 2u, 0x00020000);
+  const __amdgpu_buffer_rsrc_t yrs = __builtin_amdgcn_make_buffer_rsrc(
+      a.y, 0, (unsigned)a.N * (unsigned)a.Ho * (unsigned)a.Wo * (unsigned)a.Cout * 2u, 0x00020000);
+
+  const unsigned char* wct = a.w + (size_t)ct * nchunks * 4 * C::KBC * C::NT * 1024 + wn * 1024 + lane * 16;
+  const int kb_last = nchunks * 4 * C::KBC - 1;
+  bf16x8 wa[C::R], wb[C::R];
+  auto wload = [&](bf16x8 (&dst)[C::R], int kb0) {
+#pragma unroll
+    for (int u = 0; u < C::R; ++u) {
+      int kb = kb0 + u;
+      kb = kb < kb_last ? kb : kb_last;
+      dst[u] = *(const bf16x8*)(wct + (size_t)kb * C::NT * 1024);
+    }
+  };
+
+  const int nitems = 4 * nchunks;
+#pragma clang loop unroll(disable)
+  for (int q = 0; q < nitems; ++q) {
+    const int cls = GEO == 0 ? q / nchunks : (q & 3);
+    const int chunk = GEO == 0 ? q - cls * nchunks : (q >> 2);
+    const int ca = cls >> 1, cb = cls & 1;
+    const int wkb0 = (chunk * 4 + cls) * C::KBC;
+    if (q == 0 || C::NG == 1 || (GEO == 0 && nchunks > 1)) wload(wa, wkb0);
+
+    if (GEO == 1 || nchunks > 1 || q == 0) {
+      u32x4 raw[C::HITERS];
+      const unsigned base = ((unsigned)n * a.H * a.W * a.Cin + chunk * CK + lc * 8) * 2u;
+      const unsigned rowb = (unsigned)a.W * a.Cin * 2u, pixb = (unsigned)a.Cin * 2u;
+#pragma unroll
+      for (int it = 0; it < C::HITERS; ++it) {
+        const int p = lp0 + it * PSTEP;
+        const int hy = p / C::HW, hx = p - hy * C::HW;
+        int sy, sx, iy, ix;
+        if (GEO == 0) {
+          sy = oy0 - 1 + hy; sx = ox0 - 1 + hx;
+          iy = sy; ix = sx;
+        } else {
+          sy = oy0 - ca + hy; sx = ox0 - cb + hx;
+          iy = 2 * sy + ca; ix = 2 * sx + cb;
+        }
+        const bool v = (p < C::NP) && (unsigned)sy < (unsigned)SH && (unsigned)sx < (unsigned)SW;
+        const unsigned off = v ? base + (unsigned)iy * rowb + (unsigned)ix * pixb : 0x80000000u;
+        raw[it] = __builtin_bit_cast(u32x4, __builtin_amdgcn_raw_buffer_load_b128(xrs, off, 0, 0));
+      }
+      if (q > 0) __syncthreads();
+#pragma unroll
+      for (int it = 0; it < C::HITERS; ++it) {
+        const int p = lp0 + it * PSTEP;
+        if (p < C::NP) {
+          const int hy = p / C::HW, hx = p - hy * C::HW;
+          const int key = (hx >> C::KEY_SHIFT) & (C::NC - 1);
+          *(u32x4*)(halo + p * C::PIXB + ((lc ^ key) << 4)) = raw[it];
+        }
+      }
+      __syncthreads();
+    }
+
+    auto baddr = [&](int kb) -> const unsigned char* {
+      kb = kb < C::KBC ? kb : C::KBC - 1;
+      const int tap = kb / C::KPC, kc = kb - tap * C::KPC;
+      const int tr = tap >> 1, ts = tap & 1;
+      const int dy = GEO == 0 ? ca + tr : 1 - tr, dx = GEO == 0 ? cb + ts : 1 - ts;
+      const int hx = txl + dx;
+      const int tk = (hsel ^ ((hx >> C::KEY_SHIFT) & (C::NC - 1))) << 4;
+      return halo + pbase0 + (dy * C::HW + dx) * C::PIXB + ((kc * 32) ^ tk);
+    };
+    bf16x8 b0[PXF], b1[PXF];
+    auto bread = [&](bf16x8 (&dst)[PXF], int kb) {
+      const unsigned char* bp = baddr(kb);
+#pragma unroll
+      for (int i = 0; i < PXF; ++i) dst[i] = *(const bf16x8*)(bp + 2 * i * C::HW * C::PIXB);
+    };
+    auto group = [&](const bf16x8 (&w)[C::R], int g) {
+      const int kb0 = g * C::R;
+#pragma unroll
+      for (int u = 0; u < C::R; ++u) {
+        if ((u & 1) == 0) {
+          bread(b1, kb0 + u + 1);
+#pragma unroll
+          for (int i = 0; i < PXF; ++i) acc[i] = mfma32<OPH>(w[u], b0[i], acc[i]);
+        } else {
+          bread(b0, kb0 + u + 1);
+#pragma unroll
+          for (int i = 0; i < PXF; ++i) acc[i] = mfma32<OPH>(w[u], b1[i], acc[i]);
+        }
+      }
+    };
+    bread(b0, 0);
+    if constexpr (C::NG == 1) {
+      group(wa, 0);
+    } else {
+#pragma clang loop unroll(disable)
+      for (int g = 0; g < C::NG; g += 2) {
+        wload(wb, wkb0 + (g + 1) * C::R);
+        group(wa, g);
+        wload(wa, wkb0 + (g + 2) * C::R);
+        group(wb, g + 1);
+      }
+    }
+
+    if (GEO == 0 ? chunk == nchunks - 1 : q == nitems - 1) {
+      __syncthreads();
+      const int col0 = wn * 32 + 4 * hsel;
+      float st1[4] = {0.f, 0.f, 0.f, 0.f}, st2[4] = {0.f, 0.f, 0.f, 0.f};
+      float su1[4] = {0.f, 0.f, 0.f, 0.f}, su2[4] = {0.f, 0.f, 0.f, 0.f};
+#pragma unroll
+      for (int i = 0; i < PXF; ++i) {
+        const int p = (2 * PXF * wm + 2 * i + (j >> 4)) * 16 + (j & 15);
+        const bool inb = (oy0 + (p >> 4) < SH) && (ox0 + (p & 15) < SW);
+#pragma unroll
+        for (int qd = 0; qd < 4; ++qd) {
+          const int col = col0 + 8 * qd;
+          float v0 = acc[i][4 * qd + 0], v1 = acc[i][4 * qd + 1], v2 = acc[i][4 * qd + 2], v3 = acc[i][4 * qd + 3];
+          if (a.bias) {
+            const f32x4 b = *(const f32x4*)(smem + C::BIAS_OFF + col * 4);
+            v0 += b[0]; v1 += b[1]; v2 += b[2]; v3 += b[3];
+          }
+          const u32x2 packed = pack4f(v0, v1, v2, v3, OPH);
+          *(u32x2*)(etile + p * (CT * 2) + ((((col >> 3) ^ (p >> C::ESH)) & (C::ENC - 1)) << 4) + (col & 7) * 2) = packed;
+          if (do_stats && inb) {
+            float r0, r1, r2, r3;
+            unpack2f(packed[0], OPH, r0, r1);
+            unpack2f(packed[1], OPH, r2, r3);
+            if (ocpg >= 4) {
+              st1[qd] += (r0 + r1) + (r2 + r3);
+              st2[qd] += (r0 * r0 + r1 * r1) + (r2 * r2 + r3 * r3);
+            } else {
+              st1[qd] += r0 + r1; st2[qd] += r0 * r0 + r1 * r1;
+              su1[qd] += r2 + r3; su2[qd] += r2 * r2 + r3 * r3;
+            }
+          }
+        }
+#pragma unroll
+        for (int r = 0; r < 16; ++r) acc[i][r] = 0.f;
+      }
+      if (do_stats) {
+        stat_t* sstat = reinterpret_cast<stat_t*>(smem + C::STAT_OFF);
+        if (ocpg >= 4) {
+          float v[8];
+#pragma unroll
+          for (int qd = 0; qd < 4; ++qd) { v[2 * qd] = st1[qd]; v[2 * qd + 1] = st2[qd]; }
+          fold32<8>(v, j);
+          if ((j & 3) == 0) {
+            const int idx = j >> 2, qd = idx >> 1;
+            const int g = (ct * CT + col0 + 8 * qd) / ocpg;
+            stat_add(&sstat[2 * g + (idx & 1)], v[0]);
+          }
+        } else {
+          float v[16];
+#pragma unroll
+          for (int qd = 0; qd < 4; ++qd) { v[4 * qd] = st1[qd]; v[4 * qd + 1] = st2[qd]; v[4 * qd + 2] = su1[qd]; v[4 * qd + 3] = su2[qd]; }
+          fold32<16>(v, j);
+          if ((j & 1) == 0) {
+            const int idx = j >> 1, qd = idx >> 2;
+            const int g = (ct * CT + col0 + 8 * qd) / 2;
+            stat_add(&sstat[2 * g + (idx & 3)], v[0]);
+          }
+        }
+      }
+      __syncthreads();
+#pragma unroll
+      for (int it = 0; it < C::EITERS; ++it) {
+        const int p = epp0 + it * EPSTEP;
+        const int sy = oy0 + (p >> 4), sx = ox0 + (p & 15);
+        if (sy < SH && sx < SW) {
+          const int oy = GEO == 0 ? 2 * sy + ca : sy, ox = GEO == 0 ? 2 * sx + cb : sx;
+          __builtin_amdgcn_raw_buffer_store_b128(
+              __builtin_bit_cast(bu32x4, *(const u32x4*)(etile + p * (CT * 2) + (((epc ^ (p >> C::ESH)) & (C::ENC - 1)) << 4))), yrs,
+              ((unsigned)((n * a.Ho + oy) * a.Wo + ox) * a.Cout + ct * CT + epc * 8) * 2u, 0, 2);
+        }
+      }
+    }
+  }
+  if (do_stats) {
+    __syncthreads();
+    const stat_t* sstat = reinterpret_cast<const stat_t*>(smem + C::STAT_OFF);
+    const int g0 = (ct * CT) / ocpg, ng = CT / ocpg;
+    if (tid < 2 * ng)
+      atomicAdd((unsigned long long*)&a.out_stats[(n * a.out_groups + g0) * 2 + tid], (unsigned long long)sstat[2 * g0 + tid]);
+  }
+}
+
+template <int CK, int CT, int PXF>
+int launch_poly_cfg(ConvArgs a, hipStream_t st) {
+  using C = CfgP<CK, CT, PXF, 0>;
+  const bool out = a.mode == PTI_CONV_PHASE_OUT;
+  a.tiles_x = cdiv(out ? a.W : a.Wo, C::TW2);
+  a.tiles_y = cdiv(out ? a.H : a.Ho, C::TH2);
+  dim3 grid(a.N * a.tiles_x * a.tiles_y, a.Cout / CT);
+  const bool f16 = a.w_f16 && a.in_f16 && a.out_f16, b16 = !a.w_f16 && !a.in_f16 && !a.out_f16;
+  if (!f16 && !b16) return 5;
+  if (out) {
+    if (f16) PTI_LAUNCH((conv_mfma2_poly_kernel<CK, CT, PXF, 0, true>), grid, dim3(256), 0, st, a);
+    else PTI_LAUNCH((conv_mfma2_poly_kernel<CK, CT, PXF, 0, false>), grid, dim3(256), 0, st, a);
+  } else {
+    if (f16) PTI_LAUNCH((conv_mfma2_poly_kernel<CK, CT, PXF, 1, true>), grid, dim3(256), 0, st, a);
+    else PTI_LAUNCH((conv_mfma2_poly_kernel<CK, CT, PXF, 1, false>), grid, dim3(256), 0, st, a);
+  }
+  return 0;
+}
+int launch_poly(const ConvArgs& a, int ck, int ct, hipStream_t st) {
+  if (ct == 128) {
+    if (ck == 128) return launch_poly_cfg<128, 128, 4>(a, st);
+    if (ck == 64) return launch_poly_cfg<64, 128, 4>(a, st);
+    return launch_poly_cfg<32, 128, 4>(a, st);
+  }
+  if (ct == 64) {
+    if (ck == 64) return launch_poly_cfg<64, 64, 2>(a, st);
+    return launch_poly_cfg<32, 64, 2>(a, st);
+  }
+  return launch_poly_cfg<32, 32, 2>(a, st);
+}
+
 struct PackArgs {
   const float* src[4];
   int nsrc;
@@ -809,6 +1084,7 @@
   int ks, ck, cout_tile, flip;
   int f16;
   long long total;
+  int poly;
 };
 
 __device__ __forceinline__ void pack_eight(const PackArgs& p, int e8) {
@@ -839,10 +1115,54 @@
   *(u32x4*)(p.dst + (size_t)e8 * 8) = p.f16 ? pack8f(f, true) : pack8(f);
 }
 
+__device__ __forceinline__ void pack_eight_poly(const PackArgs& p, int e8) {
+  const int NT = p.cout_tile / 32, KPC = p.ck / 16, KBT = 16 * KPC, nch = p.cin_l / p.ck;
+  int r_ = e8;
+  const int lane = r_ % 64; r_ /= 64;
+  const int nt = r_ % NT; r_ /= NT;
+  const int kb = r_ % KBT; r_ /= KBT;
+  const int chunk = r_ % nch;
+  const int ct = r_ / nch;
+  const int co = ct * p.cout_tile + nt * 32 + (lane & 31);
+  const int cls = kb / (4 * KPC), tap = (kb / KPC) & 3, kc = kb % KPC;
+  const int ci0 = chunk * p.ck + kc * 16 + 8 * (lane >> 5);
+  const int a = cls >> 1, b = cls & 1, r = tap >> 1, s = tap & 1;
+  int kh0, kh1, kw0, kw1;
+  if (p.poly - 1 == PTI_POLY_UP2_FWD || p.poly - 1 == PTI_POLY_UP2_DGRAD) {
+    kh0 = a == 0 ? (r == 0 ? 0 : 1) : (r == 0 ? 0 : 2); kh1 = a == 0 ? (r == 0 ? 0 : 2) : (r == 0 ? 1 : 2);
+    kw0 = b == 0 ? (s == 0 ? 0 : 1) : (s == 0 ? 0 : 2); kw1 = b == 0 ? (s == 0 ? 0 : 2) : (s == 0 ? 1 : 2);
+  } else {
+    const int uh = a == 0 ? (r == 0 ? 2 : 0) : (r == 0 ? 1 : -1), uw = b == 0 ? (s == 0 ? 2 : 0) : (s == 0 ? 1 : -1);
+    kh0 = kh1 = uh; kw0 = kw1 = uw;
+    if (uh < 0 || uw < 0) { kh0 = kw0 = 0; kh1 = kw1 = -1; }
+  }
+  const float* src;
+  size_t stride;
+  if (!p.flip) {
+    src = p.src[0] + ((size_t)co * p.cin_o + ci0) * 9;
+    stride = 9;
+  } else {
+    src = p.src[0] + ((size_t)ci0 * p.cin_o + co) * 9;
+    stride = (size_t)p.cin_o * 9;
+  }
+  float f[8];
+#pragma unroll
+  for (int j = 0; j < 8; ++j) {
+    float acc = 0.f;
+    for (int kh = kh0; kh <= kh1; ++kh)
+      for (int kw = kw0; kw <= kw1; ++kw) acc += src[j * stride + kh * 3 + kw];
+    f[j] = acc;
+  }
+  *(u32x4*)(p.dst + (size_t)e8 * 8) = p.f16 ? pack8f(f, true) : pack8(f);
+}
+
 __global__ void pack_weights_kernel(PackArgs p) {
   if (p.f16) fp16_saturate_on();
   const long long e8 = (long long)blockIdx.x * blockDim.x + threadIdx.x;
-  if (e8 * 8 < p.total) pack_eight(p, (int)e8);
+  if (e8 * 8 < p.total) {
+    if (p.poly) pack_eight_poly(p, (int)e8);
+    else pack_eight(p, (int)e8);
+  }
 }
 
 __global__ void pack_weights_batched_kernel(const PackArgs* __restrict__ table, const int* __restrict__ blk_first, int n) {
@@ -855,7 +1175,10 @@
   const PackArgs p = table[lo];
   if (p.f16) fp16_saturate_on();
   const int e8 = (b - blk_first[lo]) * 256 + threadIdx.x;
-  if ((long long)e8 * 8 < p.total) pack_eight(p, e8);
+  if ((long long)e8 * 8 < p.total) {
+    if (p.poly) pack_eight_poly(p, e8);
+    else pack_eight(p, e8);
+  }
 }
 
 template <int KS, int S, int CK, int COUT_TILE>
@@ -909,6 +1232,7 @@
   p.ks = ksize;
   p.flip = transpose_flip;
   p.f16 = w_f16 ? 1 : 0;
+  p.poly = 0;
   p.cout_tile = pick_cout_tile(p.cout_l);
   p.ck = (mode == PTI_CONV_S2PAD) ? pick_ck(p.cin_l, true) : pick_ck2(p.cin_l, p.cout_tile);
   p.total = (long long)p.cout_l * p.cin_l * ksize * ksize;
@@ -927,7 +1251,7 @@
   p.cout_o = cout; p.cin_o = cin;
   p.cout_l = flip ? cin : cout;
   p.cin_l = flip ? cout : cin;
-  p.ks = ksize; p.flip = flip; p.f16 = f16 ? 1 : 0;
+  p.ks = ksize; p.flip = flip; p.f16 = f16 ? 1 : 0; p.poly = 0;
   p.cout_tile = pick_cout_tile(p.cout_l);
   p.ck = (mode == PTI_CONV_S2PAD) ? pick_ck(p.cin_l, true) : pick_ck2(p.cin_l, p.cout_tile);
   p.total = (long long)p.cout_l * p.cin_l * ksize * ksize;
@@ -941,6 +1265,37 @@
   PackArgs p;
   if (fill_pack(p, w, packed, cout, cin, ksize, mode, transpose_flip, w_f16))
     PTI_FAIL(PTI_EUNSUPPORTED, "pack_table_fill: cout=%d cin=%d k=%d", cout, cin, ksize);
+  *(PackArgs*)host_entry = p;
+  *nblocks = (p.total + 2047) / 2048;
+  return PTI_OK;
+}
+static int fill_pack_poly(PackArgs& p, const float* w, void* packed, int cout, int cin, int kind, int f16) {
+  if (cout <= 0 || cin <= 0 || cout % 32 || cin % 32 || kind < PTI_POLY_UP2_FWD || kind > PTI_POLY_S2_DGRAD) return -1;
+  const int flip = kind == PTI_POLY_UP2_DGRAD || kind == PTI_POLY_S2_DGRAD;
+  if (fill_pack(p, w, packed, cout, cin, 3, PTI_CONV_S1, flip, f16)) return -1;
+  p.poly = 1 + kind;
+  p.total = (long long)16 * cout * cin;
+  return 0;
+}
+extern "C" int64_t pti_conv_poly_packed_bytes(int cout, int cin) {
+  if (cout <= 0 || cin <= 0 || cout % 32 || cin % 32) return 0;
+  return (int64_t)2 * 16 * cout * cin;
+}
+extern "C" int pti_conv_pack_weights_poly(const float* w, void* packed, int cout, int cin, int kind, int w_f16, pti_stream_t s) {
+  if (!w || !packed) PTI_FAIL(PTI_EINVAL, "pack_weights_poly: null pointer");
+  PackArgs p;
+  if (fill_pack_poly(p, w, packed, cout, cin, kind, w_f16))
+    PTI_FAIL(PTI_EUNSUPPORTED, "pack_weights_poly: cout=%d cin=%d (multiples of 32) kind=%d (PTI_POLY_*)", cout, cin, kind);
+  PTI_LAUNCH(pack_weights_kernel, dim3((int)((p.total + 2047) / 2048)), dim3(256), 0, (hipStream_t)s, p);
+  PTI_CHECK_LAUNCH("pack_weights_poly");
+  return PTI_OK;
+}
+extern "C" int pti_conv_pack_table_fill_poly(void* host_entry, const float* w, void* packed, int cout, int cin, int kind,
+                                             int w_f16, int64_t* nblocks) {
+  if (!host_entry || !w || !packed || !nblocks) PTI_FAIL(PTI_EINVAL, "pack_table_fill_poly: null pointer");
+  PackArgs p;
+  if (fill_pack_poly(p, w, packed, cout, cin, kind, w_f16))
+    PTI_FAIL(PTI_EUNSUPPORTED, "pack_table_fill_poly: cout=%d cin=%d kind=%d", cout, cin, kind);
   *(PackArgs*)host_entry = p;
   *nblocks = (p.total + 2047) / 2048;
   return PTI_OK;
@@ -971,12 +1326,19 @@
     PTI_FAIL(PTI_EUNSUPPORTED, "conv2d_mfma: cin=%d cout=%d must be positive multiples of 32", d->cin, d->cout);
   if (d->ksize != 1 && d->ksize != 3) PTI_FAIL(PTI_EUNSUPPORTED, "conv2d_mfma: ksize %d", d->ksize);
   if (d->ksize == 1 && d->mode != PTI_CONV_S1) PTI_FAIL(PTI_EUNSUPPORTED, "conv2d_mfma: 1x1 supports PTI_CONV_S1 only");
+  const bool poly = d->mode == PTI_CONV_PHASE_OUT || d->mode == PTI_CONV_PHASE_IN;
+  if (poly && d->ksize != 3) PTI_FAIL(PTI_EUNSUPPORTED, "conv2d_mfma: the polyphase modes stand for 3x3 convs (ksize 3)");
+  if (poly && (d->prologue != PTI_PRO_NONE || d->add_residual || d->pool2x2_out || d->relu_out || gf || act_out))
+    PTI_FAIL(PTI_EUNSUPPORTED, "conv2d_mfma: the polyphase modes take no prologue, residual, pooled output, ReLU, fused GroupNorm backward or side output");
+  if (d->mode == PTI_CONV_PHASE_IN && ((d->h | d->w) & 1))
+    PTI_FAIL(PTI_EUNSUPPORTED, "conv2d_mfma: PTI_CONV_PHASE_IN needs an even input map, got %dx%d", d->h, d->w);
   if (d->n <= 0 || d->h <= 0 || d->w <= 0) PTI_FAIL(PTI_EINVAL, "conv2d_mfma: bad dims");
   int eho, ewo;
   switch (d->mode) {
     case PTI_CONV_S1: eho = d->h; ewo = d->w; break;
     case PTI_CONV_S2PAD: eho = (d->h + 1 - 3) / 2 + 1; ewo = (d->w + 1 - 3) / 2 + 1; break;
-    case PTI_CONV_UP2: case PTI_CONV_ZINS: eho = 2 * d->h; ewo = 2 * d->w; break;
+    case PTI_CONV_UP2: case PTI_CONV_ZINS: case PTI_CONV_PHASE_OUT: eho = 2 * d->h; ewo = 2 * d->w; break;
+    case PTI_CONV_PHASE_IN: eho = d->h / 2; ewo = d->w / 2; break;
     default: PTI_FAIL(PTI_EUNSUPPORTED, "conv2d_mfma: mode %d", d->mode);
   }
   if (d->ho != eho || d->wo != ewo)
@@ -1044,6 +1406,9 @@
   if (d->mode == PTI_CONV_S2PAD) {
     ck = pick_ck(d->cin, true);
     rc = launch_ck<3, 2>(a, ck, cout_tile, (hipStream_t)s);
+  } else if (poly) {
+    ck = pick_ck2(d->cin, cout_tile);
+    rc = launch_poly(a, ck, cout_tile, (hipStream_t)s);
   } else {
     ck = pick_ck2(d->cin, cout_tile);
     rc = (d->ksize == 3 && d->cin == 128 && d->cout == 128 && !a.x2) ? launch_conv_ws128(a, (hipStream_t)s) : 1;
@@ -1052,6 +1417,7 @@
   }
   if (rc == 3) PTI_FAIL(PTI_EUNSUPPORTED, "conv2d_mfma: relu_out needs a plain fp16 forward launch (w_f16, fp16 in/out, no prologue, no side output)");
   if (rc == 2) PTI_FAIL(PTI_EUNSUPPORTED, "conv2d_mfma: no fp16-operand kernel for this launch (w_f16 with this prologue / epilogue)");
+  if (rc == 5) PTI_FAIL(PTI_EUNSUPPORTED, "conv2d_mfma: the polyphase modes need all-fp16 (w_f16) or all-bf16 input, weights and output");
   if (rc == 4) PTI_FAIL(PTI_EUNSUPPORTED, "conv2d_mfma_gnbwd_chain: only 3x3 launches on 128-wide input and output tiles with an fp16 GroupNorm input");
   if (rc != 0) PTI_FAIL(PTI_EUNSUPPORTED, "conv2d_mfma: no kernel for ck=%d cout_tile=%d", ck, cout_tile);
   PTI_CHECK_LAUNCH("conv2d_mfma");
diff --git a/pti_ldm_vae_amd/engine.py b/pti_ldm_vae_amd/engine.py
--- a/pti_ldm_vae_amd/engine.py
+++ b/pti_ldm_vae_amd/engine.py
@@ -53,6 +53,9 @@
     return graphs, results
 
 
+POLY_DEFAULT = ("s2_dgrad",)
+
+
 class _MfmaConv:
 
     def __init__(self, net, wname, bname, ksize, mode, fused_names=None, fwd_f16=True):
@@ -66,6 +69,8 @@
             w = net._param_by_name[wname]
             self.cout, self.cin = w.shape[0], w.shape[1]
         self.wp = self.wpt = None
+        self.poly_fwd = self.poly_dgrad = None
+        self.wq = self.wqt = None
 
     def _w(self):
         if self.fused:
@@ -93,6 +98,10 @@
         ho, wo = ops.conv_out_hw(h, w, self.mode)
         y = _empty((n, ho, wo, self.cout), x.t, out_dtype or eng.act_dtype)
         st = eng.new_stats(n) if want_stats else None
+        odd = self.mode == PTI_CONV_S2PAD and (h % 2 or w % 2)
+        if self.poly_fwd and y.dtype == x.t.dtype and not (pro or odd or residual is not None or act_out is not None):
+            ops.conv_poly(x.t, self.wq, self.bias(), y, cout=self.cout, route=self.poly_fwd, out_stats=st, out_groups=eng.G)
+            return _Act(y, st)
         g, b = (norm.weight.data, norm.bias.data) if norm is not None else (None, None)
         ops.conv_mfma(x.t, self.wp, self.bias(), y, cout=self.cout, ksize=self.ksize, mode=self.mode, prologue=pro,
                       in_stats=x.stats if pro else None, gamma=g, beta=b, groups=eng.G, eps=eng.eps,
@@ -101,6 +110,11 @@
 
     def dgrad(self, dy, *, residual=None):
         n, ho, wo, _ = dy.shape
+        if self.poly_dgrad and residual is None:
+            shape = (n, 2 * ho, 2 * wo, self.cin) if self.mode == PTI_CONV_S2PAD else (n, ho // 2, wo // 2, self.cin)
+            out = _empty(shape, dy)
+            ops.conv_poly(dy, self.wqt, None, out, cout=self.cin, route=self.poly_dgrad)
+            return out
         if self.mode == PTI_CONV_S2PAD:
             out = _empty((n, 2 * ho, 2 * wo, self.cin), dy)
             ops.conv_mfma(dy, self.wpt, None, out, cout=self.cin, ksize=3, mode=PTI_CONV_ZINS, residual=residual)
@@ -396,6 +410,15 @@
         self._wgrad_posts, self._wgrad_zero = [], ()
         self._flush_up = int(os.environ.get("PTI_WGRAD_FLUSH_UP", "1"))
         self.gnbwd_chain = os.environ.get("PTI_GNBWD_CHAIN", "0") == "1"
+        knob = os.environ.get("PTI_RESAMPLE_POLYPHASE", "1")
+        self.poly_routes = () if knob == "0" else POLY_DEFAULT if knob == "1" else tuple(knob.split(","))
+        if any(r not in ops.POLY_ROUTES for r in self.poly_routes):
+            raise ValueError(f"PTI_RESAMPLE_POLYPHASE={knob!r}: 0, 1 or a comma-separated list of {sorted(ops.POLY_ROUTES)}")
+        for l in self.enc_layers + self.dec_layers:
+            if isinstance(l, _Resample):
+                kind = "s2" if l.conv.mode == PTI_CONV_S2PAD else "up2"
+                l.conv.poly_fwd = kind + "_fwd" if kind + "_fwd" in self.poly_routes else None
+                l.conv.poly_dgrad = kind + "_dgrad" if kind + "_dgrad" in self.poly_routes else None
         self.Lc = net.latent_channels
         self._plist = list(net._param_by_name.values())
 
@@ -435,7 +458,7 @@
                                 for t in (self.net.param_arena, self.net.grad_arena, self.workspace_side)}
 
     def _pack_buffer_ids(self):
-        ids = [t.data_ptr() for c in self.mfma_convs for t in (c.wp, c.wpt) if t is not None]
+        ids = [t.data_ptr() for c in self.mfma_convs for t in (c.wp, c.wpt, c.wq, c.wqt) if t is not None]
         for c in self.direct_convs:
             ids += [t.data_ptr() for t in (c.w_tck, c.w_tck_t, c.wp_mfma, c.wpad, c.wp_img, c.wpt_img, c.wpad_img) if t is not None]
         return tuple(ids)
@@ -452,11 +475,17 @@
         if v == self.packed_version:
             return
         if self._packer is None:
-            entries = []
+            entries, rep, targets = [], [], []
             for c in self.mfma_convs:
                 dmode = PTI_CONV_ZINS if c.mode == PTI_CONV_S2PAD else PTI_CONV_S1
-                entries += [(c._w(), c.ksize, c.mode, False, c.f16), (c._w(), c.ksize, dmode, True, False)]
-            rep, targets = [], []
+                for attr, qattr, route, e in (("wp", "wq", c.poly_fwd, (c._w(), c.ksize, c.mode, False, c.f16)),
+                                              ("wpt", "wqt", c.poly_dgrad, (c._w(), c.ksize, dmode, True, False))):
+                    if route is None or route == "s2_fwd":
+                        targets.append((c, attr, len(entries)))
+                        entries.append(e)
+                    if route is not None:
+                        targets.append((c, qattr, len(entries)))
+                        entries.append((c._w(), "poly", route, None, e[4]))
             for c in self.direct_convs:
                 c.alloc()
                 rep += c.repack_entries()
@@ -465,8 +494,6 @@
                     entries.append(e)
             self._direct_repack = ops.DirectRepack(rep)
             self._packer = ops.BatchedPacker(entries, self.dev)
-            for i, c in enumerate(self.mfma_convs):
-                c.wp, c.wpt = self._packer.outputs[2 * i], self._packer.outputs[2 * i + 1]
             for c, attr, i in targets:
                 setattr(c, attr, self._packer.outputs[i])
         self._direct_repack.run()
diff --git a/pti_ldm_vae_amd/ops.py b/pti_ldm_vae_amd/ops.py
--- a/pti_ldm_vae_amd/ops.py
+++ b/pti_ldm_vae_amd/ops.py
@@ -7,7 +7,7 @@
 import torch
 
 from . import _lib as L
-from ._lib import (PTI_CONV_S1, PTI_CONV_S2PAD, PTI_CONV_UP2, PTI_CONV_ZINS, PTI_PRO_GN, PTI_PRO_GN_SILU,
+from ._lib import (PTI_CONV_PHASE_IN, PTI_CONV_PHASE_OUT, PTI_CONV_S1, PTI_CONV_S2PAD, PTI_CONV_UP2, PTI_CONV_ZINS, PTI_PRO_GN, PTI_PRO_GN_SILU,
                    PTI_PRO_NONE, ConvDesc)
 
 BF16 = torch.bfloat16
@@ -94,6 +94,27 @@
     arr = (C.c_void_p * len(ws))(*[w.data_ptr() for w in ws])
     L.check(L.lib().pti_conv_pack_weights(arr, len(ws), _ptr(out), cout, cin, ksize, mode, int(flip), int(f16), _stream()),
             "pti_conv_pack_weights")
+    return out
+
+
+POLY_ROUTES = {"up2_fwd": (L.PTI_POLY_UP2_FWD, PTI_CONV_PHASE_OUT, True),
+               "up2_dgrad": (L.PTI_POLY_UP2_DGRAD, PTI_CONV_PHASE_IN, True),
+               "s2_fwd": (L.PTI_POLY_S2_FWD, PTI_CONV_PHASE_IN, False),
+               "s2_dgrad": (L.PTI_POLY_S2_DGRAD, PTI_CONV_PHASE_OUT, False)}
+
+
+def pack_conv_weight_poly(w, route, out=None, f16=False):
+    _chk(w, F32, "weight")
+    cout, cin = w.shape[0], w.shape[1]
+    nbytes = L.lib().pti_conv_poly_packed_bytes(cout, cin)
+    if nbytes == 0 or w.numel() != cout * cin * 9:
+        raise ValueError(f"pack_conv_weight_poly: unsupported weight {tuple(w.shape)}")
+    if out is None:
+        out = torch.empty(nbytes // 2, dtype=F16 if f16 else BF16, device=w.device)
+    elif out.numel() * 2 != nbytes or out.dtype != (F16 if f16 else BF16):
+        raise ValueError("pack_conv_weight_poly: bad out size")
+    L.check(L.lib().pti_conv_pack_weights_poly(_ptr(w), _ptr(out), cout, cin, POLY_ROUTES[route][0], int(f16), _stream()),
+            "pti_conv_pack_weights_poly")
     return out
 
 
@@ -246,6 +267,39 @@
     return y
 
 
+def conv_poly(x, w_packed, bias, y, *, cout, route, out_stats=None, out_groups=0):
+    _chk(x, ACT16, "x", 4)
+    _chk(y, ACT16, "y", 4)
+    n, h, w, cin = x.shape
+    _, mode, large = POLY_ROUTES[route]
+    if mode == PTI_CONV_PHASE_IN and (h % 2 or w % 2):
+        raise ValueError(f"conv_poly: route {route} needs an even map, got {h}x{w}")
+    ho, wo = (2 * h, 2 * w) if mode == PTI_CONV_PHASE_OUT else (h // 2, w // 2)
+    if tuple(y.shape) != (n, ho, wo, cout):
+        raise ValueError(f"conv_poly: y shape {tuple(y.shape)} != {(n, ho, wo, cout)}")
+    if w_packed.numel() != 16 * cout * cin or w_packed.dtype != x.dtype or y.dtype != x.dtype:
+        raise ValueError("conv_poly: packed weight size, or x / weight / y are not one 16-bit format")
+    if bias is not None:
+        _chk(bias, F32, "bias")
+        if bias.numel() != cout:
+            raise ValueError("conv_poly: bias size")
+    if out_stats is not None:
+        _chk_stats(out_stats, n * out_groups * 2, "out_stats")
+    f16 = int(x.dtype == F16)
+    d = ConvDesc(n=n, h=h, w=w, cin=cin, ho=ho, wo=wo, cout=cout, ksize=3, mode=mode, accum_stats=int(out_stats is not None),
+                 out_groups=out_groups, in_f16=f16, out_f16=f16, w_f16=f16)
+    prof = KERNEL_PROFILE
+    rec = None if prof is None else _prof_begin(prof)
+    L.check(L.lib().pti_conv2d_mfma(_ptr(x), _ptr(w_packed), _ptr(bias), None, None, None, None, _ptr(y), _ptr(out_stats),
+                                    C.byref(d), _stream()), "pti_conv2d_mfma")
+    if rec is not None:
+        hc, wc = (max(h, ho), max(w, wo)) if large else (min(h, ho), min(w, wo))
+        kind = "conv fwd" if route.endswith("fwd") else "conv dgrad"
+        _prof_end(rec, 2.0 * n * hc * wc * cout * cin * 9, 2.0 * (x.numel() + y.numel()),
+                  (kind, cin, cout, hc, wc, 3, route, n))
+    return y
+
+
 def _strides4(t, layout):
     s = t.stride()
     return (s[0], s[2], s[3], s[1]) if layout == "nchw" else (s[0], s[1], s[2], s[3])
@@ -654,10 +708,16 @@
             f16 = bool(rest[0]) if rest else False
             _chk(w, F32, "weight")
             cout, cin = w.shape[0], w.shape[1]
-            out = torch.empty(w.numel(), dtype=F16 if f16 else BF16, device=device)
             nb = C.c_int64(0)
-            L.check(lib.pti_conv_pack_table_fill(C.byref(hbuf, i * esz), _ptr(w), _ptr(out), cout, cin, ksize, mode,
-                                                 int(flip), int(f16), C.byref(nb)), "pti_conv_pack_table_fill")
+            if ksize == "poly":
+                out = torch.empty(16 * cout * cin, dtype=F16 if f16 else BF16, device=device)
+                L.check(lib.pti_conv_pack_table_fill_poly(C.byref(hbuf, i * esz), _ptr(w), _ptr(out), cout, cin,
+                                                          POLY_ROUTES[mode][0], int(f16), C.byref(nb)),
+                        "pti_conv_pack_table_fill_poly")
+            else:
+                out = torch.empty(w.numel(), dtype=F16 if f16 else BF16, device=device)
+                L.check(lib.pti_conv_pack_table_fill(C.byref(hbuf, i * esz), _ptr(w), _ptr(out), cout, cin, ksize, mode,
+                                                     int(flip), int(f16), C.byref(nb)), "pti_conv_pack_table_fill")
             first.append(total)
             total += nb.value
             self.outputs.append(out)
```
